# mihaibujanca/dynamicfusion

Hardware: AMD Instinct MI355X
Metric: frames/sec integrate+raycast, 640x480->512^3 TSDF (higher is better)
Workload: dtype f32 (fp16 TSDF / u16 weight storage, f64 exp + normalise as in the reference)

## Files before the change

dynamicfusion_amd/build.py:

```python
import os
import re
import shutil
import subprocess

PKG_DIR = os.path.dirname(os.path.abspath(__file__))
REPO_DIR = os.path.dirname(PKG_DIR)
CSRC = os.path.join(PKG_DIR, "csrc")
LIB_PATH = os.path.join(PKG_DIR, "libdfusion_hip.so")

SOURCES = ["dfusion_volume.hip", "dfusion_warp.hip", "dfusion_warp_nodes.hip", "dfusion_warp_points.hip", "dfusion_warp_index.hip",
           "dfusion_raycast.hip", "dfusion_frontend.hip", "dfusion_solver.hip", "dfusion_selftest.hip", "dfusion_warp_extend.hip", "dfusion_mesh.hip", "dfusion_associate.hip"]
HEADERS = ["dfusion_device.h", "dfusion_internal.h", "dfusion_nanoflann.h", "dfusion_pyramid.h", "dfusion_warp_topk.h", "dfusion_warp_sweep.h",
           "dfusion_warp_blocks.h", "dfusion_warp_pipe.h", os.path.join(REPO_DIR, "include", "dfusion.h")]

HIPCC_FLAGS = ["--offload-arch=gfx950", "-O3", "-std=c++17", "-ffp-contract=off", "-fPIC", "-shared",
               "-fno-fast-math", "-Wno-unused-result"]


def _hipcc():
    for cand in (shutil.which("hipcc"), "/opt/rocm/bin/hipcc"):
        if cand and os.path.exists(cand):
            return cand
    raise RuntimeError("hipcc not found: the dynamicfusion_amd HIP library cannot be built")


def _stale():
    if not os.path.exists(LIB_PATH):
        return True
    t = os.path.getmtime(LIB_PATH)
    deps = [os.path.join(CSRC, s) for s in SOURCES] + [h if os.path.isabs(h) else os.path.join(CSRC, h) for h in HEADERS]
    return any(os.path.getmtime(d) > t for d in deps)


def _csrc_includes(name, seen):
    if name in seen:
        return seen
    seen.append(name)
    for inc in re.findall(r'^#include "([^"]+)"', open(os.path.join(CSRC, name)).read(), re.M):
        if os.path.exists(os.path.join(CSRC, inc)):
            _csrc_includes(inc, seen)
    return seen


def kernel_source_sha(kernel):
    import hashlib
    k = kernel.replace("void ", "")
    f = ("dfusion_warp_nodes.hip" if k.startswith(("df_pack", "df_node"))
         else "dfusion_warp_points.hip" if k.startswith("df_points")
         else "dfusion_warp_index.hip" if k.startswith(("df_brick", "df_scan", "df_grow"))
         else "dfusion_warp.hip" if k.startswith(("df_warp", "df_sweep", "df_block", "df_blocks", "df_dists_max", "df_alive"))
         else "dfusion_raycast.hip" if k.startswith(("df_raycast", "df_extract"))
         else "dfusion_solver.hip" if k.startswith("df_sv")
         else "dfusion_mesh.hip" if k.startswith("df_mesh")
         else "dfusion_associate.hip" if k.startswith("df_assoc")
         else "dfusion_volume.hip")
    h = hashlib.sha256()
    for name in _csrc_includes(f, []):
        h.update(open(os.path.join(CSRC, name), "rb").read())
    return h.hexdigest()


def build_library(force=False, verbose=False):
    if not force and not _stale():
        return LIB_PATH
    cmd = [_hipcc()] + HIPCC_FLAGS + ["-I", os.path.join(REPO_DIR, "include"), "-I", CSRC]
    cmd += [os.path.join(CSRC, s) for s in SOURCES] + ["-o", LIB_PATH + ".tmp"]
    if verbose:
        print(" ".join(cmd))
    subprocess.check_call(cmd)
    os.replace(LIB_PATH + ".tmp", LIB_PATH)
    return LIB_PATH


HOST_DIR = os.path.join(PKG_DIR, "host")
HOST_LIB = os.path.join(HOST_DIR, "libkfusion_hip.so")
HOST_APP = os.path.join(HOST_DIR, "headless_frame")
HOST_KINFU_APP = os.path.join(HOST_DIR, "kinfu_headless")
HOST_WARP_TESTS = os.path.join(HOST_DIR, "warp_tests")
HOST_DEMO_CALLS = os.path.join(HOST_DIR, "demo_calls")
HOST_REG_SOLVE = os.path.join(HOST_DIR, "reg_solve")
HOST_ROBUST_SOLVE = os.path.join(HOST_DIR, "robust_solve")
HOST_ASSOCIATE = os.path.join(HOST_DIR, "associate")
HOST_PLANE_SOLVE = os.path.join(HOST_DIR, "plane_solve")
HOST_ZSLAB_LIB = os.path.join(HOST_DIR, "libkfusion_zslab.so")
HOST_ZSLAB_APP = os.path.join(HOST_DIR, "zslab_frame")


def build_host(force=False, verbose=False):
    build_library(force=False)
    src = os.path.join(HOST_DIR, "src", "kfusion_hip.cpp")
    app = os.path.join(HOST_DIR, "apps", "headless_frame.cpp")
    app2 = os.path.join(HOST_DIR, "apps", "kinfu_headless.cpp")
    app3 = os.path.join(HOST_DIR, "apps", "warp_tests.cpp")
    app4 = os.path.join(HOST_DIR, "apps", "demo_calls.cpp")
    zsrc = os.path.join(HOST_DIR, "src", "zslab_rccl.cpp")
    app5 = os.path.join(HOST_DIR, "apps", "zslab_frame.cpp")
    app6 = os.path.join(HOST_DIR, "apps", "reg_solve.cpp")
    app7 = os.path.join(HOST_DIR, "apps", "robust_solve.cpp")
    app8 = os.path.join(HOST_DIR, "apps", "associate.cpp")
    app9 = os.path.join(HOST_DIR, "apps", "plane_solve.cpp")
    deps = [src, app, app2, app3, app4, zsrc, app5, app6, app7, app8, app9, LIB_PATH] + [os.path.join(r, f) for r, _, fs in os.walk(os.path.join(HOST_DIR, "include")) for f in fs]
    outs = (HOST_LIB, HOST_APP, HOST_KINFU_APP, HOST_WARP_TESTS, HOST_DEMO_CALLS, HOST_ZSLAB_LIB, HOST_ZSLAB_APP, HOST_REG_SOLVE, HOST_ROBUST_SOLVE, HOST_ASSOCIATE, HOST_PLANE_SOLVE)
    if not force and all(os.path.exists(f) for f in outs) and min(os.path.getmtime(f) for f in outs) >= max(os.path.getmtime(d) for d in deps):
        return HOST_LIB, HOST_APP
    rocm = os.environ.get("ROCM_PATH", "/opt/rocm")
    common = ["g++", "-std=c++17", "-O2", "-D__HIP_PLATFORM_AMD__", "-I", os.path.join(HOST_DIR, "include"),
              "-I", os.path.join(REPO_DIR, "include"), "-I", os.path.join(rocm, "include")]
    link = ["-L", PKG_DIR, "-ldfusion_hip", "-L", os.path.join(rocm, "lib"), "-lamdhip64"]
    cmds = [common + ["-fPIC", "-shared", src, "-o", HOST_LIB] + link + ["-Wl,-rpath,$ORIGIN/.."],
            common + [app, "-o", HOST_APP, "-L", HOST_DIR, "-lkfusion_hip"] + link + ["-Wl,-rpath,$ORIGIN", "-Wl,-rpath,$ORIGIN/.."],
            common + [app2, "-o", HOST_KINFU_APP, "-L", HOST_DIR, "-lkfusion_hip"] + link + ["-Wl,-rpath,$ORIGIN", "-Wl,-rpath,$ORIGIN/.."],
            common + [app3, "-o", HOST_WARP_TESTS, "-L", HOST_DIR, "-lkfusion_hip"] + link + ["-Wl,-rpath,$ORIGIN", "-Wl,-rpath,$ORIGIN/.."],
            common + [app4, "-o", HOST_DEMO_CALLS, "-L", HOST_DIR, "-lkfusion_hip"] + link + ["-Wl,-rpath,$ORIGIN", "-Wl,-rpath,$ORIGIN/.."],
            common + [app6, "-o", HOST_REG_SOLVE, "-L", HOST_DIR, "-lkfusion_hip"] + link + ["-Wl,-rpath,$ORIGIN", "-Wl,-rpath,$ORIGIN/.."],
            common + [app7, "-o", HOST_ROBUST_SOLVE, "-L", HOST_DIR, "-lkfusion_hip"] + link + ["-Wl,-rpath,$ORIGIN", "-Wl,-rpath,$ORIGIN/.."],
            common + [app8, "-o", HOST_ASSOCIATE, "-L", HOST_DIR, "-lkfusion_hip"] + link + ["-Wl,-rpath,$ORIGIN", "-Wl,-rpath,$ORIGIN/.."],
            common + [app9, "-o", HOST_PLANE_SOLVE, "-L", HOST_DIR, "-lkfusion_hip"] + link + ["-Wl,-rpath,$ORIGIN", "-Wl,-rpath,$ORIGIN/.."],
            common + ["-fPIC", "-shared", zsrc, "-o", HOST_ZSLAB_LIB, "-L", HOST_DIR, "-lkfusion_hip"] + link + ["-lrccl", "-Wl,-rpath,$ORIGIN", "-Wl,-rpath,$ORIGIN/.."],
            common + [app5, "-o", HOST_ZSLAB_APP, "-L", HOST_DIR, "-lkfusion_zslab", "-lkfusion_hip"] + link + ["-lrccl", "-Wl,-rpath,$ORIGIN", "-Wl,-rpath,$ORIGIN/.."]]
    for c in cmds:
        if verbose:
            print(" ".join(c))
        subprocess.check_call(c)
    return HOST_LIB, HOST_APP


if __name__ == "__main__":
    print(build_library(force=True, verbose=True))
    print(build_host(force=True, verbose=True))
```

dynamicfusion_amd/capi.py:

```python
import ctypes as C
import os

from . import build as _build

_lib = None


class DfVolume(C.Structure):
    _fields_ = [("data", C.c_void_p), ("dims", C.c_int * 3), ("voxel_size", C.c_float * 3),
                ("trunc_dist", C.c_float), ("max_weight", C.c_int)]


class DfIcpLevel(C.Structure):
    _fields_ = [("curr", C.c_void_p), ("curr_pitch", C.c_size_t), ("ncurr", C.c_void_p), ("ncurr_pitch", C.c_size_t),
                ("prev", C.c_void_p), ("prev_pitch", C.c_size_t), ("nprev", C.c_void_p), ("nprev_pitch", C.c_size_t),
                ("cols", C.c_int), ("rows", C.c_int), ("iters", C.c_int)]


class DfSlab(C.Structure):
    _fields_ = [("z_store0", C.c_int), ("z_store_n", C.c_int), ("z_own0", C.c_int), ("z_own_n", C.c_int)]


DF_WARP_NO_CULL = 1
DF_WARP_NO_TABLE = 2
DF_WARP_NO_WEIGHT_TABLE = 4
DF_WARP_NO_LDS = 8
DF_WARP_NO_PIPELINE = 16
DF_WARP_NO_ZERO_SKIP = 32
DF_WARP_NO_DEPTH_PYRAMID = 64
DF_WARP_NO_BLOCK_MODEL = 128
DF_WARP_BLOCK_MODEL_NOW = 256
DF_WARP_NO_PREFETCH = 512
DF_WARP_STEADY_PREFETCH = 1024
DF_WARP_NO_CODES = 2048
DF_RIGID_NO_DEPTH_CULL = 1
DF_RIGID_NO_SHORT_FORMS = 2
DF_RIGID_KEEP_ALL = 4
DF_RIGID_NO_SAT = 8
DF_RIGID_POISON_SCRATCH = 16
DF_INDEX_VOXEL_TABLE = 1
DF_INDEX_WEIGHT_TABLE = 2
DF_INDEX_TABLES_ON_DEMAND = 4

SYMBOLS = [
    "dfusion_abi_version", "dfusion_error_string", "dfusion_clear", "dfusion_compute_dists", "dfusion_project_and_remove", "dfusion_integrate",
    "dfusion_raycast_points", "dfusion_raycast_depth", "dfusion_raycast_march", "dfusion_raycast_shade", "dfusion_extract_cloud",
    "dfusion_extract_normals", "dfusion_warp_create", "dfusion_warp_destroy",
    "dfusion_warp_set_nodes", "dfusion_warp_set_transforms", "dfusion_warp_build_index", "dfusion_knn",
    "dfusion_warp_points", "dfusion_integrate_warped", "dfusion_copy_bandwidth_probe", "dfusion_read_bandwidth_probe",
    "dfusion_bilateral_filter", "dfusion_truncate_depth", "dfusion_depth_pyramid", "dfusion_compute_normals_mask_depth",
    "dfusion_compute_point_normals", "dfusion_resize_depth_normals", "dfusion_resize_points_normals",
    "dfusion_icp_workspace_floats", "dfusion_icp_sums_points", "dfusion_icp_sums_depth", "dfusion_transform_points", "dfusion_warp_solve_data_term", "dfusion_warp_index_info", "dfusion_icp_estimate", "dfusion_release_scratch", "dfusion_raycast_points_of_keys",
    "dfusion_selftest_exact_forms", "dfusion_warp_set_point_tiling", "dfusion_integrate_ex", "dfusion_warp_debug_counters", "dfusion_warp_alive_blocks", "dfusion_warp_coded_blocks", "dfusion_raycast_points_of_keys_rows", "dfusion_raycast_sum_pieces", "dfusion_raycast_min_pieces", "dfusion_integrate_warped_prepare", "dfusion_integrate_warped_sweep",
    "dfusion_render_image_points", "dfusion_render_image_depth", "dfusion_render_tangent_colors", "dfusion_cloud_to_depth",
    "dfusion_warp_extend", "dfusion_warp_solve", "dfusion_warp_node_graph", "dfusion_extract_mesh",
    "dfusion_warp_solve_robust", "dfusion_associate_projective", "dfusion_warp_solve_plane",
]


class DfusionError(RuntimeError):
    pass


def library_path():
    return _build.LIB_PATH


def lib():
    global _lib
    if _lib is not None:
        return _lib
    try:
        import torch
    except Exception:
        pass
    path = _build.LIB_PATH
    try:
        path = _build.build_library()
    except Exception as e:
        if not os.path.exists(path):
            raise DfusionError("libdfusion_hip.so is missing and could not be built: %s" % e)
    _lib = load(path)
    return _lib


def load(path, strict=True):
    L = C.CDLL(path)
    if not strict:
        class _Missing:
            missing = True
        for s in SYMBOLS:
            if not hasattr(L, s):
                setattr(L, s, _Missing())
    fp = C.POINTER(C.c_float)
    vp = C.c_void_p
    L.dfusion_abi_version.restype = C.c_int
    L.dfusion_error_string.restype = C.c_char_p
    L.dfusion_error_string.argtypes = [C.c_int]
    L.dfusion_clear.argtypes = [DfVolume, C.POINTER(DfSlab), vp]
    L.dfusion_compute_dists.argtypes = [vp, C.c_size_t, vp, C.c_size_t, C.c_int, C.c_int, fp, vp]
    L.dfusion_project_and_remove.argtypes = [vp, C.c_size_t, vp, C.c_size_t, C.c_int, C.c_int, vp, C.c_ulonglong, fp, vp, vp, vp]
    L.dfusion_integrate.argtypes = [vp, C.c_size_t, C.c_int, C.c_int, DfVolume, C.POINTER(DfSlab), fp, fp, vp, vp]
    L.dfusion_raycast_points.argtypes = [DfVolume, C.POINTER(DfSlab), fp, fp, fp, vp, C.c_size_t, vp, C.c_size_t,
                                         C.c_int, C.c_int, C.c_float, C.c_float, vp, vp]
    L.dfusion_raycast_depth.argtypes = [DfVolume, C.POINTER(DfSlab), fp, fp, fp, vp, C.c_size_t, vp, C.c_size_t,
                                        C.c_int, C.c_int, C.c_float, C.c_float, vp]
    L.dfusion_raycast_march.argtypes = [DfVolume, C.POINTER(DfSlab), fp, fp, C.c_int, C.c_int, C.c_float, C.c_uint, vp, vp]
    L.dfusion_raycast_shade.argtypes = [DfVolume, C.POINTER(DfSlab), fp, fp, fp, vp, vp, C.c_size_t, vp, C.c_size_t,
                                        C.c_int, C.c_int, C.c_float, vp]
    L.dfusion_raycast_points_of_keys.argtypes = [fp, fp, fp, vp, vp, C.c_size_t, vp, C.c_size_t, C.c_int, C.c_int, vp]
    L.dfusion_raycast_points_of_keys_rows.argtypes = [fp, fp, fp, vp, vp, C.c_size_t, vp, C.c_size_t, C.c_int, C.c_int, C.c_int, C.c_int, vp]
    L.dfusion_extract_cloud.argtypes = [DfVolume, C.POINTER(DfSlab), fp, vp, C.c_ulonglong, vp, vp]
    L.dfusion_extract_normals.argtypes = [DfVolume, C.POINTER(DfSlab), fp, fp, vp, C.c_ulonglong, C.c_float, vp, vp]
    L.dfusion_extract_mesh.argtypes = [DfVolume, C.POINTER(DfSlab), fp, vp, C.c_ulonglong, vp, C.c_ulonglong, vp, vp]
    L.dfusion_warp_create.argtypes = [C.POINTER(vp)]
    L.dfusion_warp_destroy.argtypes = [vp]
    L.dfusion_warp_set_nodes.argtypes = [vp, vp, vp, vp, C.c_int, vp]
    L.dfusion_warp_set_transforms.argtypes = [vp, vp, vp]
    L.dfusion_warp_build_index.argtypes = [vp, DfVolume, C.POINTER(DfSlab), fp, C.c_int, C.c_uint, vp]
    L.dfusion_knn.argtypes = [vp, C.c_int, vp, C.c_int, vp, vp, vp]
    L.dfusion_warp_points.argtypes = [vp, C.c_int, vp, vp, C.c_int, fp, vp]
    L.dfusion_integrate_warped.argtypes = [vp, C.c_size_t, C.c_int, C.c_int, DfVolume, C.POINTER(DfSlab), fp, fp, fp,
                                           vp, C.c_int, C.c_uint, vp, vp]
    sz = C.c_size_t
    L.dfusion_bilateral_filter.argtypes = [vp, sz, vp, sz, C.c_int, C.c_int, C.c_int, C.c_float, C.c_float, vp]
    L.dfusion_truncate_depth.argtypes = [vp, sz, C.c_int, C.c_int, C.c_float, vp]
    L.dfusion_cloud_to_depth.argtypes = [vp, sz, vp, sz, C.c_int, C.c_int, vp]
    L.dfusion_depth_pyramid.argtypes = [vp, sz, C.c_int, C.c_int, vp, sz, C.c_float, vp]
    L.dfusion_compute_normals_mask_depth.argtypes = [vp, sz, vp, sz, C.c_int, C.c_int, fp, vp]
    L.dfusion_compute_point_normals.argtypes = [vp, sz, vp, sz, vp, sz, C.c_int, C.c_int, fp, vp]
    L.dfusion_resize_depth_normals.argtypes = [vp, sz, vp, sz, C.c_int, C.c_int, vp, sz, vp, sz, vp]
    L.dfusion_resize_points_normals.argtypes = [vp, sz, vp, sz, C.c_int, C.c_int, vp, sz, vp, sz, vp]
    L.dfusion_transform_points.argtypes = [vp, sz, C.c_int, vp, sz, C.c_int, C.c_int, C.c_int, fp, vp]
    L.dfusion_warp_solve_data_term.argtypes = [vp, C.c_int, vp, vp, C.c_int, C.c_int, C.c_float, vp, vp, vp]
    L.dfusion_warp_solve.argtypes = [vp, C.c_int, vp, vp, C.c_int, C.c_int, C.c_float, C.c_int, C.c_float, vp, vp, vp]
    L.dfusion_warp_node_graph.argtypes = [vp, C.c_int, vp, vp, vp]
    L.dfusion_warp_solve_robust.argtypes = [vp, C.c_int, vp, vp, C.c_int, C.c_int, C.c_float, C.c_int, C.c_float, C.c_int, C.c_float, C.c_float,
                                            vp, vp, vp, vp, vp]
    L.dfusion_warp_solve_plane.argtypes = [vp, C.c_int, vp, vp, vp, C.c_int, C.c_int, C.c_float, C.c_int, C.c_float, C.c_int, C.c_float, C.c_float,
                                           vp, vp, vp, vp, vp]
    L.dfusion_associate_projective.argtypes = [vp, vp, C.c_int, vp, C.c_size_t, vp, C.c_size_t, C.c_int, C.c_int, fp, C.c_float, C.c_float, C.c_float,
                                               vp, vp, vp, vp]
    L.dfusion_warp_extend.argtypes = [vp, C.c_int, vp, C.c_int, C.c_float, C.c_float, C.c_int, vp, vp, vp, C.POINTER(C.c_int),
                                      C.POINTER(C.c_int), vp]
    L.dfusion_warp_index_info.argtypes = [vp, C.POINTER(C.c_ulonglong), C.POINTER(C.c_uint), C.POINTER(C.c_int)]
    L.dfusion_selftest_exact_forms.argtypes = [C.c_ulonglong, vp, vp]
    L.dfusion_raycast_sum_pieces.argtypes = [vp, C.c_int, C.c_ulonglong, vp, vp]
    L.dfusion_raycast_min_pieces.argtypes = [vp, C.c_int, C.c_ulonglong, vp, vp]
    L.dfusion_integrate_warped_prepare.argtypes = [vp, C.c_size_t, C.c_int, C.c_int, DfVolume, C.POINTER(DfSlab), fp, fp, fp, vp, C.c_int, C.c_uint, vp]
    L.dfusion_integrate_warped_sweep.argtypes = [DfVolume, C.POINTER(DfSlab), vp, vp, vp]
    L.dfusion_warp_set_point_tiling.argtypes = [vp, C.c_int]
    L.dfusion_icp_estimate.argtypes = [C.POINTER(DfIcpLevel), C.c_int, C.c_int, fp, C.c_float, C.c_float, vp, vp, vp]
    L.dfusion_icp_workspace_floats.argtypes = [C.c_int, C.c_int]
    L.dfusion_icp_sums_points.argtypes = [vp, sz, vp, sz, vp, sz, vp, sz, C.c_int, C.c_int, fp, fp, C.c_float, C.c_float, vp, vp, vp, vp]
    L.dfusion_icp_sums_depth.argtypes = [vp, sz, vp, sz, vp, sz, vp, sz, C.c_int, C.c_int, fp, fp, C.c_float, C.c_float, vp, vp, vp, vp]
    L.dfusion_render_image_points.argtypes = [vp, sz, vp, sz, C.c_int, C.c_int, fp, vp, sz, vp]
    L.dfusion_render_image_depth.argtypes = [vp, sz, vp, sz, C.c_int, C.c_int, fp, fp, vp, sz, vp]
    L.dfusion_render_tangent_colors.argtypes = [vp, sz, C.c_int, C.c_int, vp, sz, vp]
    L.dfusion_integrate_ex.argtypes = [vp, C.c_size_t, C.c_int, C.c_int, DfVolume, C.POINTER(DfSlab), fp, fp, C.c_uint, vp, vp, vp]
    L.dfusion_warp_debug_counters.argtypes = [vp, vp]
    L.dfusion_warp_alive_blocks.argtypes = [vp, C.c_int, C.c_int, vp, C.c_int, vp]
    L.dfusion_warp_coded_blocks.argtypes = [vp, C.c_int, C.c_int, vp, C.c_int, vp]
    L.dfusion_copy_bandwidth_probe.argtypes = [vp, vp, C.c_size_t, vp]
    L.dfusion_read_bandwidth_probe.argtypes = [vp, C.c_size_t, vp, vp]
    for s in SYMBOLS:
        if s not in ("dfusion_error_string",):
            getattr(L, s).restype = C.c_int
    return L


def check(rc, what=""):
    if rc != 0:
        msg = lib().dfusion_error_string(rc)
        raise DfusionError("%s failed: %s (code %d)" % (what or "dfusion call", msg.decode() if msg else "?", rc))


def floats(seq):
    seq = [float(x) for x in seq]
    return (C.c_float * len(seq))(*seq)
```

dynamicfusion_amd/csrc/dfusion_internal.h:

```cpp
#pragma once
#include <hip/hip_runtime.h>
#include <stdint.h>
#include <string.h>
#include <memory>
#include <utility>
#include "dfusion.h"
#include "dfusion_device.h"
#include "dfusion_nanoflann.h"

#define DF_BRICK 8
#define DF_WARP_PREFETCH_MARGIN_M 0.05f
#define DF_WARP_PREFETCH_CAP 1024u

#define DF_HIP(expr) do { hipError_t e__ = (expr); if (e__ != hipSuccess) return (int)e__; } while (0)
#define DF_LAUNCH_CHECK() do { hipError_t e__ = hipGetLastError(); if (e__ != hipSuccess) return (int)e__; } while (0)

static inline DfSlab df_slab_or_full(const DfVolume& v, const DfSlab* s)
{
    if (s) return *s;
    DfSlab f; f.z_store0 = 0; f.z_store_n = v.dims[2]; f.z_own0 = 0; f.z_own_n = v.dims[2]; return f;
}
static inline bool df_slab_valid(const DfVolume& v, const DfSlab& s)
{
    return s.z_store_n > 0 && s.z_own_n >= 0 && s.z_store0 >= 0 && s.z_store0 + s.z_store_n <= v.dims[2] &&
           s.z_own0 >= s.z_store0 && s.z_own0 + s.z_own_n <= s.z_store0 + s.z_store_n;
}
static inline bool df_volume_valid(const DfVolume& v)
{
    return v.data && v.dims[0] > 0 && v.dims[1] > 0 && v.dims[2] > 0 && (v.dims[0] % 4) == 0 &&
           v.voxel_size[0] > 0 && v.voxel_size[1] > 0 && v.voxel_size[2] > 0 && v.trunc_dist > 0;
}
static inline DfAff df_aff(const float a[12]) { DfAff r; memcpy(r.R, a, 36); memcpy(r.t, a + 9, 12); return r; }
static inline bool df_pitch_ok(size_t pitch, int cols, size_t bpp) { return cols > 0 && pitch >= (size_t)cols * bpp; }

struct DfWarpView {
    const float4* pos_sigma;
    const float4* rot;
    const float4* dual;
    const float4* node_t;
    const float4* rt;
    int M;
    const uint32_t* brick_off;
    const uint16_t* brick_list;
    const float* brick_thr;
    int bx, by, bz;
    DfNfView nf;
};

template <typename T>
struct DfDevBuf {
    T* p = nullptr; size_t cap = 0;
    DfDevBuf() = default;
    DfDevBuf(DfDevBuf&& o) noexcept : p(o.p), cap(o.cap) { o.p = nullptr; o.cap = 0; }
    DfDevBuf& operator=(DfDevBuf&& o) noexcept { std::swap(p, o.p); std::swap(cap, o.cap); return *this; }
    ~DfDevBuf() { (void)hipFree(p); }
    operator T*() const { return p; }
    void release() { (void)hipFree(p); p = nullptr; cap = 0; }
    int reserve(size_t n)
    {
        if (n <= cap) return DF_OK;
        release();
        DF_HIP(hipMalloc((void**)&p, n * sizeof(T)));
        cap = n;
        return DF_OK;
    }
};

struct DfPrepared;

struct __attribute__((visibility("hidden"))) DfWarpField {
    DfWarpField(); ~DfWarpField();
    int device = 0;
    int M = 0, cap = 0;
    DfDevBuf<float4> pos_sigma, rot, dual, node_t;
    DfDevBuf<uint32_t> brick_off, brick_cnt; DfDevBuf<uint16_t> brick_list; DfDevBuf<float> brick_thr;
    size_t off_cap = 0;
    DfDevBuf<uint32_t> scan_tmp; size_t scan_cap = 0;
    int bx = 0, by = 0, bz = 0, k_built = 0;
    int geom_dims[3] = {}; float geom_vs[3] = {}; float geom_aff[12] = {};
    float geom_inv[12] = {}; bool geom_inv_ok = false;
    bool index_valid = false;
    unsigned index_flags = 0; DfSlab index_slab = {};
    DfDevBuf<uint16_t> knn_tab;
    int tab_z0 = 0, tab_zn = 0, tab_k = 0; bool tab_valid = false;
    DfDevBuf<float> w_tab; bool w_tab_valid = false;
    DfDevBuf<float> tile_wmax;
    DfDevBuf<float> bounds_dev;
    int max_phase = 0;
    std::unique_ptr<DfPrepared> prep; bool prep_valid = false;
    hipEvent_t ev_prep_done = nullptr, ev_sweep_done[2] = {}; bool split_events = false;
    DfDevBuf<float4> rot_alt, dual_alt, node_t_alt;
    DfDevBuf<float4> rt, rt_alt;
    unsigned long long seq = 0, recorded_seq = 0;
    unsigned long long ring_seq[2] = {};
    unsigned long long node_reader[2] = {}; int nphase = 0;
    unsigned long long plan_reader[2] = {};
    DfDevBuf<unsigned long long> plan_mask2[2]; DfDevBuf<unsigned int> plan_list2[2]; int pphase = 0; unsigned hphase = 0;
    DfDevBuf<unsigned long long> plan_code2[2];
    DfDevBuf<uint16_t> pyr_mem;
    DfDevBuf<char> solver_ws;
    DfDevBuf<int> graph_nbr; DfDevBuf<float> graph_alpha; DfDevBuf<unsigned int> graph_in_off, graph_in_edge; DfDevBuf<char> graph_ws;
    int graph_kg = 0;
    DfDevBuf<int> pt_ids;
    int pt_image_cols = 0;
    DfDevBuf<DfNfNode> nf_nodes; DfDevBuf<uint16_t> nf_vpos; bool nf_ok = false; int nf_depth = 0;
    DfDevBuf<unsigned int> plan_hist; size_t plan_cap = 0;
    DfDevBuf<uint8_t> blk_state; DfDevBuf<float> blk_wmax; DfDevBuf<uint8_t> blk_alive; DfDevBuf<uint32_t> blk_work, blk_cnt; size_t blk_cap = 0; int blk_phase = 0;
    DfDevBuf<uint8_t> blk_tie;
    DfDevBuf<uint16_t> bm_idx; DfDevBuf<uint32_t> bm_lam, bm_w; DfDevBuf<uint8_t> bm_cnt; size_t bm_cap = 0;
    DfDevBuf<uint32_t> code_tab; size_t code_cap = 0; DfDevBuf<uint32_t> bm_ids; DfDevBuf<uint8_t> bm_coded;
    bool tab_complete = false;
    int tab_sweeps = 0;
    unsigned long long* dbg_swept = nullptr;
    bool alive_valid = false;
    hipStream_t side = nullptr; hipEvent_t ev_fork = nullptr, ev_join = nullptr; bool side_pending = false;
    volatile uint32_t* host_report = nullptr;
    DfDevBuf<char> ext_ws;
    DfDevBuf<char> grow_ws;
};

#define DF_DISPATCH_K(k, ...)                             \
    switch (k) {                                          \
        case 1: { constexpr int K = 1; __VA_ARGS__; } break; \
        case 2: { constexpr int K = 2; __VA_ARGS__; } break; \
        case 3: { constexpr int K = 3; __VA_ARGS__; } break; \
        case 4: { constexpr int K = 4; __VA_ARGS__; } break; \
        case 5: { constexpr int K = 5; __VA_ARGS__; } break; \
        case 6: { constexpr int K = 6; __VA_ARGS__; } break; \
        case 7: { constexpr int K = 7; __VA_ARGS__; } break; \
        case 8: { constexpr int K = 8; __VA_ARGS__; } break; \
        default: return DF_E_INVALID;                     \
    }

struct DfWarpedArgs;
#define DF_LOCAL __attribute__((visibility("hidden")))
DF_LOCAL DfWarpView df_view(const DfWarpField* wf);
DF_LOCAL int df_side_init(DfWarpField* wf);
DF_LOCAL int df_side_join(DfWarpField* wf, hipStream_t st);
DF_LOCAL void df_side_drain(DfWarpField* wf);
DF_LOCAL int df_wait_split_sweep(DfWarpField* wf, hipStream_t st);
DF_LOCAL int df_wait_reader(DfWarpField* wf, unsigned long long reader, hipStream_t st);
DF_LOCAL int df_wait_all_sweeps_host(DfWarpField* wf);
DF_LOCAL int df_warp_reserve(DfWarpField* wf, int M);
DF_LOCAL int df_warp_pack_current(DfWarpField* wf, const float* pos, const float* dq, const float* sigma, hipStream_t st);
DF_LOCAL int df_warp_build_tie_tree(DfWarpField* wf, hipStream_t st);
DF_LOCAL int df_index_bricks(DfWarpField* wf, const DfVolume& v, const float vol2world[12], int k, hipStream_t st);
DF_LOCAL DfWarpedArgs df_table_args(const DfWarpField* wf);
DF_LOCAL int df_tables_complete(DfWarpField* wf, hipStream_t st);
DF_LOCAL int df_build_voxel_table(DfWarpField* wf, const DfVolume& v, const DfSlab& s, const float vol2world[12], int k, bool weights,
                                  bool on_demand, hipStream_t st);

struct DfScratchEntry;
DF_LOCAL DfScratchEntry* df_scratch_acquire(hipStream_t st, size_t bytes, char** mem_out);
DF_LOCAL void df_scratch_release(DfScratchEntry* entry);
struct DfScratchHold {
    char* mem = nullptr; DfScratchEntry* entry;
    DfScratchHold(hipStream_t st, size_t bytes) : entry(df_scratch_acquire(st, bytes, &mem)) {}
    ~DfScratchHold() { if (entry) df_scratch_release(entry); }
    DfScratchHold(const DfScratchHold&) = delete; DfScratchHold& operator=(const DfScratchHold&) = delete;
};

int df_warp_grow(DfWarpField* wf, const float* pos, const float* dq, const float* sigma, int Mn, hipStream_t st);

template <int K>
__device__ __forceinline__ void dqb_weights(const DfWarpView& W, const float (&bd)[K], const int (&bi)[K], float (&wt)[K])
{
#pragma unroll
    for (int i = 0; i < K; ++i) wt[i] = dqb_weight(bd[i], W.pos_sigma[bi[i]].w);
}
template <int K>
__device__ __forceinline__ void dqb_blend_w(const DfWarpView& W, const float (&wt)[K], const int (&bi)[K], quat* rot_out,
                                            quat* dual_out)
{
    quat tsum, rsum;
    tsum.w = tsum.x = tsum.y = tsum.z = 0.f;
    rsum.w = rsum.x = rsum.y = rsum.z = 0.f;
#pragma unroll
    for (int i = 0; i < K; ++i) {
        const int j = bi[i];
        const float w = wt[i];
        const float4 t4 = W.node_t[j], r4 = W.rot[j];
        quat t, r;
        t.w = t4.x; t.x = t4.y; t.y = t4.z; t.z = t4.w;
        r.w = r4.x; r.x = r4.y; r.y = r4.z; r.z = r4.w;
        tsum = q_add(tsum, q_scale(w, t));
        rsum = q_add(rsum, q_scale(w, r));
    }
    rsum = q_normalize(rsum);
    quat half;
    half.w = 0.5f * tsum.w; half.x = 0.5f * tsum.x; half.y = 0.5f * tsum.y; half.z = 0.5f * tsum.z;
    *rot_out = rsum;
    *dual_out = q_mul(half, rsum);
}
```

dynamicfusion_amd/csrc/dfusion_warp.hip:

```cpp
#include "dfusion_internal.h"
#include "dfusion_pyramid.h"
#include "dfusion_warp_sweep.h"
#include "dfusion_warp_blocks.h"
#include "dfusion_warp_pipe.h"
#include <atomic>
#include <stdlib.h>
#include <stdio.h>
#include <math.h>

__global__ __launch_bounds__(256) void df_dists_max_kernel(const uint16_t* __restrict__ dists, size_t pitch, int cols, int rows,
                                                           float* __restrict__ out)
{
    float m = 0.f;
    for (int i = blockIdx.x * 256 + threadIdx.x; i < cols * rows; i += gridDim.x * 256) {
        const int y = i / cols, x = i - y * cols;
        const float d = h2f_bits(*(const uint16_t*)((const char*)dists + (size_t)y * pitch + 2 * (size_t)x));
        if (!(d <= 3.0e38f)) m = 3.0e38f;
        else m = fmaxf(m, d);
    }
#pragma unroll
    for (int o = 32; o >= 1; o >>= 1) m = fmaxf(m, __shfl_xor(m, o, 64));
    if ((threadIdx.x & 63) == 0) atomicMax((unsigned int*)out, __float_as_uint(m));
}

static double df_tile_radius(const float vol2world[12], double nx, double ny, double nz, const DfVolume& v)
{
    double r = 0.0;
    for (int sx = -1; sx <= 1; sx += 2) for (int sy = -1; sy <= 1; sy += 2) for (int sz = -1; sz <= 1; sz += 2) {
        double ex = sx * 0.5 * (nx - 1) * v.voxel_size[0], ey = sy * 0.5 * (ny - 1) * v.voxel_size[1], ez = sz * 0.5 * (nz - 1) * v.voxel_size[2];
        double wx = vol2world[0] * ex + vol2world[1] * ey + vol2world[2] * ez;
        double wy = vol2world[3] * ex + vol2world[4] * ey + vol2world[5] * ez;
        double wz = vol2world[6] * ex + vol2world[7] * ey + vol2world[8] * ez;
        double d = sqrt(wx * wx + wy * wy + wz * wz);
        if (d > r) r = d;
    }
    return r;
}

extern "C" int dfusion_warp_debug_counters(DfWarpField* wf, unsigned long long* swept_dev)
{
    if (!wf) return DF_E_INVALID;
    wf->dbg_swept = swept_dev;
    return DF_OK;
}

__global__ __launch_bounds__(256) void df_alive_per_layer_kernel(const uint8_t* __restrict__ alive, unsigned mask, unsigned per_layer, int layer0, int l_lo,
                                                                 int l_hi, unsigned long long* __restrict__ out)
{
    __shared__ unsigned s[4];
    const int layer = layer0 + (int)blockIdx.x;
    if (layer < l_lo || layer >= l_hi) return;
    const uint8_t* a = alive + (size_t)blockIdx.x * per_layer;
    unsigned n = 0;
    for (unsigned i = threadIdx.x; i < per_layer; i += 256) n += (a[i] & mask) ? 1u : 0u;
#pragma unroll
    for (int o = 32; o >= 1; o >>= 1) n += __shfl_xor(n, o, 64);
    if ((threadIdx.x & 63) == 0) s[threadIdx.x >> 6] = n;
    __syncthreads();
    if (threadIdx.x == 0) atomicAdd(&out[layer], (unsigned long long)(s[0] + s[1] + s[2] + s[3]));
}
static int df_count_verdicts(DfWarpField* wf, unsigned mask, int z0, int zn, unsigned long long* per_layer_dev, int n_layers, dfStream stream)
{
    if (!wf || !per_layer_dev || n_layers <= 0 || z0 < 0 || zn < 0) return DF_E_INVALID;
    if (!wf->tab_valid || !wf->alive_valid || !wf->blk_alive) return DF_E_NO_INDEX;
    const int ntx = (wf->geom_dims[0] + DF_TAB_TX - 1) / DF_TAB_TX, nty = (wf->geom_dims[1] + DF_TAB_TY - 1) / DF_TAB_TY;
    const unsigned per_layer = (unsigned)(ntx * (DF_TAB_TX / 8)) * (unsigned)(nty * (DF_TAB_TY / 8));
    const int nbz = wf->tab_zn / 8, layer0 = wf->tab_z0 / 8;
    const int l_lo = (z0 + 7) / 8, l_hi = min((z0 + zn) / 8, n_layers);
    if (nbz <= 0 || l_hi <= l_lo) return DF_OK;
    hipLaunchKernelGGL(df_alive_per_layer_kernel, dim3((unsigned)nbz), dim3(256), 0, (hipStream_t)stream, wf->blk_alive, mask, per_layer, layer0, l_lo,
                       l_hi, per_layer_dev);
    DF_LAUNCH_CHECK();
    return DF_OK;
}
extern "C" int dfusion_warp_alive_blocks(DfWarpField* wf, int z0, int zn, unsigned long long* per_layer_dev, int n_layers, dfStream stream)
{
    return df_count_verdicts(wf, 0xffu, z0, zn, per_layer_dev, n_layers, stream);
}
extern "C" int dfusion_warp_coded_blocks(DfWarpField* wf, int z0, int zn, unsigned long long* per_layer_dev, int n_layers, dfStream stream)
{
    return df_count_verdicts(wf, 2u, z0, zn, per_layer_dev, n_layers, stream);
}

DfWarpedArgs df_table_args(const DfWarpField* wf)
{
    DfWarpedArgs a;
    memset(&a, 0, sizeof(a));
    const int ntx = (wf->geom_dims[0] + DF_TAB_TX - 1) / DF_TAB_TX, nty = (wf->geom_dims[1] + DF_TAB_TY - 1) / DF_TAB_TY;
    a.w_tab = wf->w_tab_valid ? wf->w_tab : nullptr;
    a.tile_wmax = wf->w_tab_valid ? wf->tile_wmax : nullptr;
    a.blk_wmax = wf->w_tab_valid ? wf->blk_wmax : nullptr;
    a.X = wf->geom_dims[0]; a.Y = wf->geom_dims[1]; a.Z = wf->geom_dims[2];
    a.z_store0 = wf->tab_z0; a.z_own0 = wf->tab_z0; a.z_own_n = wf->tab_zn;
    a.vsx = wf->geom_vs[0]; a.vsy = wf->geom_vs[1]; a.vsz = wf->geom_vs[2];
    a.vol2world = df_aff(wf->geom_aff);
    a.knn_tab = wf->knn_tab; a.tab_z0 = wf->tab_z0; a.tab_ntx = ntx; a.tab_nty = nty;
    a.tab_nvox = (size_t)ntx * DF_TAB_TX * nty * DF_TAB_TY * wf->tab_zn;
    a.bz0 = wf->tab_z0 / DF_BRICK;
    a.bm_nbx = ntx * (DF_TAB_TX / 8); a.bm_nby = nty * (DF_TAB_TY / 8);
    a.code_tab = wf->code_tab; a.bm_ids = wf->bm_ids; a.bm_coded = wf->bm_coded;
    a.blk_tie = wf->blk_tie;
    return a;
}
static size_t df_lds_limit()
{
    static std::atomic<size_t> cached{0};
    size_t v = cached.load();
    if (v) return v;
    int dev = 0, bytes = 0;
    if (hipGetDevice(&dev) != hipSuccess || hipDeviceGetAttribute(&bytes, hipDeviceAttributeMaxSharedMemoryPerBlock, dev) != hipSuccess || bytes < 64 * 1024) {
        (void)hipGetLastError();
        bytes = 64 * 1024;
    }
    v = (size_t)bytes < (size_t)160 * 1024 ? (size_t)bytes : (size_t)160 * 1024;
    cached.store(v);
    return v;
}

static unsigned df_work_grid(const void* kernel)
{
    int per_cu = 0, dev = 0; hipDeviceProp_t prop;
    if (hipOccupancyMaxActiveBlocksPerMultiprocessor(&per_cu, kernel, 256, 0) != hipSuccess || per_cu < 1) per_cu = 2;
    if (hipGetDevice(&dev) != hipSuccess || hipGetDeviceProperties(&prop, dev) != hipSuccess || prop.multiProcessorCount < 1) return 512u;
    return (unsigned)per_cu * (unsigned)prop.multiProcessorCount;
}

static int df_build_listed(DfWarpField* wf, const uint32_t* cnt, hipStream_t st, int list = 0)
{
    DfWarpedArgs b = df_table_args(wf);
    b.work = wf->blk_work + (size_t)list * wf->blk_cap; b.work_cnt = cnt + (list ? 3 : 0); b.work_cursor = const_cast<uint32_t*>(cnt) + (list ? 4 : 2);
    b.work_cap = list ? DF_WARP_PREFETCH_CAP : 0u;
    const DfWarpView W = df_view(wf);
    static unsigned grid[9] = {0};
    DF_DISPATCH_K(wf->tab_k, {
        if (!grid[K]) grid[K] = df_work_grid((const void*)df_warp_brick_kernel<K, true>);
        df_warp_brick_kernel<K, true><<<dim3(grid[K]), dim3(256), 0, st>>>(b, W);
    });
    DF_LAUNCH_CHECK();
    return DF_OK;
}

int df_tables_complete(DfWarpField* wf, hipStream_t st)
{
    if (wf->tab_complete) return DF_OK;
    const DfWarpedArgs b = df_table_args(wf);
    const int nbz = wf->tab_zn / 8;
    const size_t nblk = (size_t)b.bm_nbx * b.bm_nby * nbz;
    uint32_t* cnt = wf->blk_cnt + 8 * wf->blk_phase;
    uint32_t* cnt_next = wf->blk_cnt + 8 * (wf->blk_phase ^ 1);
    hipLaunchKernelGGL(df_blocks_unbuilt_kernel, dim3((unsigned)((nblk + 255) / 256)), dim3(256), 0, st, b.bm_nbx, b.bm_nby, nbz, wf->bx, wf->by,
                       wf->tab_z0 / 8, wf->blk_state, wf->blk_work, cnt, cnt_next);
    DF_LAUNCH_CHECK();
    wf->blk_phase ^= 1;
    int rc = df_build_listed(wf, cnt, st);
    if (rc) return rc;
    wf->tab_complete = true;
    return DF_OK;
}

static int df_block_verdicts(DfWarpField* wf, DfWarpedArgs& a, int k, unsigned flags, hipStream_t st)
{
    const int nbx = a.tab_ntx * (DF_TAB_TX / 8), nby = a.tab_nty * (DF_TAB_TY / 8), nbz = wf->tab_zn / 8;
    const size_t nblk = (size_t)nbx * nby * nbz;
    if (nblk == 0 || nblk > wf->blk_cap) return DF_E_INVALID;
    const bool use_models = !(flags & DF_WARP_NO_BLOCK_MODEL) && (k == 8 || k == 4);
    const int want_models = !use_models ? 0 : (flags & DF_WARP_BLOCK_MODEL_NOW) ? 2 : wf->tab_sweeps >= 1 ? 1 : 0;
    if (want_models && nblk > wf->bm_cap) {
        wf->bm_cap = 0;
        { int rc = wf->bm_idx.reserve(nblk * DF_BM_NU); if (rc) return rc; }
        { int rc = wf->bm_lam.reserve(nblk * DF_BM_NU); if (rc) return rc; }
        { int rc = wf->bm_w.reserve(nblk * DF_BM_NU); if (rc) return rc; }
        { int rc = wf->bm_cnt.reserve(nblk); if (rc) return rc; }
        wf->bm_cap = nblk;
    }
    if (want_models && k == 8 && (nblk * 512 > wf->code_cap || !wf->bm_ids || !wf->code_tab || !wf->bm_coded)) {
        wf->code_cap = 0;
        { int rc = wf->bm_ids.reserve(nblk * 64); if (rc) return rc; }
        { int rc = wf->code_tab.reserve(nblk * 512); if (rc) return rc; }
        { int rc = wf->bm_coded.reserve(nblk); if (rc) return rc; }
        DF_HIP(hipMemsetAsync(wf->bm_coded, 0, nblk, st));
        wf->code_cap = nblk * 512;
    }
    bool ahead = !(flags & (DF_WARP_NO_PREFETCH | DF_WARP_BLOCK_MODEL_NOW));
    if (ahead) { int rc = df_side_init(wf); if (rc) return rc; }
    if (ahead && !(flags & DF_WARP_STEADY_PREFETCH) && wf->tab_sweeps >= 8 && (wf->tab_sweeps & 7) != 0 && wf->host_report &&
        wf->host_report[0] == 0u && wf->host_report[1] == 0u && wf->host_report[2] == 0u) ahead = false;
    const bool quiet = !ahead && !(flags & (DF_WARP_NO_PREFETCH | DF_WARP_BLOCK_MODEL_NOW));
    const int want_models_policy = want_models;
    const int want_models_now = quiet ? 0 : want_models_policy;
    a.pf_margin = ahead && !wf->tab_complete && wf->tab_sweeps >= 1 ? DF_WARP_PREFETCH_MARGIN_M : 0.f;
    a.pf_cap = DF_WARP_PREFETCH_CAP;
    uint32_t* cnt = wf->blk_cnt + 8 * wf->blk_phase;
    uint32_t* cnt_next = wf->blk_cnt + 8 * (wf->blk_phase ^ 1);
    uint32_t* list_urgent = wf->blk_work, *list_ahead = wf->blk_work + wf->blk_cap, *list_model = wf->blk_work + 2 * wf->blk_cap;
    hipLaunchKernelGGL(df_block_verdict_kernel, dim3((unsigned)((nblk + 255) / 256)), dim3(256), 0, st, a, wf->rot, wf->node_t, nbx, nby, nbz,
                       wf->blk_state, wf->blk_wmax, wf->brick_thr + wf->off_cap, wf->bx, wf->by, a.tile_wmax != nullptr ? 1 : 0,
                       (use_models && wf->bm_cap >= nblk ? 1 : 0) | (k == 8 && wf->bm_cnt && wf->code_tab && wf->bm_ids && wf->bm_coded && wf->code_cap >= nblk * 512 ? 2 : 0),
                       want_models_now,
                       wf->tab_complete ? 0 : 1, wf->bm_idx, wf->bm_lam, wf->bm_w, wf->bm_cnt, wf->bm_coded, wf->blk_alive, list_urgent, list_ahead, list_model,
                       cnt, cnt_next);
    a.blk_cnt = cnt; a.host_report = (uint32_t*)wf->host_report; a.sweep_no = (uint32_t)wf->tab_sweeps;
    DF_LAUNCH_CHECK();
#ifdef DF_TRACE_VERDICT
    if (getenv("DF_TRACE_VERDICT_FILE")) {
        DF_HIP(hipStreamSynchronize(st));
        static unsigned long long h[8192 * 4];
        DF_HIP(hipMemcpyFromSymbol(h, HIP_SYMBOL(g_df_vtrace), sizeof(h)));
        FILE* f = fopen(getenv("DF_TRACE_VERDICT_FILE"), "wb");
        if (f) { fwrite(h, 8, 8192 * 4, f); fclose(f); }
    }
#endif
    wf->blk_phase ^= 1;
    auto launch_models = [&](hipStream_t s2) -> int {
        const DfWarpedArgs b = df_table_args(wf);
        static unsigned g8 = 0, g4 = 0;
        if (!g8) {
            g8 = df_work_grid((const void*)df_block_model_kernel<8>); g4 = df_work_grid((const void*)df_block_model_kernel<4>);
        }
        if (k == 8) hipLaunchKernelGGL(df_block_model_kernel<8>, dim3(g8), dim3(256), 0, s2, b, nbx, nby, nbz, list_model, cnt + 1,
                                       wf->bm_idx, wf->bm_lam, wf->bm_w, wf->bm_cnt, wf->blk_state);
        else hipLaunchKernelGGL(df_block_model_kernel<4>, dim3(g4), dim3(256), 0, s2, b, nbx, nby, nbz, list_model, cnt + 1,
                                wf->bm_idx, wf->bm_lam, wf->bm_w, wf->bm_cnt, wf->blk_state);
        DF_LAUNCH_CHECK();
        return DF_OK;
    };
    const bool side_work = ahead && (!wf->tab_complete || want_models_now);
    if (side_work) {
        DF_HIP(hipEventRecord(wf->ev_fork, st));
        DF_HIP(hipStreamWaitEvent(wf->side, wf->ev_fork, 0));
        int rc_side = DF_OK;
        if (!wf->tab_complete) rc_side = df_build_listed(wf, cnt, wf->side, 1);
        if (rc_side == DF_OK && want_models_now) rc_side = launch_models(wf->side);
        if (hipEventRecord(wf->ev_join, wf->side) == hipSuccess) wf->side_pending = true;
        else { (void)hipGetLastError(); df_side_drain(wf); if (rc_side == DF_OK) rc_side = (int)hipErrorUnknown; }
        if (rc_side != DF_OK) return rc_side;
    }
    if (!wf->tab_complete) { int rc = df_build_listed(wf, cnt, st, 0); if (rc) return rc; }
    if (want_models_now && !ahead) { int rc = launch_models(st); if (rc) return rc; }
    a.blk_alive = wf->blk_alive; a.bm_nbx = nbx; a.bm_nby = nby;
    wf->alive_valid = true;
    return DF_OK;
}

typedef void (*df_lds_kernel_t)(const DfWarpedArgs, const DfWarpView, int);
struct DfPrepared { DfWarpedArgs a; DfWarpView W; df_lds_kernel_t kern; dim3 grid; unsigned threads; size_t lds; int tiles_x; DfVolume v; DfSlab s; unsigned long long seq; };
DfWarpField::DfWarpField() = default;
DfWarpField::~DfWarpField() = default;
enum { DF_MODE_WHOLE = 0, DF_MODE_PREPARE = 1 };

static int df_integrate_warped_impl(const uint16_t* dists, size_t pitch, int cols, int rows, DfVolume v, const DfSlab* slab,
                                    const float vol2world[12], const float world2cam[12], const float proj[4],
                                    DfWarpField* wf, int k, unsigned flags, unsigned long long* n_updated, dfStream stream, int mode);

extern "C" int dfusion_integrate_warped(const uint16_t* dists, size_t pitch, int cols, int rows, DfVolume v, const DfSlab* slab,
                                        const float vol2world[12], const float world2cam[12], const float proj[4],
                                        DfWarpField* wf, int k, unsigned flags, unsigned long long* n_updated, dfStream stream)
{
    return df_integrate_warped_impl(dists, pitch, cols, rows, v, slab, vol2world, world2cam, proj, wf, k, flags, n_updated, stream, DF_MODE_WHOLE);
}

extern "C" int dfusion_integrate_warped_prepare(const uint16_t* dists, size_t pitch, int cols, int rows, DfVolume geometry, const DfSlab* slab,
                                                const float vol2world[12], const float world2cam[12], const float proj[4],
                                                DfWarpField* wf, int k, unsigned flags, dfStream stream)
{
    if (!wf) return DF_E_INVALID;
    if (!wf->split_events) {
        hipEvent_t e[3] = {nullptr, nullptr, nullptr};
        for (int i = 0; i < 3; ++i)
            if (hipEventCreateWithFlags(&e[i], hipEventDisableTiming) != hipSuccess) {
                for (int j = 0; j < i; ++j) (void)hipEventDestroy(e[j]);
                return (int)hipGetLastError();
            }
        wf->ev_prep_done = e[0]; wf->ev_sweep_done[0] = e[1]; wf->ev_sweep_done[1] = e[2]; wf->split_events = true;
    }
    wf->prep_valid = false;
    if (!geometry.data) geometry.data = (void*)(size_t)16;
    const int rc = df_integrate_warped_impl(dists, pitch, cols, rows, geometry, slab, vol2world, world2cam, proj, wf, k, flags, nullptr, stream, DF_MODE_PREPARE);
    if (rc != DF_OK) return rc;
    DF_HIP(hipEventRecord(wf->ev_prep_done, (hipStream_t)stream));
    return DF_OK;
}

extern "C" int dfusion_integrate_warped_sweep(DfVolume v, const DfSlab* slab, DfWarpField* wf, unsigned long long* n_updated, dfStream stream)
{
    if (!wf || !df_volume_valid(v)) return DF_E_INVALID;
    const DfSlab s = df_slab_or_full(v, slab);
    if (!df_slab_valid(v, s)) return DF_E_INVALID;
    if (s.z_own_n == 0) return DF_OK;
    DfPrepared* P = wf->prep.get();
    if (!P || !wf->prep_valid) return DF_E_INVALID;
    if (memcmp(P->v.dims, v.dims, sizeof(v.dims)) || memcmp(P->v.voxel_size, v.voxel_size, sizeof(v.voxel_size)) || P->v.trunc_dist != v.trunc_dist ||
        P->v.max_weight != v.max_weight || memcmp(&P->s, &s, sizeof(s))) return DF_E_INVALID;
    hipStream_t st = (hipStream_t)stream;
    wf->prep_valid = false;
    DF_HIP(hipStreamWaitEvent(st, wf->ev_prep_done, 0));
    P->a.vol = (uint32_t*)v.data; P->a.n_upd = n_updated;
    P->kern<<<P->grid, dim3(P->threads), P->lds, st>>>(P->a, P->W, P->tiles_x);
    DF_LAUNCH_CHECK();
    DF_HIP(hipEventRecord(wf->ev_sweep_done[P->seq & 1], st));
    wf->recorded_seq = P->seq; wf->ring_seq[P->seq & 1] = P->seq;
    return DF_OK;
}

static int df_integrate_warped_impl(const uint16_t* dists, size_t pitch, int cols, int rows, DfVolume v, const DfSlab* slab,
                                    const float vol2world[12], const float world2cam[12], const float proj[4],
                                    DfWarpField* wf, int k, unsigned flags, unsigned long long* n_updated, dfStream stream, int mode)
{
    if (!dists || !vol2world || !world2cam || !proj || !wf || cols <= 0 || rows <= 0 || !df_pitch_ok(pitch, cols, 2) || !df_volume_valid(v)) return DF_E_INVALID;
    if (k < 1 || k > 8 || wf->M < k) return DF_E_INVALID;
    DfSlab s = df_slab_or_full(v, slab);
    if (!df_slab_valid(v, s)) return DF_E_INVALID;
    if (!wf->index_valid || wf->k_built < k || memcmp(wf->geom_dims, v.dims, sizeof(wf->geom_dims)) ||
        memcmp(wf->geom_vs, v.voxel_size, sizeof(wf->geom_vs)) || memcmp(wf->geom_aff, vol2world, sizeof(wf->geom_aff)))
        return DF_E_NO_INDEX;
    if (s.z_own_n == 0) return DF_OK;
    hipStream_t st = (hipStream_t)stream;
    if (mode == DF_MODE_WHOLE) { int rc = df_wait_split_sweep(wf, st); if (rc) return rc; }
    { int rc = df_side_join(wf, st); if (rc) return rc; }
    wf->prep_valid = false;

    DfWarpedArgs a;
    memset(&a, 0, sizeof(a));
    a.vol = (uint32_t*)v.data; a.X = v.dims[0]; a.Y = v.dims[1]; a.Z = v.dims[2];
    a.z_store0 = s.z_store0; a.z_own0 = s.z_own0; a.z_own_n = s.z_own_n;
    a.vsx = v.voxel_size[0]; a.vsy = v.voxel_size[1]; a.vsz = v.voxel_size[2];
    a.vol2world = df_aff(vol2world); a.world2cam = df_aff(world2cam);
    {
        static const float I9[9] = {1.f, 0.f, 0.f, 0.f, 1.f, 0.f, 0.f, 0.f, 1.f};
        a.v2w_identity = memcmp(vol2world, I9, sizeof(I9)) == 0;
    }
    a.P.dists = dists; a.P.pitch = pitch; a.P.cols = cols; a.P.rows = rows;
    a.P.fx = proj[0]; a.P.fy = proj[1]; a.P.cx = proj[2]; a.P.cy = proj[3];
    a.P.trunc = v.trunc_dist; a.P.trunc_inv = 1.f / v.trunc_dist; a.P.max_weight = v.max_weight;
    a.sat_ok = df_sat_trunc_ok(v.trunc_dist) ? 1 : 0;
    a.n_upd = n_updated;
    a.n_swept = wf->dbg_swept;
    a.kf = (float)k; a.cam_scale = 1.f; a.origin_cam = -1.f;
    const bool use_tab = wf->tab_valid && wf->tab_k == k && !(flags & DF_WARP_NO_TABLE) && s.z_own0 >= wf->tab_z0 &&
                         s.z_own0 + s.z_own_n <= wf->tab_z0 + wf->tab_zn;
    const bool use_w = use_tab && wf->w_tab_valid && !(flags & DF_WARP_NO_WEIGHT_TABLE);
    if (use_tab) {
        a.knn_tab = wf->knn_tab; a.tab_z0 = wf->tab_z0;
        a.tab_ntx = (a.X + DF_TAB_TX - 1) / DF_TAB_TX; a.tab_nty = (a.Y + DF_TAB_TY - 1) / DF_TAB_TY;
        a.tab_nvox = (size_t)a.tab_ntx * DF_TAB_TX * a.tab_nty * DF_TAB_TY * wf->tab_zn;
    }
    if (use_w) a.w_tab = wf->w_tab;
    const size_t lds_limit = df_lds_limit();
    const bool no_lds = (flags & DF_WARP_NO_LDS) != 0;
    const bool lds_fits = (size_t)wf->M * 32 <= lds_limit;
    const bool pipe_form_ok = use_w && !(flags & DF_WARP_NO_PIPELINE) && pitch < (1u << 24) && rows < (1 << 24) &&
                              (unsigned long long)rows * pitch < (1ull << 32) && (unsigned long long)v.dims[0] * v.dims[1] < (1ull << 30);
    const bool pipe_sweep = use_tab && !no_lds && pipe_form_ok && (k == 8 || k == 4);

    if (!(flags & DF_WARP_NO_CULL) && proj[0] > 0.f && proj[1] > 0.f) {
        if (!(flags & DF_WARP_NO_DEPTH_PYRAMID)) {
            const size_t elems = df_pyramid_elems(cols, rows);
            { int rc = wf->pyr_mem.reserve(elems); if (rc) return rc; }
            const bool pipe_path = pipe_sweep;
            wf->max_phase ^= 1;
            unsigned int* max_word = (unsigned int*)(wf->bounds_dev + 6 + wf->max_phase);
            int rc = df_build_dists_pyramid(dists, pitch, cols, rows, wf->pyr_mem, wf->pyr_mem.cap, &a.py, st, pipe_path, nullptr,
                                            pipe_path ? max_word : nullptr);
            if (rc) return rc;
        }
        if (a.py.top == 0) {
            DF_HIP(hipMemsetAsync(wf->bounds_dev + 2, 0, sizeof(float), st));
            hipLaunchKernelGGL(df_dists_max_kernel, dim3(64), dim3(256), 0, st, dists, pitch, cols, rows, wf->bounds_dev + 2);
            DF_LAUNCH_CHECK();
        }
        {
            bool rigid = true;
            for (int i = 0; i < 3 && rigid; ++i)
                for (int j = 0; j < 3; ++j) {
                    double d = 0.0;
                    for (int r = 0; r < 3; ++r) d += (double)world2cam[3 * r + i] * world2cam[3 * r + j];
                    if (!(fabs(d - (i == j ? 1.0 : 0.0)) < 1e-5)) { rigid = false; break; }
                }
            a.origin_cam = rigid ? (float)(sqrt((double)world2cam[9] * world2cam[9] + (double)world2cam[10] * world2cam[10] +
                                                (double)world2cam[11] * world2cam[11]) * 1.0001 + 1e-6) : -1.f;
        }
        const double r = use_tab ? df_tile_radius(vol2world, DF_ROW_TX, DF_ROW_TY, DF_ROW_TZ, v)
                                 : df_tile_radius(vol2world, DF_BRICK, DF_BRICK, DF_BRICK, v);
        double fro = 0.0;
        for (int i = 0; i < 9; ++i) fro += (double)world2cam[i] * world2cam[i];
        fro = sqrt(fro);
        a.cam_scale = (float)((fabs(fro - 1.7320508075688772) < 1e-3) ? 1.001 : fro * 1.001);
        a.tile_r = (float)(r * 1.001 + 1e-6);
        a.cull = wf->bounds_dev;
        if (use_w && !(flags & DF_WARP_NO_ZERO_SKIP)) a.tile_wmax = wf->tile_wmax;
    }

    DfWarpView W = df_view(wf);
    if (use_tab && !no_lds && (pipe_sweep || lds_fits)) {
        const int tiles_x = (a.X + DF_ROW_TX - 1) / DF_ROW_TX, tiles_y = (a.Y + DF_LDS_TY - 1) / DF_LDS_TY;
        const int zt_lo = s.z_own0 / DF_ROW_TZ, zt_hi = (s.z_own0 + s.z_own_n - 1) / DF_ROW_TZ;
        a.bz0 = zt_lo;
        const bool pipe_ok = pipe_sweep;
        if (a.cull) a.tile_r = (float)(df_tile_radius(vol2world, pipe_ok ? 8 : DF_ROW_TX, pipe_ok ? 8 : DF_LDS_TY, DF_ROW_TZ, v) * 1.001 + 1e-6);
        const bool k4_table = pipe_ok && k == 4 && lds_fits;
        const size_t lds = !pipe_ok || k4_table ? (size_t)wf->M * 32 : k == 8 ? (size_t)(DF_PIPE_WGT / 64) * 4096 : 0;
        typedef void (*lds_kernel_t)(const DfWarpedArgs, const DfWarpView, int);
        lds_kernel_t kern = nullptr;
        const long long cols_layers = (long long)tiles_x * tiles_y * (zt_hi - zt_lo + 1);
        const bool pipe = pipe_sweep;
        a.zt = !pipe ? DF_LDS_ZT : cols_layers <= 8192 ? 4 : cols_layers <= 65536 ? 8 : 16;
        dim3 grid((unsigned)(tiles_x * tiles_y), (unsigned)((zt_hi - zt_lo + 1 + a.zt - 1) / a.zt));
        const bool wide = k4_table && lds > 80 * 1024;
        const bool vi = a.v2w_identity != 0;
        unsigned wg_threads = 512u;
        if (pipe_ok && k == 8) {
            kern = vi ? df_warp_rows_pipe_kernel<8, 1, DF_PIPE_WGT, true, false> : df_warp_rows_pipe_kernel<8, 1, DF_PIPE_WGT, false, false>;
            wg_threads = (unsigned)DF_PIPE_WGT;
        } else if (pipe_ok && k4_table) {
            kern = wide ? (vi ? df_warp_rows_pipe_kernel<4, 2, 1024, true, true> : df_warp_rows_pipe_kernel<4, 2, 1024, false, true>)
                        : (vi ? df_warp_rows_pipe_kernel<4, 2, 512, true, true> : df_warp_rows_pipe_kernel<4, 2, 512, false, true>);
            wg_threads = wide ? 1024u : 512u;
        } else if (pipe_ok) {
            kern = vi ? df_warp_rows_pipe_kernel<4, 2, 512, true, false> : df_warp_rows_pipe_kernel<4, 2, 512, false, false>;
        }
        else if (use_w) { DF_DISPATCH_K(k, kern = (df_warp_rows_lds_kernel<K, true, 2>)); }
        else { DF_DISPATCH_K(k, kern = (df_warp_rows_lds_kernel<K, false, 1>)); }
        if (lds > lds_limit) return DF_E_INVALID;
        DF_HIP(hipFuncSetAttribute((const void*)kern, hipFuncAttributeMaxDynamicSharedMemorySize, (int)lds_limit));
        if (!pipe) { int rc = df_tables_complete(wf, st); if (rc) return rc; }
        if (pipe) {
            const unsigned n_zb = grid.y, n_items = (unsigned)tiles_x * (unsigned)tiles_y * 2u * n_zb;
            if (n_items > wf->plan_cap) {
                { int rc = df_wait_all_sweeps_host(wf); if (rc) return rc; }
                wf->plan_cap = 0;
                for (int i = 0; i < 2; ++i) {
                    { int rc = wf->plan_mask2[i].reserve(n_items); if (rc) return rc; }
                    { int rc = wf->plan_list2[i].reserve((size_t)n_items * DF_PLAN_BINS); if (rc) return rc; }
                    { int rc = wf->plan_code2[i].reserve(n_items); if (rc) return rc; }
                }
                wf->plan_cap = n_items; wf->plan_reader[0] = wf->plan_reader[1] = 0;
            }
            if (!wf->plan_hist) {
                { int rc = wf->plan_hist.reserve(4 * 128); if (rc) return rc; }
                DF_HIP(hipMemsetAsync(wf->plan_hist, 0, 4 * 128 * sizeof(unsigned int), st));
                wf->hphase = 0;
            }
            wf->pphase ^= 1;
            { int rc = df_wait_reader(wf, wf->plan_reader[wf->pphase], st); if (rc) return rc; }
            if (a.cull) { int rc = df_block_verdicts(wf, a, k, flags, st); if (rc) return rc; }
            else { int rc = df_tables_complete(wf, st); if (rc) return rc; }
            ++wf->tab_sweeps;
            unsigned int* cnt = wf->plan_hist + 128 * (wf->hphase & 3u);
            unsigned int* cnt_next = wf->plan_hist + 128 * ((wf->hphase + 2u) & 3u);
            unsigned long long* pmask = wf->plan_mask2[wf->pphase]; unsigned int* plist = wf->plan_list2[wf->pphase];
            unsigned long long* pcode = nullptr;
            if (k == 8 && a.cull && a.blk_alive && wf->code_tab && wf->bm_ids && wf->bm_coded && wf->bm_cap >= (size_t)a.bm_nbx * a.bm_nby * (wf->tab_zn / 8) &&
                !(flags & (DF_WARP_NO_BLOCK_MODEL | DF_WARP_NO_CODES))) {
                pcode = wf->plan_code2[wf->pphase];
                a.code_tab = wf->code_tab; a.bm_ids = wf->bm_ids; a.bm_coded = wf->bm_coded;
            }
            hipLaunchKernelGGL(df_sweep_plan_kernel, dim3((n_items + DF_PLAN_WG / 64 - 1) / (DF_PLAN_WG / 64)), dim3(DF_PLAN_WG), 0, st, a, tiles_x, tiles_y, n_items, pmask, cnt,
                               plist, cnt_next, pcode);
            DF_LAUNCH_CHECK();
            a.plan_code = pcode;
            ++wf->hphase;
            a.plan_mask = pmask; a.plan_bins = plist; a.plan_cnt = cnt; a.plan_items = n_items; a.plan_tiles_y = tiles_y;
            wf->plan_reader[wf->pphase] = wf->node_reader[wf->nphase] = ++wf->seq;
            const unsigned spw = wg_threads >= 256u ? wg_threads / 256u : 1u;
            const unsigned groups = (n_items + spw - 1) / spw;
            grid = dim3(groups, 1);
#ifdef DF_TRACE_WG
            static unsigned long long* trace_dev = nullptr; static size_t trace_cap = 0;
            const size_t trace_n = (size_t)groups * (wg_threads / 64u) * 4;
            if (trace_n > trace_cap) { (void)hipFree(trace_dev); DF_HIP(hipMalloc((void**)&trace_dev, trace_n * 8)); trace_cap = trace_n; }
            DF_HIP(hipMemsetAsync(trace_dev, 0, trace_n * 8, st));
            a.trace = trace_dev;
            kern<<<grid, dim3(wg_threads), lds, st>>>(a, W, tiles_x);
            if (getenv("DF_TRACE_FILE")) {
                DF_HIP(hipStreamSynchronize(st));
                unsigned long long* h = (unsigned long long*)malloc(trace_n * 8);
                DF_HIP(hipMemcpy(h, trace_dev, trace_n * 8, hipMemcpyDeviceToHost));
                FILE* f = fopen(getenv("DF_TRACE_FILE"), "wb");
                if (f) { unsigned long long hdr[4] = {groups, 1, (unsigned long long)(wg_threads / 64u), 0}; fwrite(hdr, 8, 4, f); fwrite(h, 8, trace_n, f); fclose(f); }
                free(h);
            }
            DF_LAUNCH_CHECK();
            return DF_OK;
#endif
        }
        if (mode == DF_MODE_PREPARE) {
            if (!pipe) return DF_E_INVALID;
            if (!wf->prep) wf->prep.reset(new DfPrepared());
            DfPrepared* P = wf->prep.get();
            P->a = a; P->W = W; P->kern = kern; P->grid = grid; P->threads = wg_threads; P->lds = lds; P->tiles_x = tiles_x; P->v = v; P->s = s;
            P->seq = wf->seq;
            wf->prep_valid = true;
            return DF_OK;
        }
        kern<<<grid, dim3(wg_threads), lds, st>>>(a, W, tiles_x);
        if (pipe && wf->split_events) {
            DF_LAUNCH_CHECK();
            DF_HIP(hipEventRecord(wf->ev_sweep_done[wf->seq & 1], st));
            wf->recorded_seq = wf->seq; wf->ring_seq[wf->seq & 1] = wf->seq;
        }
    } else if (use_tab) {
        if (mode == DF_MODE_PREPARE) return DF_E_INVALID;
        { int rc = df_tables_complete(wf, st); if (rc) return rc; }
        const int tiles_x = (a.X + DF_ROW_TX - 1) / DF_ROW_TX, tiles_y = (a.Y + DF_ROW_TY - 1) / DF_ROW_TY;
        const int zt_lo = s.z_own0 / DF_ROW_TZ, zt_hi = (s.z_own0 + s.z_own_n - 1) / DF_ROW_TZ;
        a.bz0 = zt_lo;
        dim3 grid((unsigned)(tiles_x * tiles_y), (unsigned)(zt_hi - zt_lo + 1));
        if (use_w) { DF_DISPATCH_K(k, df_warp_rows_kernel<K, true, 4><<<grid, dim3(256), 0, st>>>(a, W, tiles_x)); }
        else { DF_DISPATCH_K(k, df_warp_rows_kernel<K, false, 4><<<grid, dim3(256), 0, st>>>(a, W, tiles_x)); }
    } else {
        if (mode == DF_MODE_PREPARE) return DF_E_INVALID;
        const int bz_lo = s.z_own0 / DF_BRICK, bz_hi = (s.z_own0 + s.z_own_n - 1) / DF_BRICK;
        a.bz0 = bz_lo;
        dim3 grid((unsigned)(W.bx * W.by), (unsigned)(bz_hi - bz_lo + 1));
        DF_DISPATCH_K(k, df_warp_brick_kernel<K, false><<<grid, dim3(256), 0, st>>>(a, W));
    }
    DF_LAUNCH_CHECK();
    return DF_OK;
}

int df_build_voxel_table(DfWarpField* wf, const DfVolume& v, const DfSlab& s, const float vol2world[12], int k, bool weights,
                                bool on_demand, hipStream_t st)
{
    (void)vol2world;
    if (s.z_own_n == 0) return DF_OK;
    const int bz_lo = s.z_own0 / DF_BRICK, bz_hi = (s.z_own0 + s.z_own_n - 1) / DF_BRICK;
    const int tz0 = bz_lo * DF_BRICK, tzn = (bz_hi - bz_lo + 1) * DF_BRICK;
    const int ntx = (v.dims[0] + DF_TAB_TX - 1) / DF_TAB_TX, nty = (v.dims[1] + DF_TAB_TY - 1) / DF_TAB_TY;
    if (ntx * (DF_TAB_TX / 8) > 1023 || nty * (DF_TAB_TY / 8) > 1023 || bz_hi > 4095) return DF_E_INVALID;
    const size_t nvox = (size_t)ntx * DF_TAB_TX * nty * DF_TAB_TY * tzn;
    const size_t need = nvox * k;
    { int rc = wf->knn_tab.reserve(need); if (rc) return rc; }
    if (weights) { int rc = wf->w_tab.reserve(need); if (rc) return rc; }
    const size_t ntile = (size_t)ntx * nty * (tzn / DF_TAB_TZ);
    if (weights) {
        { int rc = wf->tile_wmax.reserve(ntile); if (rc) return rc; }
        DF_HIP(hipMemsetAsync(wf->tile_wmax, 0, ntile * sizeof(float), st));
    }
    const size_t nblk = (size_t)ntx * (DF_TAB_TX / 8) * nty * (DF_TAB_TY / 8) * (tzn / 8);
    if (nblk > wf->blk_cap) {
        wf->blk_cap = 0;
        { int rc = wf->blk_state.reserve(nblk); if (rc) return rc; }
        { int rc = wf->blk_tie.reserve(nblk); if (rc) return rc; }
        { int rc = wf->blk_wmax.reserve(nblk); if (rc) return rc; }
        { int rc = wf->blk_alive.reserve(nblk); if (rc) return rc; }
        { int rc = wf->blk_work.reserve(3 * nblk); if (rc) return rc; }
        wf->blk_cap = nblk;
    }
    { int rc = wf->blk_cnt.reserve(16); if (rc) return rc; }
    DF_HIP(hipMemsetAsync(wf->blk_cnt, 0, 16 * sizeof(uint32_t), st));
    DF_HIP(hipMemsetAsync(wf->blk_state, on_demand ? 0 : 1, nblk, st));
    DF_HIP(hipMemsetAsync(wf->blk_tie, 0, nblk, st));
    DF_HIP(hipMemsetAsync(wf->blk_wmax, 0, nblk * sizeof(float), st));
    wf->blk_phase = 0;
    wf->tab_z0 = tz0; wf->tab_zn = tzn; wf->tab_k = k; wf->tab_valid = true; wf->w_tab_valid = weights;
    wf->tab_complete = !on_demand; wf->tab_sweeps = 0; wf->alive_valid = false;
    if (on_demand) return DF_OK;
    const DfWarpedArgs a = df_table_args(wf);
    DfWarpView W = df_view(wf);
    dim3 grid((unsigned)(W.bx * W.by), (unsigned)(bz_hi - bz_lo + 1));
    DF_DISPATCH_K(k, df_warp_brick_kernel<K, true><<<grid, dim3(256), 0, st>>>(a, W));
    hipError_t e = hipGetLastError();
    if (e == hipSuccess) e = hipStreamSynchronize(st);
    if (e != hipSuccess) {
        wf->tab_valid = false; wf->w_tab_valid = false; wf->tab_complete = false;
        return (int)e;
    }
    return DF_OK;
}
```

dynamicfusion_amd/csrc/dfusion_warp_blocks.h:

```cpp
#pragma once
#include "dfusion_warp_sweep.h"

#define DF_BM_NU 16
#define DF_BM_NONE 0xffu

struct DfIv { float lo, hi; };
__device__ __forceinline__ DfIv iv(float lo, float hi) { DfIv r; r.lo = lo; r.hi = hi; return r; }
__device__ __forceinline__ DfIv iv_add(DfIv a, DfIv b) { return iv(a.lo + b.lo, a.hi + b.hi); }
__device__ __forceinline__ DfIv iv_sub(DfIv a, DfIv b) { return iv(a.lo - b.hi, a.hi - b.lo); }
__device__ __forceinline__ DfIv iv_mul(DfIv a, DfIv b)
{
    const float p0 = a.lo * b.lo, p1 = a.lo * b.hi, p2 = a.hi * b.lo, p3 = a.hi * b.hi;
    return iv(fminf(fminf(p0, p1), fminf(p2, p3)), fmaxf(fmaxf(p0, p1), fmaxf(p2, p3)));
}
__device__ __forceinline__ DfIv iv_sq(DfIv a)
{
    const float l2 = a.lo * a.lo, h2 = a.hi * a.hi;
    return iv((a.lo <= 0.f && a.hi >= 0.f) ? 0.f : fminf(l2, h2), fmaxf(l2, h2));
}
struct DfIv3 { DfIv x, y, z; };
__device__ __forceinline__ DfIv3 iv_cross(const DfIv3& a, const DfIv3& b)
{
    DfIv3 r;
    r.x = iv_sub(iv_mul(a.y, b.z), iv_mul(a.z, b.y));
    r.y = iv_sub(iv_mul(a.z, b.x), iv_mul(a.x, b.z));
    r.z = iv_sub(iv_mul(a.x, b.y), iv_mul(a.y, b.x));
    return r;
}

__device__ __forceinline__ uint32_t df_f2h_up(float x)
{
    _Float16 h = (_Float16)x;
    unsigned short b = __builtin_bit_cast(unsigned short, h);
    if ((float)h < x) b = (unsigned short)(b + 1u);
    return b;
}
__device__ __forceinline__ uint32_t df_bm_pack(float lo, float hi)
{
    const _Float16 m = (_Float16)(0.5f * (lo + hi));
    const float mf = (float)m;
    const float hw = fmaxf(hi - mf, mf - lo) * 1.00390625f + 1e-7f;
    return (uint32_t)__builtin_bit_cast(unsigned short, m) | (df_f2h_up(hw) << 16);
}

template <int K>
__global__ __launch_bounds__(256, K == 8 ? 3 : 4) void df_block_model_kernel(const DfWarpedArgs a, int nbx, int nby, int nbz, const uint32_t* __restrict__ list,
                                                             const uint32_t* __restrict__ count, uint16_t* __restrict__ bm_idx,
                                                             uint32_t* __restrict__ bm_lam, uint32_t* __restrict__ bm_w,
                                                             uint8_t* __restrict__ bm_cnt, uint8_t* __restrict__ blk_state)
{
    __shared__ uint32_t s_idx[4][DF_BM_NU], s_lam[4][DF_BM_NU], s_w[4][DF_BM_NU];
    __shared__ float s_hw[4][DF_BM_NU];
    const int wave = threadIdx.x >> 6, ln = threadIdx.x & 63;
    const size_t nblk = (size_t)nbx * nby * nbz;
    const uint32_t n_work = *count;
    for (uint32_t it = blockIdx.x * 4 + wave; it < n_work; it += gridDim.x * 4) {
    const size_t blk = list[it];
    const int bx = (int)(blk % (size_t)nbx), by = (int)((blk / (size_t)nbx) % (size_t)nby), bz = (int)(blk / ((size_t)nbx * nby));
    const int x = bx * 8 + (ln & 7), y = by * 8 + (ln >> 3), z0 = a.tab_z0 + bz * 8;
    const bool col_in = x < a.X && y < a.Y;
    int ids[8][K];
    float wv[8][K], inv[8];
    bool bad = false;
    unsigned valid = 0;
#pragma unroll
    for (int j = 0; j < 8; ++j) {
        const bool in = col_in && z0 + j < a.Z;
        const size_t tv = df_tab_index(a, in ? x : 0, in ? y : 0, in ? z0 + j : z0);
        knn_tab_load<K>(a.knn_tab, tv, ids[j]);
        w_tab_load<K>(a.w_tab, a.tab_nvox, tv, wv[j]);
        float s = 0.f;
#pragma unroll
        for (int i = 0; i < K; ++i) s += wv[j][i];
        inv[j] = 1.f / s;
        if (in) { valid |= 1u << j; if (!(s > 1e-30f && s < 3.0e38f)) bad = true; }
    }
    bad = __builtin_amdgcn_ballot_w64(bad) != 0ull;
    const bool any_valid = __builtin_amdgcn_ballot_w64(valid != 0u) != 0ull;
    int n = 0, last = -1;
    bool overflow = false;
    if (!bad && any_valid) {
        for (;;) {
            int cand = 0x7fffffff;
#pragma unroll
            for (int j = 0; j < 8; ++j)
                if (valid & (1u << j)) {
#pragma unroll
                    for (int i = 0; i < K; ++i) { const int id = ids[j][i]; cand = (id > last && id < cand) ? id : cand; }
                }
#pragma unroll
            for (int o = 32; o >= 1; o >>= 1) cand = min(cand, __shfl_xor(cand, o, 64));
            if (cand == 0x7fffffff) break;
            if (n == DF_BM_NU) { overflow = true; break; }
            float lmin = 3.0e38f, lmax = 0.f, wmin = 3.0e38f, wmax = 0.f;
#pragma unroll
            for (int j = 0; j < 8; ++j)
                if (valid & (1u << j)) {
                    float w = 0.f;
#pragma unroll
                    for (int i = 0; i < K; ++i) w = ids[j][i] == cand ? wv[j][i] : w;
                    const float lam = w * inv[j];
                    lmin = fminf(lmin, lam); lmax = fmaxf(lmax, lam); wmin = fminf(wmin, w); wmax = fmaxf(wmax, w);
                }
#pragma unroll
            for (int o = 32; o >= 1; o >>= 1) {
                lmin = fminf(lmin, __shfl_xor(lmin, o, 64)); lmax = fmaxf(lmax, __shfl_xor(lmax, o, 64));
                wmin = fminf(wmin, __shfl_xor(wmin, o, 64)); wmax = fmaxf(wmax, __shfl_xor(wmax, o, 64));
            }
            if (ln == 0) {
                const uint32_t lp = df_bm_pack(lmin * (1.f - 0x1p-18f), lmax * (1.f + 0x1p-18f));
                s_idx[wave][n] = (uint32_t)cand; s_lam[wave][n] = lp; s_w[wave][n] = df_bm_pack(wmin, wmax);
                s_hw[wave][n] = h2f_bits(lp >> 16);
            }
            last = cand; ++n;
        }
    }
    __builtin_amdgcn_wave_barrier();
    if constexpr (K == 8) {
        if (a.code_tab && a.bm_ids && !any_valid) { if (ln == 0) a.bm_coded[blk] = 0; }
        if (a.code_tab && a.bm_ids && any_valid) {
            unsigned code[8];
#pragma unroll
            for (int j = 0; j < 8; ++j) code[j] = 0u;
            int last_h[2] = {-1, -1};
            bool sub_over = false;
            const bool writer = (ln & 0x1b) == 0;
            const unsigned qd = ((unsigned)(ln >> 2) & 1u) | (((unsigned)(ln >> 5) & 1u) << 1);
            uint32_t* ids_out = a.bm_ids + blk * 64;
            ids_out[ln] = 0u;
            __builtin_amdgcn_wave_barrier();
            for (int e = 0;; ++e) {
                int cand_h[2];
#pragma unroll
                for (int h = 0; h < 2; ++h) {
                    int c = 0x7fffffff;
#pragma unroll
                    for (int j = 4 * h; j < 4 * h + 4; ++j)
                        if (valid & (1u << j)) {
#pragma unroll
                            for (int i = 0; i < K; ++i) { const int id = ids[j][i]; c = (id > last_h[h] && id < c) ? id : c; }
                        }
                    c = min(c, __shfl_xor(c, 1, 64)); c = min(c, __shfl_xor(c, 2, 64)); c = min(c, __shfl_xor(c, 8, 64)); c = min(c, __shfl_xor(c, 16, 64));
                    cand_h[h] = c;
                }
                if (__builtin_amdgcn_ballot_w64(cand_h[0] != 0x7fffffff || cand_h[1] != 0x7fffffff) == 0ull) break;
                if (e == DF_BM_NU) { sub_over = true; break; }
#pragma unroll
                for (int h = 0; h < 2; ++h) {
                    if (cand_h[h] == 0x7fffffff) continue;
#pragma unroll
                    for (int j = 4 * h; j < 4 * h + 4; ++j)
                        if (valid & (1u << j)) {
                            unsigned hit = 0u;
#pragma unroll
                            for (int i = 0; i < K; ++i) hit = ids[j][i] == cand_h[h] ? (unsigned)e << (4 * i) : hit;
                            code[j] |= hit;
                        }
                    if (writer) ((uint16_t*)(ids_out + qd * 16 + (unsigned)e))[h] = (uint16_t)cand_h[h];
                    last_h[h] = cand_h[h];
                }
            }
            if (!sub_over) {
#pragma unroll
                for (int j = 0; j < 8; ++j)
                    if (col_in && z0 + j < a.Z) a.code_tab[df_code_index(a, x, y, z0 + j)] = code[j];
            }
            __builtin_amdgcn_wave_barrier();
            if (ln == 0) a.bm_coded[blk] = sub_over ? (uint8_t)0 : (uint8_t)1;
        }
    }
    if (ln == 0) blk_state[blk] = 2;
    if (bad || overflow || n == 0) { if (ln == 0) bm_cnt[blk] = DF_BM_NONE; continue; }
    float h = ln < n ? s_hw[wave][ln] : -1.f;
    int e0 = ln;
#pragma unroll
    for (int o = 32; o >= 1; o >>= 1) {
        const float ho = __shfl_xor(h, o, 64); const int eo = __shfl_xor(e0, o, 64);
        if (ho > h || (ho == h && eo < e0)) { h = ho; e0 = eo; }
    }
    if (ln < n) {
        const int dst = ln == e0 ? 0 : ln == 0 ? e0 : ln;
        bm_idx[(size_t)dst * nblk + blk] = (uint16_t)s_idx[wave][ln];
        bm_lam[(size_t)dst * nblk + blk] = s_lam[wave][ln];
        bm_w[(size_t)dst * nblk + blk] = s_w[wave][ln];
    }
    if (ln == 0) bm_cnt[blk] = (uint8_t)n;
    __builtin_amdgcn_wave_barrier();
    }
}

__device__ __forceinline__ bool df_block_box_dead(const DfWarpedArgs& a, const float4* __restrict__ rot, const float4* __restrict__ node_t,
                                                  int nbx, int nby, size_t nblk, size_t blk, unsigned n, const uint16_t* __restrict__ bm_idx,
                                                  const uint32_t* __restrict__ bm_lam, const uint32_t* __restrict__ bm_w)
{
    float slm = 0.f, Nx = 0.f, Ny = 0.f, Nz = 0.f, Ex = 0.f, Ey = 0.f, Ez = 0.f, Dmin = 3.0e38f, Dmax = 0.f;
    float Tx = 0.f, Ty = 0.f, Tz = 0.f, Fx = 0.f, Fy = 0.f, Fz = 0.f, sx = 0.f, sy = 0.f, sz = 0.f;
    {   const float4 r0 = rot[bm_idx[blk]]; sx = r0.y; sy = r0.z; sz = r0.w; }
    for (unsigned e0 = 0; e0 < n; e0 += 4) {
        unsigned id[4]; uint32_t lp[4], wp[4];
#pragma unroll
        for (int i = 0; i < 4; ++i) {
            const size_t at = (size_t)min(e0 + (unsigned)i, n - 1u) * nblk + blk;
            id[i] = bm_idx[at]; lp[i] = bm_lam[at]; wp[i] = bm_w[at];
        }
        float4 r4[4], t4[4];
#pragma unroll
        for (int i = 0; i < 4; ++i) { r4[i] = rot[id[i]]; t4[i] = node_t[id[i]]; }
#pragma unroll
        for (int i = 0; i < 4; ++i) {
            const bool on = e0 + (unsigned)i < n;
            const float lm = on ? h2f_bits(lp[i]) : 0.f, lh = on ? h2f_bits(lp[i] >> 16) : 0.f, wm = on ? h2f_bits(wp[i]) : 0.f, wh = on ? h2f_bits(wp[i] >> 16) : 0.f;
            slm += lm;
            Nx += lm * r4[i].y; Ny += lm * r4[i].z; Nz += lm * r4[i].w;
            Ex += lh * fabsf(r4[i].y - sx); Ey += lh * fabsf(r4[i].z - sy); Ez += lh * fabsf(r4[i].w - sz);
            Dmin = fminf(Dmin, r4[i].x); Dmax = fmaxf(Dmax, r4[i].x);
            Tx += wm * t4[i].y; Ty += wm * t4[i].z; Tz += wm * t4[i].w;
            Fx += wh * fabsf(t4[i].y); Fy += wh * fabsf(t4[i].z); Fz += wh * fabsf(t4[i].w);
        }
    }
    const float rest = 1.f - slm;
    Nx += rest * sx; Ny += rest * sy; Nz += rest * sz;
    bool dead = false;
    if (Dmin > 0.f) {
        const float id0 = 1.f / Dmin, id1 = 1.f / Dmax;
        DfIv3 U, Q;
        U.x = iv(fminf((Nx - Ex) * id0, (Nx - Ex) * id1), fmaxf((Nx + Ex) * id0, (Nx + Ex) * id1));
        U.y = iv(fminf((Ny - Ey) * id0, (Ny - Ey) * id1), fmaxf((Ny + Ey) * id0, (Ny + Ey) * id1));
        U.z = iv(fminf((Nz - Ez) * id0, (Nz - Ez) * id1), fmaxf((Nz + Ez) * id0, (Nz + Ez) * id1));
        const float umax = fmaxf(fmaxf(fmaxf(fabsf(U.x.lo), fabsf(U.x.hi)), fmaxf(fabsf(U.y.lo), fabsf(U.y.hi))), fmaxf(fabsf(U.z.lo), fabsf(U.z.hi)));
        const bool u_ok = umax < 1.0e3f;
        const int bx = (int)(blk % (size_t)nbx), by = (int)((blk / (size_t)nbx) % (size_t)nby), bz = (int)(blk / ((size_t)nbx * nby));
        const int x0 = bx * 8, y0 = by * 8, z0 = a.tab_z0 + bz * 8;
        const int x1 = min(x0 + 7, a.X - 1), y1 = min(y0 + 7, a.Y - 1), z1 = min(z0 + 7, a.Z - 1);
        const float cxv = 0.5f * (float)(x0 + x1) * a.vsx, cyv = 0.5f * (float)(y0 + y1) * a.vsy, czv = 0.5f * (float)(z0 + z1) * a.vsz;
        const float hxv = 0.5f * (float)(x1 - x0) * a.vsx, hyv = 0.5f * (float)(y1 - y0) * a.vsy, hzv = 0.5f * (float)(z1 - z0) * a.vsz;
        const f3 c = aff_mul(a.vol2world, mk3(cxv, cyv, czv));
        const float* M = a.vol2world.R;
        const float hx = fabsf(M[0]) * hxv + fabsf(M[1]) * hyv + fabsf(M[2]) * hzv, hy = fabsf(M[3]) * hxv + fabsf(M[4]) * hyv + fabsf(M[5]) * hzv,
                    hz = fabsf(M[6]) * hxv + fabsf(M[7]) * hyv + fabsf(M[8]) * hzv;
        Q.x = iv(c.x - hx, c.x + hx); Q.y = iv(c.y - hy, c.y + hy); Q.z = iv(c.z - hz, c.z + hz);
        const DfIv3 c1 = iv_cross(U, Q), c2 = iv_cross(U, c1);
        const DfIv ux2 = iv_sq(U.x), uy2 = iv_sq(U.y), uz2 = iv_sq(U.z);
        const DfIv S = iv(2.f / (1.f + (ux2.hi + uy2.hi + uz2.hi)), 2.f / (1.f + (ux2.lo + uy2.lo + uz2.lo)));
        DfIv3 P;
        P.x = iv_add(iv_add(Q.x, iv_mul(S, iv_add(c1.x, c2.x))), iv(Tx - Fx, Tx + Fx));
        P.y = iv_add(iv_add(Q.y, iv_mul(S, iv_add(c1.y, c2.y))), iv(Ty - Fy, Ty + Fy));
        P.z = iv_add(iv_add(Q.z, iv_mul(S, iv_add(c1.z, c2.z))), iv(Tz - Fz, Tz + Fz));
        const f3 pc = mk3(0.5f * (P.x.lo + P.x.hi), 0.5f * (P.y.lo + P.y.hi), 0.5f * (P.z.lo + P.z.hi));
        const float prx = 0.5f * (P.x.hi - P.x.lo), pry = 0.5f * (P.y.hi - P.y.lo), prz = 0.5f * (P.z.hi - P.z.lo);
        const f3 cc = aff_mul(a.world2cam, pc);
        const float* R = a.world2cam.R;
        const float mag = fabsf(pc.x) + fabsf(pc.y) + fabsf(pc.z) + fabsf(cc.x) + fabsf(cc.y) + fabsf(cc.z) + prx + pry + prz;
        const float infl = 1e-3f + 1e-5f * mag;
        const float rx = fabsf(R[0]) * prx + fabsf(R[1]) * pry + fabsf(R[2]) * prz + infl, ry = fabsf(R[3]) * prx + fabsf(R[4]) * pry + fabsf(R[5]) * prz + infl,
                    rz = fabsf(R[6]) * prx + fabsf(R[7]) * pry + fabsf(R[8]) * prz + infl;
        const float xl = cc.x - rx, xh = cc.x + rx, yl = cc.y - ry, yh = cc.y + ry, zl = cc.z - rz, zh = cc.z + rz;
        const bool ok = u_ok && mag < 1.0e15f;
        if (zh <= 0.f) dead = true;
        const float nx = (xl <= 0.f && xh >= 0.f) ? 0.f : fminf(fabsf(xl), fabsf(xh)), ny = (yl <= 0.f && yh >= 0.f) ? 0.f : fminf(fabsf(yl), fabsf(yh)),
                    nz = (zl <= 0.f && zh >= 0.f) ? 0.f : fminf(fabsf(zl), fabsf(zh));
        const float rmin = sqrtf(nx * nx + ny * ny + nz * nz) * 0.9999f;
        float max_dist;
        if (a.py.top != 0) { const uint32_t tb = df_pyramid_image_max(a.py); max_dist = tb < 0x7c00u ? h2f_bits((uint16_t)tb) : 3.0e38f; }
        else max_dist = a.cull[2];
        if (rmin > max_dist * 1.002f + a.P.trunc) dead = true;
        if (!dead && ok && zl > 0.05f) {
            const float il = 1.f / zl, ih = 1.f / zh;
            const float ulo = a.P.fx * fminf(xl * il, xl * ih) + a.P.cx - 2.f, uhi = a.P.fx * fmaxf(xh * il, xh * ih) + a.P.cx + 2.f;
            const float vlo = a.P.fy * fminf(yl * il, yl * ih) + a.P.cy - 2.f, vhi = a.P.fy * fmaxf(yh * il, yh * ih) + a.P.cy + 2.f;
            if (ulo == ulo && uhi == uhi && vlo == vlo && vhi == vhi) {
                if (uhi < 0.f || vhi < 0.f || ulo > (float)(a.P.cols - 1) || vlo > (float)(a.P.rows - 1)) dead = true;
                else if (a.py.top != 0) {
                    const int iu0 = (int)fmaxf(ulo, 0.f), iv0 = (int)fmaxf(vlo, 0.f);
                    const int iu1 = (int)fminf(uhi, (float)(a.P.cols - 1)), iv1 = (int)fminf(vhi, (float)(a.P.rows - 1));
                    const uint32_t dbits = df_pyramid_max_fine(a.py, iu0, iv0, iu1, iv1, 2);
                    if (dbits == 0u) dead = true;
                    else if (dbits < 0x7c00u && rmin > h2f_bits((uint16_t)dbits) * 1.002f + a.P.trunc) dead = true;
                }
            }
        }
        dead = dead && ok;
    }
    return dead;
}

#ifdef DF_TRACE_VERDICT
__device__ unsigned long long g_df_vtrace[8192 * 4];
#define DF_VT(i) do { if ((threadIdx.x & 63) == 0 && blockIdx.x * 4 + (threadIdx.x >> 6) < 8192) g_df_vtrace[(blockIdx.x * 4 + (threadIdx.x >> 6)) * 4 + (i)] = wall_clock64(); } while (0)
#else
#define DF_VT(i) do { } while (0)
#endif
__global__ __launch_bounds__(256) void df_block_verdict_kernel(const DfWarpedArgs a, const float4* __restrict__ rot, const float4* __restrict__ node_t,
                                                               int nbx, int nby, int nbz, uint8_t* __restrict__ blk_state,
                                                               const float* __restrict__ blk_wmax, const float* __restrict__ brick_d1, int vbx, int vby, int zero_skip, int use_models, int want_models,
                                                               int build_on_demand, const uint16_t* __restrict__ bm_idx,
                                                               const uint32_t* __restrict__ bm_lam, const uint32_t* __restrict__ bm_w,
                                                               const uint8_t* __restrict__ bm_cnt, const uint8_t* __restrict__ bm_coded, uint8_t* __restrict__ alive,
                                                               uint32_t* __restrict__ build_list, uint32_t* __restrict__ ahead_list, uint32_t* __restrict__ model_list,
                                                               uint32_t* __restrict__ cnt, uint32_t* __restrict__ cnt_next)
{
    const size_t nblk = (size_t)nbx * nby * nbz;
    const size_t blk = (size_t)blockIdx.x * 256 + threadIdx.x;
    DF_VT(0);
    if (blockIdx.x == 0 && threadIdx.x < 8) cnt_next[threadIdx.x] = 0u;
    bool keep = false, near = false, need_build = false, need_ahead = false, need_model = false;
    int bx = 0, by = 0, bz = 0;
    if (blk < nblk) {
        bx = (int)(blk % (size_t)nbx); by = (int)((blk / (size_t)nbx) % (size_t)nby); bz = (int)(blk / ((size_t)nbx * nby));
        const int x0 = bx * 8, y0 = by * 8, z0 = a.tab_z0 + bz * 8;
        const int own1 = min(a.z_own0 + a.z_own_n, a.Z);
        keep = x0 < a.X && y0 < a.Y && max(z0, a.z_own0) < min(z0 + 8, own1);
        const unsigned st = keep ? blk_state[blk] : 0u;
        if (keep) {
            float wk = a.kf;
            if (zero_skip && st >= 1u) {
                const float wmax = blk_wmax[blk];
                keep = !(wmax * a.cull[3] < DF_ZERO_WEIGHT);
                wk = fminf(wk, wmax * 1.0001f);
            } else if (zero_skip && a.cull[4] < 1.0e30f && a.cull[4] > 0.f) {
                const float dmin = fmaxf(brick_d1[((size_t)(a.tab_z0 / 8 + bz) * vby + by) * vbx + bx] - a.tile_r, 0.f) * 0.999f;
                const float sg = a.cull[4];
                const float wmax = a.kf * 1.001f * __expf(-(dmin * dmin) / (2.f * sg * sg) * 0.998f);
                keep = !(wmax * a.cull[3] < DF_ZERO_WEIGHT);
                wk = fminf(wk, wmax);
            }
            if (keep) {
                const f3 c = aff_mul(a.vol2world, mk3(((float)x0 + 3.5f) * a.vsx, ((float)y0 + 3.5f) * a.vsy, ((float)z0 + 3.5f) * a.vsz));
                if (a.pf_margin > 0.f && st < 2u) {
                    near = !df_tile_culled(a, c, wk, a.pf_margin);
                    keep = near && !df_tile_culled(a, c, wk);
                } else keep = !df_tile_culled(a, c, wk);
            }
        }
        DF_VT(1);
        if (keep && st == 2u && (use_models & 1)) {
            const unsigned n = bm_cnt[blk];
            if (n != DF_BM_NONE && a.cull[1] <= 1.0f) keep = !df_block_box_dead(a, rot, node_t, nbx, nby, nblk, blk, n, bm_idx, bm_lam, bm_w);
        }
        DF_VT(2);
        alive[blk] = keep ? (uint8_t)(1u | ((st == 2u && (use_models & 2) && bm_coded[blk] != 0) ? 2u : 0u)) : (uint8_t)0;
        need_build = keep && build_on_demand && st == 0u;
        need_ahead = !keep && near && build_on_demand && st == 0u;
        need_model = (keep || near) && want_models && (st == 1u || (need_build && want_models > 1));
        if (need_build) blk_state[blk] = 1;
    }
    const unsigned long long mb = __builtin_amdgcn_ballot_w64(need_build), ma = __builtin_amdgcn_ballot_w64(need_ahead), mm = __builtin_amdgcn_ballot_w64(need_model);
    const unsigned long long below = ((unsigned long long)1 << (threadIdx.x & 63)) - 1ull;
    const unsigned code = (unsigned)bx | ((unsigned)by << 10) | ((unsigned)(a.tab_z0 / 8 + bz) << 20);
    if (mb) {
        unsigned base = 0;
        if ((threadIdx.x & 63) == 0) base = atomicAdd(&cnt[0], (unsigned)__popcll(mb));
        base = (unsigned)__builtin_amdgcn_readfirstlane((int)base);
        if (need_build) build_list[base + (unsigned)__popcll(mb & below)] = code;
    }
    if (ma) {
        unsigned base = 0;
        if ((threadIdx.x & 63) == 0) base = atomicAdd(&cnt[3], (unsigned)__popcll(ma));
        base = (unsigned)__builtin_amdgcn_readfirstlane((int)base);
        const unsigned slot = base + (unsigned)__popcll(ma & below);
        if (need_ahead && slot < a.pf_cap) { ahead_list[slot] = code; blk_state[blk] = 1; }
    }
    if (mm) {
        unsigned base = 0;
        if ((threadIdx.x & 63) == 0) base = atomicAdd(&cnt[1], (unsigned)__popcll(mm));
        base = (unsigned)__builtin_amdgcn_readfirstlane((int)base);
        if (need_model) model_list[base + (unsigned)__popcll(mm & below)] = (unsigned)blk;
    }
    DF_VT(3);
}

__global__ __launch_bounds__(256) void df_blocks_unbuilt_kernel(int nbx, int nby, int nbz, int vbx, int vby, int tab_bz0, uint8_t* __restrict__ blk_state,
                                                                uint32_t* __restrict__ build_list, uint32_t* __restrict__ cnt,
                                                                uint32_t* __restrict__ cnt_next)
{
    const size_t nblk = (size_t)nbx * nby * nbz;
    const size_t blk = (size_t)blockIdx.x * 256 + threadIdx.x;
    if (blockIdx.x == 0 && threadIdx.x < 8) cnt_next[threadIdx.x] = 0u;
    bool need = false;
    int bx = 0, by = 0, bz = 0;
    if (blk < nblk) {
        bx = (int)(blk % (size_t)nbx); by = (int)((blk / (size_t)nbx) % (size_t)nby); bz = (int)(blk / ((size_t)nbx * nby));
        need = blk_state[blk] == 0 && bx < vbx && by < vby;
        if (blk_state[blk] == 0) blk_state[blk] = 1;
    }
    const unsigned long long m = __builtin_amdgcn_ballot_w64(need);
    if (m) {
        unsigned base = 0;
        if ((threadIdx.x & 63) == 0) base = atomicAdd(&cnt[0], (unsigned)__popcll(m));
        base = (unsigned)__builtin_amdgcn_readfirstlane((int)base);
        if (need) build_list[base + (unsigned)__popcll(m & (((unsigned long long)1 << (threadIdx.x & 63)) - 1ull))] =
                      (unsigned)bx | ((unsigned)by << 10) | ((unsigned)(tab_bz0 + bz) << 20);
    }
}
```

dynamicfusion_amd/csrc/dfusion_warp_pipe.h:

```cpp
#pragma once
#include "dfusion_warp_sweep.h"

template <int K> struct DfTabRaw;
template <> struct DfTabRaw<8> { uint4 idx; float4 w0, w1; unsigned code; };
template <> struct DfTabRaw<4> { uint2 idx; float4 w0; };
__device__ __forceinline__ void tab_raw_load(const DfWarpedArgs& a, size_t tv, DfTabRaw<8>& r)
{
    r.idx = reinterpret_cast<const uint4*>(a.knn_tab)[tv];
    r.w0 = reinterpret_cast<const float4*>(a.w_tab)[tv];
    r.w1 = reinterpret_cast<const float4*>(a.w_tab)[a.tab_nvox + tv];
}
__device__ __forceinline__ void tab_raw_load(const DfWarpedArgs& a, size_t tv, DfTabRaw<4>& r)
{
    r.idx = reinterpret_cast<const uint2*>(a.knn_tab)[tv];
    r.w0 = reinterpret_cast<const float4*>(a.w_tab)[tv];
}
typedef float df_v4f __attribute__((ext_vector_type(4)));
typedef unsigned int df_v4u __attribute__((ext_vector_type(4)));
typedef unsigned int df_v2u __attribute__((ext_vector_type(2)));
template <typename T> using df_global_ptr = __attribute__((address_space(1))) T*;
template <typename T>
__device__ __forceinline__ df_global_ptr<T> df_wave_uniform(T* p)
{
    const unsigned long long v = (unsigned long long)p;
    const unsigned lo = (unsigned)__builtin_amdgcn_readfirstlane((int)(unsigned)v), hi = (unsigned)__builtin_amdgcn_readfirstlane((int)(unsigned)(v >> 32));
    return (df_global_ptr<T>)(((unsigned long long)hi << 32) | lo);
}
#define DF_TAB_LD(p) __builtin_nontemporal_load(p)
__device__ __forceinline__ void tab_raw_load_at(const DfWarpedArgs& a, size_t rec, size_t rec_c, bool coded, unsigned lane, unsigned lane_c, DfTabRaw<8>& r)
{
    r.idx = make_uint4(0u, 0u, 0u, 0u); r.code = 0u;
    if (coded) {
        r.code = DF_TAB_LD(df_wave_uniform(a.code_tab + rec_c) + lane_c);
    } else {
        const df_v4u i4 = DF_TAB_LD(df_wave_uniform(reinterpret_cast<const df_v4u*>(a.knn_tab) + rec) + lane);
        r.idx = make_uint4(i4.x, i4.y, i4.z, i4.w);
    }
    const df_v4f a4 = DF_TAB_LD(df_wave_uniform(reinterpret_cast<const df_v4f*>(a.w_tab) + rec) + lane);
    const df_v4f b4 = DF_TAB_LD(df_wave_uniform(reinterpret_cast<const df_v4f*>(a.w_tab) + a.tab_nvox + rec) + lane);
    r.w0 = make_float4(a4.x, a4.y, a4.z, a4.w); r.w1 = make_float4(b4.x, b4.y, b4.z, b4.w);
}
__device__ __forceinline__ void tab_raw_load_at(const DfWarpedArgs& a, size_t rec, size_t, bool, unsigned lane, unsigned, DfTabRaw<4>& r)
{
    const df_v2u i2 = DF_TAB_LD(df_wave_uniform(reinterpret_cast<const df_v2u*>(a.knn_tab) + rec) + lane);
    const df_v4f a4 = DF_TAB_LD(df_wave_uniform(reinterpret_cast<const df_v4f*>(a.w_tab) + rec) + lane);
    r.idx = make_uint2(i2.x, i2.y); r.w0 = make_float4(a4.x, a4.y, a4.z, a4.w);
}
__device__ __forceinline__ void tab_raw_unpack(const DfTabRaw<8>& r, int (&bi)[8], float (&wt)[8])
{
    bi[0] = r.idx.x & 0xffff; bi[1] = r.idx.x >> 16; bi[2] = r.idx.y & 0xffff; bi[3] = r.idx.y >> 16;
    bi[4] = r.idx.z & 0xffff; bi[5] = r.idx.z >> 16; bi[6] = r.idx.w & 0xffff; bi[7] = r.idx.w >> 16;
    wt[0] = r.w0.x; wt[1] = r.w0.y; wt[2] = r.w0.z; wt[3] = r.w0.w; wt[4] = r.w1.x; wt[5] = r.w1.y; wt[6] = r.w1.z; wt[7] = r.w1.w;
}
__device__ __forceinline__ void tab_raw_unpack(const DfTabRaw<4>& r, int (&bi)[4], float (&wt)[4])
{
    bi[0] = r.idx.x & 0xffff; bi[1] = r.idx.x >> 16; bi[2] = r.idx.y & 0xffff; bi[3] = r.idx.y >> 16;
    wt[0] = r.w0.x; wt[1] = r.w0.y; wt[2] = r.w0.z; wt[3] = r.w0.w;
}
__device__ __forceinline__ unsigned df_node_off_lo(unsigned v)
{
    unsigned r;
    asm("v_lshlrev_b32_sdwa %0, 5, %1 dst_sel:DWORD dst_unused:UNUSED_PAD src0_sel:DWORD src1_sel:WORD_0" : "=v"(r) : "v"(v));
    return r;
}
__device__ __forceinline__ unsigned df_node_off_hi(unsigned v)
{
    unsigned r;
    asm("v_lshlrev_b32_sdwa %0, 5, %1 dst_sel:DWORD dst_unused:UNUSED_PAD src0_sel:DWORD src1_sel:WORD_1" : "=v"(r) : "v"(v));
    return r;
}
typedef const __attribute__((address_space(3))) df_v4f df_lds_cf4;
__device__ __forceinline__ df_v2f df_pk_mul_lo(df_v2f w, df_v2f q)
{
    df_v2f r;
    asm("v_pk_mul_f32 %0, %1, %2 op_sel_hi:[0,1]" : "=v"(r) : "v"(w), "v"(q));
    return r;
}
__device__ __forceinline__ df_v2f df_pk_mul_hi(df_v2f w, df_v2f q)
{
    df_v2f r;
    asm("v_pk_mul_f32 %0, %1, %2 op_sel:[1,0] op_sel_hi:[1,1]" : "=v"(r) : "v"(w), "v"(q));
    return r;
}
__device__ __forceinline__ void df_blend_acc(DfBlendSums& S, df_v2f wp, df_v4f r_lo, df_v4f t_lo, df_v4f r_hi, df_v4f t_hi)
{
    {
        const df_v2f ta = {t_lo.x, t_lo.y}, tb = {t_lo.z, t_lo.w}, ra = {r_lo.x, r_lo.y}, rb = {r_lo.z, r_lo.w};
        S.t01 = S.t01 + df_pk_mul_lo(wp, ta); S.t23 = S.t23 + df_pk_mul_lo(wp, tb);
        S.r01 = S.r01 + df_pk_mul_lo(wp, ra); S.r23 = S.r23 + df_pk_mul_lo(wp, rb);
    }
    {
        const df_v2f ta = {t_hi.x, t_hi.y}, tb = {t_hi.z, t_hi.w}, ra = {r_hi.x, r_hi.y}, rb = {r_hi.z, r_hi.w};
        S.t01 = S.t01 + df_pk_mul_hi(wp, ta); S.t23 = S.t23 + df_pk_mul_hi(wp, tb);
        S.r01 = S.r01 + df_pk_mul_hi(wp, ra); S.r23 = S.r23 + df_pk_mul_hi(wp, rb);
    }
}
__device__ __forceinline__ void df_blend_pair_at(DfBlendSums& S, unsigned off_lo, unsigned off_hi, df_v2f wp)
{
    df_lds_cf4* nl = (df_lds_cf4*)(size_t)off_lo; df_lds_cf4* nh = (df_lds_cf4*)(size_t)off_hi;
    df_blend_acc(S, wp, nl[0], nl[1], nh[0], nh[1]);
}
__device__ __forceinline__ DfBlendSums dqb_sums_lds_rec(const DfTabRaw<4>& r)
{
    DfBlendSums S;
    S.t01 = S.t23 = S.r01 = S.r23 = df_v2f{0.f, 0.f};
    df_blend_pair_at(S, df_node_off_lo(r.idx.x), df_node_off_hi(r.idx.x), df_v2f{r.w0.x, r.w0.y});
    df_blend_pair_at(S, df_node_off_lo(r.idx.y), df_node_off_hi(r.idx.y), df_v2f{r.w0.z, r.w0.w});
    return S;
}
__device__ __forceinline__ void df_blend_pair_global(DfBlendSums& S, df_global_ptr<const char> rt, unsigned idx2, df_v2f wp)
{
    const df_global_ptr<const df_v4f> nl = (df_global_ptr<const df_v4f>)(rt + df_node_off_lo(idx2));
    const df_global_ptr<const df_v4f> nh = (df_global_ptr<const df_v4f>)(rt + df_node_off_hi(idx2));
    df_blend_acc(S, wp, nl[0], nl[1], nh[0], nh[1]);
}
__device__ __forceinline__ DfBlendSums dqb_sums_global_rec(const DfTabRaw<8>& r, df_global_ptr<const char> rt)
{
    DfBlendSums S;
    S.t01 = S.t23 = S.r01 = S.r23 = df_v2f{0.f, 0.f};
    df_blend_pair_global(S, rt, r.idx.x, df_v2f{r.w0.x, r.w0.y}); df_blend_pair_global(S, rt, r.idx.y, df_v2f{r.w0.z, r.w0.w});
    df_blend_pair_global(S, rt, r.idx.z, df_v2f{r.w1.x, r.w1.y}); df_blend_pair_global(S, rt, r.idx.w, df_v2f{r.w1.z, r.w1.w});
    return S;
}
__device__ __forceinline__ DfBlendSums dqb_sums_global_rec(const DfTabRaw<4>& r, df_global_ptr<const char> rt)
{
    DfBlendSums S;
    S.t01 = S.t23 = S.r01 = S.r23 = df_v2f{0.f, 0.f};
    df_blend_pair_global(S, rt, r.idx.x, df_v2f{r.w0.x, r.w0.y}); df_blend_pair_global(S, rt, r.idx.y, df_v2f{r.w0.z, r.w0.w});
    return S;
}
__device__ __forceinline__ DfBlendSums dqb_sums_codes(const DfTabRaw<8>& r, unsigned lbase)
{
    DfBlendSums S;
    S.t01 = S.t23 = S.r01 = S.r23 = df_v2f{0.f, 0.f};
    const unsigned c = r.code;
#define DF_CODE_OFF(i) ((((i) == 0 ? (c << 5) : (i) == 1 ? (c << 1) : (c >> (4 * (i) - 5))) & 0x1e0u) | lbase)
    df_blend_pair_at(S, DF_CODE_OFF(0), DF_CODE_OFF(1), df_v2f{r.w0.x, r.w0.y}); df_blend_pair_at(S, DF_CODE_OFF(2), DF_CODE_OFF(3), df_v2f{r.w0.z, r.w0.w});
    df_blend_pair_at(S, DF_CODE_OFF(4), DF_CODE_OFF(5), df_v2f{r.w1.x, r.w1.y}); df_blend_pair_at(S, DF_CODE_OFF(6), DF_CODE_OFF(7), df_v2f{r.w1.z, r.w1.w});
#undef DF_CODE_OFF
    return S;
}

__device__ __forceinline__ unsigned df_lane_id() { return __builtin_amdgcn_mbcnt_hi(~0u, __builtin_amdgcn_mbcnt_lo(~0u, 0u)); }
__device__ __forceinline__ unsigned df_lane_id_here()
{
    unsigned r;
    asm volatile("v_mbcnt_lo_u32_b32 %0, -1, 0\n\tv_mbcnt_hi_u32_b32 %0, -1, %0" : "=v"(r));
    return r;
}
__device__ __forceinline__ __amdgpu_buffer_rsrc_t df_plane_rsrc(uint32_t* plane_ptr, unsigned bytes)
{
    return __builtin_amdgcn_make_buffer_rsrc((void*)df_wave_uniform(plane_ptr), (short)0, (int)bytes, 0x00020000);
}

#define DF_PLAN_BINS 65
#define DF_PLAN_WG 1024
__global__ __launch_bounds__(DF_PLAN_WG) void df_sweep_plan_kernel(const DfWarpedArgs a, int tiles_x, int tiles_y, unsigned n_items,
                                                                   unsigned long long* __restrict__ mask_out, unsigned int* __restrict__ cnt,
                                                                   unsigned int* __restrict__ bins, unsigned int* __restrict__ cnt_next,
                                                                   unsigned long long* __restrict__ code_out)
{
    __shared__ unsigned int s_cnt[DF_PLAN_BINS], s_base[DF_PLAN_BINS];
    if (threadIdx.x < DF_PLAN_BINS) { s_cnt[threadIdx.x] = 0u; if (blockIdx.x == 0) cnt_next[threadIdx.x] = 0u; }
    if (blockIdx.x == 0 && threadIdx.x < 2 && a.py.capped && a.cull) ((uint32_t*)a.cull)[6 + threadIdx.x] = 0u;
    if (blockIdx.x == 0 && threadIdx.x == 0 && a.host_report && a.blk_cnt) {
        a.host_report[0] = a.blk_cnt[0]; a.host_report[1] = a.blk_cnt[1]; a.host_report[2] = a.blk_cnt[3]; a.host_report[3] = a.sweep_no;
    }
    __syncthreads();
    const unsigned item = blockIdx.x * (DF_PLAN_WG / 64) + (threadIdx.x >> 6);
    const int ln = threadIdx.x & 63, p = ln >> 4, l = ln & 15;
    unsigned long long m = 0;
    if (item < n_items) {
        const unsigned half = item & 1u, tcol = item >> 1;
        const int tx = (int)(tcol % (unsigned)tiles_x), ty = (int)((tcol / (unsigned)tiles_x) % (unsigned)tiles_y);
        const int zb = (int)(tcol / ((unsigned)tiles_x * (unsigned)tiles_y));
        const int lt0 = a.bz0 + zb * a.zt;
        const int own1 = min(a.z_own0 + a.z_own_n, a.Z);
        const int x0 = tx * DF_ROW_TX + p * 8, y0 = ty * DF_LDS_TY + (int)half * 8;
        bool keep = l < a.zt && max((lt0 + l) * DF_ROW_TZ, a.z_own0) < min((lt0 + l + 1) * DF_ROW_TZ, own1) && x0 < a.X && y0 < a.Y;
        unsigned verdict = 1u;
        if (keep && a.blk_alive) {
            verdict = a.blk_alive[((size_t)(lt0 + l - a.tab_z0 / DF_ROW_TZ) * a.bm_nby + (unsigned)(y0 >> 3)) * a.bm_nbx + (unsigned)(x0 >> 3)];
            keep = verdict != 0u;
        }
        m = __builtin_amdgcn_ballot_w64(keep);
        if (code_out) {
            const bool coded = keep && a.blk_alive && (verdict & 2u) != 0u;
            const unsigned long long cm = __builtin_amdgcn_ballot_w64(coded);
            if (ln == 0 && m) code_out[item] = cm;
        }
        if (a.n_swept) {
            unsigned v = keep ? (unsigned)(64 * (min((lt0 + l + 1) * DF_ROW_TZ, own1) - max((lt0 + l) * DF_ROW_TZ, a.z_own0))) : 0u;
#pragma unroll
            for (int o = 32; o >= 1; o >>= 1) v += __shfl_xor(v, o, 64);
            if (ln == 0 && v) atomicAdd(a.n_swept, (unsigned long long)v);
        }
    }
    const unsigned w = (unsigned)__popcll(m);
    unsigned slot = 0;
    if (ln == 0 && m) slot = atomicAdd(&s_cnt[w], 1u);
    __syncthreads();
    if (threadIdx.x < DF_PLAN_BINS && s_cnt[threadIdx.x]) s_base[threadIdx.x] = atomicAdd(&cnt[threadIdx.x], s_cnt[threadIdx.x]);
    __syncthreads();
    if (ln == 0 && m) {
        mask_out[item] = m;
        bins[(size_t)w * n_items + s_base[w] + slot] = item;
    }
}

template <int K, int U, int WGT, bool V2W_IDENTITY, bool LDSN>
__global__ __launch_bounds__(WGT, LDSN ? (WGT == 512 ? 4 : 1) : (K == 8 ? 6 : 5)) void df_warp_rows_pipe_kernel(const DfWarpedArgs a, const DfWarpView W, int tiles_x)
{
    extern __shared__ __attribute__((aligned(16))) float4 s_lds[];
    constexpr bool CODES = !LDSN && K == 8;
    static_assert(!CODES || U == 1, "a coded batch lies in one half layer");
    constexpr unsigned SPW = WGT >= 256 ? WGT / 256 : 1;
    constexpr unsigned NW = WGT / 64;
    const int wave = __builtin_amdgcn_readfirstlane((int)(threadIdx.x >> 6));
    const unsigned group = blockIdx.x, share = (unsigned)wave;
    if ((unsigned)(size_t)(df_lds_cf4*)s_lds != 0u) __builtin_trap();
    if constexpr (LDSN) {
        for (int j = threadIdx.x; j < W.M; j += WGT) { s_lds[2 * j] = W.rot[j]; s_lds[2 * j + 1] = W.node_t[j]; }
        __syncthreads();
    }
    const df_global_ptr<const char> rt_g = (df_global_ptr<const char>)df_wave_uniform(reinterpret_cast<const char*>(W.rt));
    const size_t plane = (size_t)a.X * a.Y;
    const int own1 = min(a.z_own0 + a.z_own_n, a.Z);
    const unsigned pitch24 = (unsigned)a.P.pitch;
    unsigned int wave_upd = 0;
    const unsigned bin_cnt = a.plan_cnt[DF_PLAN_BINS - 1 - df_lane_id_here()];
    unsigned bin_end = bin_cnt;
#pragma unroll
    for (int o = 1; o < 64; o <<= 1) { const unsigned t = __shfl_up(bin_end, o, 64); if ((int)df_lane_id() >= o) bin_end += t; }
    const unsigned n_alive = (unsigned)__builtin_amdgcn_readlane((int)bin_end, 63);
    if (group * SPW >= n_alive) return;
#ifdef DF_TRACE_WG
    const unsigned long long t_start = wall_clock64();
    unsigned n_layers = 0;
#endif
    unsigned items_s[SPW]; unsigned long long masks_s[SPW];
    unsigned long long cmask_s[SPW];
    unsigned total2 = 0;
#pragma unroll
    for (unsigned s_ = 0; s_ < SPW; ++s_) {
        const unsigned sidx = group * SPW + s_;
        items_s[s_] = 0u; masks_s[s_] = 0ull;
        cmask_s[s_] = 0ull;
        if (sidx < n_alive) {
            const int j = __ffsll((unsigned long long)__builtin_amdgcn_ballot_w64(sidx < bin_end)) - 1;
            const unsigned r = sidx - ((unsigned)__builtin_amdgcn_readlane((int)bin_end, j) - (unsigned)__builtin_amdgcn_readlane((int)bin_cnt, j));
            items_s[s_] = (unsigned)__builtin_amdgcn_readfirstlane((int)a.plan_bins[(size_t)(DF_PLAN_BINS - 1 - j) * a.plan_items + r]);
            const unsigned long long m = a.plan_mask[items_s[s_]];
            masks_s[s_] = ((unsigned long long)(unsigned)__builtin_amdgcn_readfirstlane((int)(unsigned)(m >> 32)) << 32) |
                          (unsigned long long)(unsigned)__builtin_amdgcn_readfirstlane((int)(unsigned)m);
            total2 += 2u * (unsigned)__popcll(masks_s[s_]);
            if (CODES && a.plan_code) {
                const unsigned long long cm = a.plan_code[items_s[s_]];
                cmask_s[s_] = ((unsigned long long)(unsigned)__builtin_amdgcn_readfirstlane((int)(unsigned)(cm >> 32)) << 32) |
                              (unsigned long long)(unsigned)__builtin_amdgcn_readfirstlane((int)(unsigned)cm);
            }
        }
    }
    const unsigned c0 = total2 * share / NW, c1 = total2 * (share + 1u) / NW;
    unsigned pre = 0;
#pragma unroll 1
    for (unsigned q = 0; q < SPW * 4u; ++q) {
    unsigned item = items_s[0]; unsigned long long m_item = masks_s[0];
#pragma unroll
    for (unsigned s_ = 1; s_ < SPW; ++s_) if ((q >> 2) == s_) { item = items_s[s_]; m_item = masks_s[s_]; }
    const unsigned a16 = (unsigned)(m_item >> (16u * (q & 3u))) & 0xffffu;
    unsigned long long c_item = cmask_s[0];
#pragma unroll
    for (unsigned s_ = 1; s_ < SPW; ++s_) if ((q >> 2) == s_) c_item = cmask_s[s_];
    const unsigned cbits = CODES ? (unsigned)(c_item >> (16u * (q & 3u))) & 0xffffu : 0u;
    const unsigned n2 = 2u * (unsigned)__popc(a16);
    const unsigned seg_lo = max(c0, pre), seg_hi = min(c1, pre + n2);
    const unsigned pre0 = pre;
    pre += n2;
    if (seg_lo >= seg_hi) continue;
    const unsigned lo = seg_lo - pre0, hi = seg_hi - pre0;
    unsigned alive = a16;
    for (unsigned i = 0; i < (lo >> 1); ++i) alive &= alive - 1u;
    {
        unsigned keep = ((hi - 1u) >> 1) - (lo >> 1) + 1u, rest = alive, seg = 0u;
        for (unsigned i = 0; i < keep; ++i) { const unsigned low = rest & (0u - rest); seg |= low; rest ^= low; }
        alive = seg;
    }
    int first_l = __ffs(alive) - 1, last_l = 31 - __clz(alive);
    int z_first_off = (int)(lo & 1u) * (DF_ROW_TZ / 2), z_last_off = ((int)((hi - 1u) & 1u) + 1) * (DF_ROW_TZ / 2);
    const int wave_patch = (int)(q & 3u);
    const unsigned tcol = item >> 1;
    const int tx = (int)(tcol % (unsigned)tiles_x), ty = (int)((tcol / (unsigned)tiles_x) % (unsigned)a.plan_tiles_y);
    const int wv = (int)(item & 1u) * 4 + wave_patch;
    const int lnq = (int)df_lane_id_here();
    const int x = tx * DF_ROW_TX + (wv & 3) * 8 + (lnq & 7);
    const int y = ty * DF_LDS_TY + (wv >> 2) * 8 + (lnq >> 3);
    const bool in_xy = x < a.X && y < a.Y;
    const int xc = min(x, a.X - 1), yc = min(y, a.Y - 1);
    const float fxv = (float)x * a.vsx, fyv = (float)y * a.vsy;
    const int lt0 = a.bz0 + (int)(tcol / ((unsigned)tiles_x * (unsigned)a.plan_tiles_y)) * a.zt;
    auto layer_zb = [&](int l) { const int z = max((lt0 + l) * DF_ROW_TZ, a.z_own0); return l == first_l ? max(z, (lt0 + l) * DF_ROW_TZ + z_first_off) : z; };
    auto layer_ze = [&](int l) { const int z = min((lt0 + l + 1) * DF_ROW_TZ, own1); return l == last_l ? min(z, (lt0 + l) * DF_ROW_TZ + z_last_off) : z; };
    if (alive && layer_zb(first_l) >= layer_ze(first_l)) { alive &= alive - 1u; first_l = alive ? __ffs(alive) - 1 : 0; z_first_off = 0; }
    if (alive && layer_zb(last_l) >= layer_ze(last_l)) { alive &= ~(1u << last_l); last_l = alive ? 31 - __clz(alive) : 0; z_last_off = DF_ROW_TZ; }
    if (alive) {
        auto advance = [&](int l, int z0, int* nl, int* nz0) {
            *nl = l; *nz0 = z0 + U;
            if (*nz0 >= layer_ze(l)) {
                const unsigned rem = alive >> (l + 1);
                *nl = rem ? l + 1 + (__ffs(rem) - 1) : -1;
                *nz0 = *nl >= 0 ? layer_zb(*nl) : 0;
            }
        };
        const unsigned lane_vox4 = (unsigned)(yc * a.X + xc) * 4u;
        const unsigned plane_bytes = (unsigned)plane * 4u;
        const unsigned lane_tab = df_tab_in_plane(xc, yc);
        const size_t tile_col = (size_t)(yc / DF_TAB_TY) * a.tab_ntx + (size_t)(xc / DF_TAB_TX);
        const size_t tile_col_u = (size_t)__builtin_amdgcn_readfirstlane((int)tile_col);
        static_assert(DF_ROW_TZ == DF_TAB_TZ, "the sweep's layers are the tables' tile layers");
        const size_t rec_layer = (size_t)a.tab_nty * (size_t)a.tab_ntx * (DF_TAB_TX * DF_TAB_TY * DF_TAB_TZ);
        const size_t rec0 = ((size_t)(lt0 - a.tab_z0 / DF_TAB_TZ) * a.tab_nty * a.tab_ntx + tile_col_u) * (DF_TAB_TX * DF_TAB_TY * DF_TAB_TZ);
        const unsigned code_patch = ((unsigned)wv << 6);
        const unsigned lds_wave = (unsigned)wave * 4096u;
        const unsigned lq_base = lds_wave + ((((unsigned)xc >> 2) & 1u) | ((((unsigned)yc >> 2) & 1u) << 1)) * 512u;
        int loc_layer = -1;
        unsigned ids_nxt = 0u;
        const unsigned coded_alive = CODES ? (alive & cbits) : 0u;
        const unsigned blk_x = (unsigned)tx * (DF_ROW_TX / 8) + ((unsigned)wv & 3u), blk_y = (unsigned)ty * (DF_LDS_TY / 8) + ((unsigned)wv >> 2);
        auto lane_id = [&]() -> unsigned { return df_lane_id(); };
        auto ids_load = [&](int l) -> unsigned {
            const size_t blk = ((size_t)(unsigned)(lt0 + l - a.tab_z0 / DF_ROW_TZ) * (unsigned)a.bm_nby + blk_y) * (unsigned)a.bm_nbx + blk_x;
            return *((df_global_ptr<const uint32_t>)(a.bm_ids + blk * 64) + lane_id());
        };
        auto refill = [&](int l) {
            const unsigned ids = ids_nxt;
            const df_global_ptr<const df_v4f> n0 = (df_global_ptr<const df_v4f>)(rt_g + df_node_off_lo(ids));
            const df_global_ptr<const df_v4f> n1 = (df_global_ptr<const df_v4f>)(rt_g + df_node_off_hi(ids));
            const df_v4f r0 = n0[0], t0 = n0[1], r1 = n1[0], t1 = n1[1];
            __builtin_amdgcn_sched_barrier(0);
            const unsigned rem = coded_alive >> (l + 1);
            ids_nxt = ids_load(rem ? l + 1 + (__ffs(rem) - 1) : l);
            __builtin_amdgcn_sched_barrier(0);
            df_v4f* loc = (df_v4f*)((char*)s_lds + lds_wave + lane_id() * 32u);
            loc[0] = r0; loc[1] = t0; loc[128] = r1; loc[129] = t1;
            asm volatile("s_waitcnt lgkmcnt(0)" ::: "memory");
        };
        if (coded_alive) ids_nxt = ids_load(__ffs(coded_alive) - 1);
        auto load_batch = [&](DfTabRaw<K> (&S)[U], int l, int z0) {
#pragma unroll
            for (int u = 0; u < U; ++u) {
                const int zi = min(z0 + u, layer_ze(l) - 1) - (lt0 + l) * DF_ROW_TZ;
                const size_t rec = rec0 + (size_t)(unsigned)l * rec_layer + (size_t)(unsigned)(zi * (DF_TAB_TX * DF_TAB_TY));
                const bool coded_l = CODES && ((cbits >> l) & 1u) != 0u;
                tab_raw_load_at(a, rec, rec + code_patch, coded_l, lane_tab, lane_id(), S[u]);
            }
        };
        int l = __ffs(alive) - 1, z0 = layer_zb(l);
        int l1, z1; advance(l, z0, &l1, &z1);
        DfTabRaw<K> S0[U], S1[U];
        load_batch(S0, l, z0);
        load_batch(S1, l1 >= 0 ? l1 : l, l1 >= 0 ? z1 : z0);

        struct { float d2[U]; uint16_t dpb[U]; uint32_t vox[U]; int z[U]; } pend;
#pragma unroll
        for (int u = 0; u < U; ++u) { pend.d2[u] = 1.f; pend.dpb[u] = 0; pend.vox[u] = 0u; pend.z[u] = a.z_store0; }
        const float sat_t = df_sat_threshold(a.P.trunc);
        auto finish_pending = [&]() {
#pragma unroll
            for (int u = 0; u < U; ++u) {
                const float Dp = h2f_bits(pend.dpb[u]);
                const float d2 = pend.d2[u];
                const float sdf_a = Dp - __builtin_amdgcn_sqrtf(d2);
                const unsigned long long live_m = __builtin_amdgcn_ballot_w64(Dp != 0.f);
                const unsigned long long decided_m = __builtin_amdgcn_ballot_w64(fabsf(sdf_a) >= sat_t) & __builtin_amdgcn_ballot_w64(d2 <= 1024.f);
                bool upd; uint32_t out;
                if (a.sat_ok && (live_m & ~decided_m) == 0ull) {
                    const unsigned long long upd_m = live_m & __builtin_amdgcn_ballot_w64(sdf_a >= sat_t);
                    upd = (Dp != 0.f) & (sdf_a >= sat_t);
                    const unsigned long long one_m = __builtin_amdgcn_ballot_w64(pend.vox[u] == 0u) | __builtin_amdgcn_ballot_w64((pend.vox[u] & 0xffffu) == 0x3c00u);
                    if ((upd_m & ~one_m) == 0ull) out = tsdf_fuse_one(pend.vox[u], a.P.max_weight);
                    else out = tsdf_fuse(pend.vox[u], 1.f, a.P.max_weight);
                    wave_upd += (unsigned)__popcll(upd_m);
                } else {
                    float vn;
                    if (__builtin_expect(df_wave_all(df_sqrt_short_ok(d2)), 1)) vn = df_sqrt_short(d2);
                    else vn = sqrtf(d2);
                    const float sdf = Dp - vn;
                    upd = (Dp != 0.f) & (sdf >= -a.P.trunc);
                    out = tsdf_fuse(pend.vox[u], fminf(1.f, sdf * a.P.trunc_inv), a.P.max_weight);
                    wave_upd += (unsigned)__popcll(live_m & __builtin_amdgcn_ballot_w64(sdf >= -a.P.trunc));
                }
                if (upd) __builtin_amdgcn_raw_buffer_store_b32(out, df_plane_rsrc(a.vol + (size_t)(pend.z[u] - a.z_store0) * plane, plane_bytes), lane_vox4, 0, 0);
            }
        };
        auto step = [&](DfTabRaw<K> (&S)[U], int l, int z0, int l2, int z2) {
            const int ze = layer_ze(l);
            bool inz[U]; int zv[U];
#pragma unroll
            for (int u = 0; u < U; ++u) {
                inz[u] = in_xy && z0 + u < ze;
                zv[u] = min(z0 + u, ze - 1);
            }
            f3 vc[U]; bool ok[U]; uint16_t dpb[U];
            const bool coded = CODES && ((cbits >> l) & 1u) != 0u;
            if (CODES && coded && l != loc_layer) { refill(l); loc_layer = l; }
#pragma unroll
            for (int u = 0; u < U; ++u) {
                const f3 pv3 = mk3(fxv, fyv, (float)(z0 + u) * a.vsz);
                f3 q;
                if constexpr (V2W_IDENTITY) q = add3(pv3, mk3(a.vol2world.t[0], a.vol2world.t[1], a.vol2world.t[2]));
                else q = aff_mul(a.vol2world, pv3);
                DfBlendSums B;
                if constexpr (LDSN) B = dqb_sums_lds_rec(S[u]);
                else if constexpr (CODES) {
                    if (coded) B = dqb_sums_codes(S[u], lq_base | (((unsigned)(z0 + u) & 4u) << 9));
                    else B = dqb_sums_global_rec(S[u], rt_g);
                } else B = dqb_sums_global_rec(S[u], rt_g);
                quat rsum, rn; quat2 half;
                rsum.w = B.r01.x; rsum.x = B.r01.y; rsum.y = B.r23.x; rsum.z = B.r23.y;
                half.wx = B.t01 * 0.5f; half.yz = B.t23 * 0.5f;
                const float s1 = q_sumsq(rsum);
                float n1;
                if (__builtin_expect(df_wave_all(df_sqrt_short_ok(s1)), 1)) n1 = df_sqrt_short(s1);
                else n1 = sqrtf(s1);
                const quat rot = q_scale_f64(df_rcp_short((double)n1), rsum);
                const quat2 dual = q_mul_pk(half, q_pairs(rot));
                const float s2 = q_sumsq(rot);
                if (__builtin_expect(df_wave_all(q_near_unit_ok(s2)), 1)) rn = q_normalize_near_unit(rot, s2);
                else rn = q_normalize(rot);
                vc[u] = aff_mul(a.world2cam, dq_transform_rn_pk(rn, dual, q));
                const float pu = fmaf(a.P.fx, vc[u].x / vc[u].z, a.P.cx);
                const float pv = fmaf(a.P.fy, vc[u].y / vc[u].z, a.P.cy);
                ok[u] = inz[u] & (vc[u].z > 0.f) & (pu >= 0.f) & (pv >= 0.f) & (pu < (float)a.P.cols) & (pv < (float)a.P.rows);
                const int ui = (int)__builtin_amdgcn_fmed3f(pu, 0.f, (float)(a.P.cols - 1));
                const int vi = (int)__builtin_amdgcn_fmed3f(pv, 0.f, (float)(a.P.rows - 1));
                dpb[u] = *(const uint16_t*)((const char*)a.P.dists + (__umul24((unsigned)vi, pitch24) + 2u * (unsigned)ui));
            }
            finish_pending();
            __builtin_amdgcn_sched_barrier(0);
            load_batch(S, l2 >= 0 ? l2 : l, l2 >= 0 ? z2 : z0);
            __builtin_amdgcn_sched_barrier(0);
#pragma unroll
            for (int u = 0; u < U; ++u) {
                uint32_t vw = 0u;
                if (ok[u]) vw = __builtin_amdgcn_raw_buffer_load_b32(df_plane_rsrc(a.vol + (size_t)(zv[u] - a.z_store0) * plane, plane_bytes), lane_vox4, 0, 0);
                pend.d2[u] = dot3(vc[u], vc[u]); pend.dpb[u] = ok[u] ? dpb[u] : (uint16_t)0; pend.vox[u] = vw; pend.z[u] = zv[u];
            }
        };
        for (;;) {
            int l2, z2;
            if (l1 >= 0) advance(l1, z1, &l2, &z2); else { l2 = -1; z2 = 0; }
            step(S0, l, z0, l2, z2);
            if (l1 < 0) break;
            int l3, z3;
            if (l2 >= 0) advance(l2, z2, &l3, &z3); else { l3 = -1; z3 = 0; }
            step(S1, l1, z1, l3, z3);
            if (l2 < 0) break;
// ... 21 lines not shown
```

dynamicfusion_amd/csrc/dfusion_warp_sweep.h:

```cpp
#pragma once
#include "dfusion_internal.h"
#include "dfusion_pyramid.h"
#include "dfusion_warp_topk.h"

struct DfWarpedArgs {
    uint32_t* vol; int X, Y, Z;
    int z_store0, z_own0, z_own_n;
    int bz0;
    float vsx, vsy, vsz;
    DfAff vol2world, world2cam;
    DfIntegrateParams P;
    unsigned long long* n_upd;
    unsigned long long* n_swept;
    const float* cull;
    float kf;
    float tile_r;
    float cam_scale;
    float origin_cam;
    DfDistsPyramid py;
    uint16_t* knn_tab; float* w_tab; int tab_z0; size_t tab_nvox; int tab_ntx, tab_nty;
    int zt;
    int v2w_identity;
    int sat_ok;
    const unsigned long long* plan_mask; const unsigned int* plan_bins; const unsigned int* plan_cnt; unsigned int plan_items; int plan_tiles_y;
    const uint32_t* blk_cnt; uint32_t* host_report; uint32_t sweep_no;
#ifdef DF_TRACE_WG
    unsigned long long* trace;
#endif
    float* tile_wmax;
    const uint8_t* blk_alive; int bm_nbx, bm_nby;
    uint32_t* code_tab; uint32_t* bm_ids; uint8_t* bm_coded;
    const unsigned long long* plan_code;
    float* blk_wmax; const uint32_t* work; const uint32_t* work_cnt; uint32_t* work_cursor;
    float pf_margin;
    unsigned pf_cap;
    unsigned work_cap;
    uint8_t* blk_tie;
};
#define DF_ZERO_WEIGHT 1.3234890e-23f

#define DF_TAB_TX 32
#define DF_TAB_TY 16
#define DF_TAB_TZ 8
__device__ __forceinline__ unsigned df_tab_in_plane(int x, int y)
{
    const unsigned xt = (unsigned)x % DF_TAB_TX, yt = (unsigned)y % DF_TAB_TY;
    return yt * DF_TAB_TX + xt;
}
__device__ __forceinline__ size_t df_tab_index(const DfWarpedArgs& a, int x, int y, int z)
{
    const int zl = z - a.tab_z0;
    const size_t tile = ((size_t)(zl / DF_TAB_TZ) * a.tab_nty + (y / DF_TAB_TY)) * a.tab_ntx + (x / DF_TAB_TX);
    return tile * (DF_TAB_TX * DF_TAB_TY * DF_TAB_TZ) + (size_t)(zl % DF_TAB_TZ) * (DF_TAB_TX * DF_TAB_TY) + df_tab_in_plane(x, y);
}

__device__ __forceinline__ unsigned df_code_in_plane(int x, int y)
{
    const unsigned xt = (unsigned)x % DF_TAB_TX, yt = (unsigned)y % DF_TAB_TY;
    return (((yt >> 3) * (DF_TAB_TX / 8) + (xt >> 3)) << 6) + ((yt & 7u) << 3) + (xt & 7u);
}
__device__ __forceinline__ size_t df_code_index(const DfWarpedArgs& a, int x, int y, int z)
{
    const int zl = z - a.tab_z0;
    const size_t tile = ((size_t)(zl / DF_TAB_TZ) * a.tab_nty + (y / DF_TAB_TY)) * a.tab_ntx + (x / DF_TAB_TX);
    return tile * (DF_TAB_TX * DF_TAB_TY * DF_TAB_TZ) + (size_t)(zl % DF_TAB_TZ) * (DF_TAB_TX * DF_TAB_TY) + df_code_in_plane(x, y);
}

#define DF_CAND_CHUNK 256

template <int K>
__device__ __forceinline__ void knn_tab_store(uint16_t* tab, size_t voxel, const int (&bi)[K])
{
    if constexpr (K == 8) {
        uint4 v;
        v.x = (uint32_t)bi[0] | ((uint32_t)bi[1] << 16); v.y = (uint32_t)bi[2] | ((uint32_t)bi[3] << 16);
        v.z = (uint32_t)bi[4] | ((uint32_t)bi[5] << 16); v.w = (uint32_t)bi[6] | ((uint32_t)bi[7] << 16);
        reinterpret_cast<uint4*>(tab)[voxel] = v;
    } else if constexpr (K == 4) {
        uint2 v;
        v.x = (uint32_t)bi[0] | ((uint32_t)bi[1] << 16); v.y = (uint32_t)bi[2] | ((uint32_t)bi[3] << 16);
        reinterpret_cast<uint2*>(tab)[voxel] = v;
    } else {
#pragma unroll
        for (int i = 0; i < K; ++i) tab[voxel * K + i] = (uint16_t)bi[i];
    }
}
template <int K>
__device__ __forceinline__ void knn_tab_load(const uint16_t* tab, size_t voxel, int (&bi)[K])
{
    if constexpr (K == 8) {
        const uint4 v = reinterpret_cast<const uint4*>(tab)[voxel];
        bi[0] = v.x & 0xffff; bi[1] = v.x >> 16; bi[2] = v.y & 0xffff; bi[3] = v.y >> 16;
        bi[4] = v.z & 0xffff; bi[5] = v.z >> 16; bi[6] = v.w & 0xffff; bi[7] = v.w >> 16;
    } else if constexpr (K == 4) {
        const uint2 v = reinterpret_cast<const uint2*>(tab)[voxel];
        bi[0] = v.x & 0xffff; bi[1] = v.x >> 16; bi[2] = v.y & 0xffff; bi[3] = v.y >> 16;
    } else {
#pragma unroll
        for (int i = 0; i < K; ++i) bi[i] = tab[voxel * K + i];
    }
}
template <int K>
__device__ __forceinline__ void w_tab_store(float* tab, size_t nvox, size_t voxel, const float (&wt)[K])
{
    if constexpr (K % 4 == 0) {
#pragma unroll
        for (int i = 0; i < K / 4; ++i)
            reinterpret_cast<float4*>(tab)[(size_t)i * nvox + voxel] = make_float4(wt[4 * i], wt[4 * i + 1], wt[4 * i + 2], wt[4 * i + 3]);
    } else {
#pragma unroll
        for (int i = 0; i < K; ++i) tab[(size_t)i * nvox + voxel] = wt[i];
    }
}
template <int K>
__device__ __forceinline__ void w_tab_load(const float* tab, size_t nvox, size_t voxel, float (&wt)[K])
{
    if constexpr (K % 4 == 0) {
#pragma unroll
        for (int i = 0; i < K / 4; ++i) {
            const float4 v = reinterpret_cast<const float4*>(tab)[(size_t)i * nvox + voxel];
            wt[4 * i] = v.x; wt[4 * i + 1] = v.y; wt[4 * i + 2] = v.z; wt[4 * i + 3] = v.w;
        }
    } else {
#pragma unroll
        for (int i = 0; i < K; ++i) wt[i] = tab[(size_t)i * nvox + voxel];
    }
}

__device__ __forceinline__ bool df_tile_culled(const DfWarpedArgs& a, f3 c, float wk, float extra = 0.f)
{
    const float max_t = a.cull[0], sin_half = a.cull[1];
    if (!(sin_half <= 1.0f && max_t < 1.0e30f)) return false;
    float max_dist;
    if (a.py.top != 0) { const uint32_t tb = df_pyramid_image_max(a.py); max_dist = tb < 0x7c00u ? h2f_bits((uint16_t)tb) : 3.0e38f; }
    else max_dist = a.cull[2];
    const float cn = sqrtf(dot3(c, c));
    const float delta = 2.f * sin_half * (cn + a.tile_r) + wk * max_t;
    const float rho = a.cam_scale * (a.tile_r + delta + extra) * 1.002f + 1e-3f;
    const float rho_r = a.origin_cam >= 0.f ? fminf(rho, (a.tile_r + 2.f * sin_half * a.origin_cam + wk * max_t + extra) * 1.002f + 1e-3f) : rho;
    const f3 cc = aff_mul(a.world2cam, c);
    const float rmin = sqrtf(dot3(cc, cc)) - rho_r;
    bool out = false;
    if (cc.z + rho <= 0.f) out = true;
    if (rmin > max_dist * 1.002f + a.P.trunc) out = true;
    const float nl = sqrtf(a.P.fx * a.P.fx + a.P.cx * a.P.cx);
    if ((a.P.fx * cc.x + a.P.cx * cc.z) / nl < -rho) out = true;
    const float cr = (float)a.P.cols - a.P.cx;
    const float nr = sqrtf(a.P.fx * a.P.fx + cr * cr);
    if ((-a.P.fx * cc.x + cr * cc.z) / nr < -rho) out = true;
    const float nt = sqrtf(a.P.fy * a.P.fy + a.P.cy * a.P.cy);
    if ((a.P.fy * cc.y + a.P.cy * cc.z) / nt < -rho) out = true;
    const float cb = (float)a.P.rows - a.P.cy;
    const float nbt = sqrtf(a.P.fy * a.P.fy + cb * cb);
    if ((-a.P.fy * cc.y + cb * cc.z) / nbt < -rho) out = true;
    const float zl = cc.z - rho, zh = cc.z + rho;
    if (!out && a.py.top != 0 && zl > 0.05f) {
        const float il = 1.f / zl, ih = 1.f / zh;
        const float xl = cc.x - rho, xh = cc.x + rho, yl = cc.y - rho, yh = cc.y + rho;
        const float ulo = a.P.fx * fminf(xl * il, xl * ih) + a.P.cx - 2.f, uhi = a.P.fx * fmaxf(xh * il, xh * ih) + a.P.cx + 2.f;
        const float vlo = a.P.fy * fminf(yl * il, yl * ih) + a.P.cy - 2.f, vhi = a.P.fy * fmaxf(yh * il, yh * ih) + a.P.cy + 2.f;
        if (ulo == ulo && uhi == uhi && vlo == vlo && vhi == vhi) {
            if (uhi < 0.f || vhi < 0.f || ulo > (float)(a.P.cols - 1) || vlo > (float)(a.P.rows - 1)) out = true;
            else {
                const int iu0 = (int)fmaxf(ulo, 0.f), iv0 = (int)fmaxf(vlo, 0.f);
                const int iu1 = (int)fminf(uhi, (float)(a.P.cols - 1)), iv1 = (int)fminf(vhi, (float)(a.P.rows - 1));
                const uint32_t dbits = df_pyramid_max_fine(a.py, iu0, iv0, iu1, iv1, 2);
                if (dbits == 0u) out = true;
                else if (dbits < 0x7c00u && rmin > h2f_bits((uint16_t)dbits) * 1.002f + a.P.trunc) out = true;
            }
        }
    }
    return out;
}

template <int K>
__device__ __forceinline__ unsigned int df_warp_update(const DfWarpedArgs& a, const DfWarpView& W, f3 q, const float (&wt)[K],
                                                       const int (&bi)[K], uint32_t* vox)
{
    quat rot, dual;
    dqb_blend_w<K>(W, wt, bi, &rot, &dual);
    const f3 vc = aff_mul(a.world2cam, dq_transform(rot, dual, q));
    float ts;
    if (!tsdf_sample(a.P, vc, &ts)) return 0u;
    *vox = tsdf_fuse(*vox, ts, a.P.max_weight);
    return 1u;
// ... 262 lines not shown
```

dynamicfusion_amd/tsdf_volume.py:

```python
import ctypes as C

import numpy as np
import torch

from . import capi
from .synth import aff12, affine_inv, affine_mul

F32 = np.float32


def _stream():
    return C.c_void_p(torch.cuda.current_stream().cuda_stream)


def _ptr(t):
    return C.c_void_p(t.data_ptr())


U16 = (torch.int16, None, 2, 2)
F4 = (torch.float32, 4, 4, 16)
BGRA = (torch.uint8, 4, 1, 4)


def _image(t, kind, check_device=True):
# ... 35 lines not shown


def upload_u16(arr, device="cuda"):
    return torch.from_numpy(np.ascontiguousarray(arr).view(np.int16)).to(device)


def download_u16(t):
    return t.detach().cpu().numpy().view(np.uint16)


def compute_dists(depth, intr, dists=None):
    dp, dpitch, rows, cols = _image(depth, U16)
    if dists is None:
        dists = torch.empty((rows, cols), dtype=torch.int16, device=depth.device)
    op, opitch, orows, ocols = _image(dists, U16)
    if (orows, ocols) != (rows, cols):
        raise ValueError("dists %s does not match depth %s" % ((orows, ocols), (rows, cols)))
    capi.check(capi.lib().dfusion_compute_dists(dp, dpitch, op, opitch, cols, rows,
                                                intr.as_proj(), _stream()), "dfusion_compute_dists")
    return dists


class TsdfVolume:

    def __init__(self, dims, device="cuda", slab=None, allocate=True):
        self.trunc_dist_ = float(F32(0.03))
        self.max_weight_ = 128
        self.size_ = np.full(3, 3.0, F32)
        self.pose_ = np.eye(4, dtype=F32)
        self.gradient_delta_factor_ = 0.75
        self.raycast_step_factor_ = 0.75
        self.device = torch.device(device)
        self.slab_ = slab
        self.data_ = None
        self.allocate_ = allocate
        self.create(dims)

    def create(self, dims):
        self.dims_ = tuple(int(d) for d in dims)
        X, Y, Z = self.dims_
        if X % 4:
            raise ValueError("dims[0] must be a multiple of 4 (reference asserts % 32, kinfu.cpp:97)")
        if self.slab_ is None:
            self.z_store0, self.z_store_n, self.z_own0, self.z_own_n = 0, Z, 0, Z
        else:
            z_own0, z_own_n, halo = self.slab_
            lo, hi = max(0, z_own0 - halo), min(Z, z_own0 + z_own_n + halo)
            self.z_store0, self.z_store_n, self.z_own0, self.z_own_n = lo, hi - lo, z_own0, z_own_n
        self.setTruncDist(self.trunc_dist_)
        if self.allocate_:
            self.data_ = torch.empty((self.z_store_n, Y, X), dtype=torch.int32, device=self.device)
            self.clear()

    def owning_stored_planes(self):
        import copy
        v = copy.copy(self)
        v.slab_ = (self.z_store0, self.z_store_n, 0)
        v.z_own0, v.z_own_n = self.z_store0, self.z_store_n
        return v

    def getDims(self):
        return self.dims_

    def getVoxelSize(self):
        return np.array([F32(self.size_[i]) / F32(self.dims_[i]) for i in range(3)], F32)

    def data(self):
        return self.data_

    def getSize(self):
        return self.size_.copy()

    def setSize(self, size):
        self.size_ = np.asarray(size, F32).reshape(3).copy()
        self.setTruncDist(self.trunc_dist_)

    def getTruncDist(self):
        return self.trunc_dist_

    def setTruncDist(self, distance):
        vsz = self.getVoxelSize()
        max_coeff = max(vsz[0], vsz[1], vsz[2])
        self.trunc_dist_ = float(max(F32(distance), F32(2.1) * F32(max_coeff)))

    def getMaxWeight(self):
        return int(self.max_weight_)

    def setMaxWeight(self, weight):
        self.max_weight_ = weight

    def getPose(self):
        return self.pose_.copy()

    def setPose(self, pose):
        self.pose_ = np.asarray(pose, F32).reshape(4, 4).copy()

    def getRaycastStepFactor(self):
        return self.raycast_step_factor_

    def setRaycastStepFactor(self, factor):
        self.raycast_step_factor_ = float(factor)

    def getGradientDeltaFactor(self):
        return self.gradient_delta_factor_

    def setGradientDeltaFactor(self, factor):
        self.gradient_delta_factor_ = float(factor)

    def swap(self, data):
        self.data_, other = data, self.data_
        return other

    def applyAffine(self, affine):
        self.pose_ = affine_mul(np.asarray(affine, F32), self.pose_)

    def c_volume(self):
        if self.data_ is None:
            raise capi.DfusionError("TsdfVolume has no device blob (allocate=False)")
        v = capi.DfVolume()
        v.data = self.data_.data_ptr()
        v.dims[:] = self.dims_
        v.voxel_size[:] = [float(x) for x in self.getVoxelSize()]
        v.trunc_dist = self.trunc_dist_
        v.max_weight = int(self.max_weight_)
        return v

    def c_slab(self):
        if self.slab_ is None:
            return None
        return C.byref(capi.DfSlab(self.z_store0, self.z_store_n, self.z_own0, self.z_own_n))

    def clear(self):
        capi.check(capi.lib().dfusion_clear(self.c_volume(), self.c_slab(), _stream()), "dfusion_clear")

    def integrate(self, dists, camera_pose, intr, n_updated=None, sync=True, flags=0, n_swept=None):
        vol2cam = affine_mul(affine_inv(np.asarray(camera_pose, F32)), self.pose_)
        dp, pitch, rows, cols = _image(dists, U16)
        if flags == 0 and n_swept is None:
            capi.check(capi.lib().dfusion_integrate(dp, pitch, cols, rows, self.c_volume(), self.c_slab(),
                                                    capi.floats(aff12(vol2cam)), intr.as_proj(),
                                                    _ptr(n_updated) if n_updated is not None else None, _stream()),
                       "dfusion_integrate")
        else:
            capi.check(capi.lib().dfusion_integrate_ex(dp, pitch, cols, rows, self.c_volume(), self.c_slab(),
                                                       capi.floats(aff12(vol2cam)), intr.as_proj(), int(flags),
                                                       _ptr(n_updated) if n_updated is not None else None,
                                                       _ptr(n_swept) if n_swept is not None else None, _stream()),
                       "dfusion_integrate_ex")
        if sync:
            torch.cuda.current_stream().synchronize()

    def integrate_warped(self, dists, camera_pose, intr, warp_field, k=None, n_updated=None, cull=True, sync=True,
                         use_table=True, use_weights=True, use_lds=True, pipelined=True, zero_skip=True, depth_pyramid=True, block_model=True,
                         prefetch=True, codes=True):
        k = warp_field.k if k is None else k
        world2cam = affine_mul(affine_inv(np.asarray(camera_pose, F32)), warp_field.warp_to_live_)
        warp_field.ensure_index(self, k)
        dp, pitch, rows, cols = _image(dists, U16)
        capi.check(capi.lib().dfusion_integrate_warped(
            dp, pitch, cols, rows, self.c_volume(), self.c_slab(), capi.floats(aff12(self.pose_)),
            capi.floats(aff12(world2cam)), intr.as_proj(), warp_field.handle, k,
            (0 if cull else capi.DF_WARP_NO_CULL) | (0 if use_table else capi.DF_WARP_NO_TABLE) |
            (0 if use_weights else capi.DF_WARP_NO_WEIGHT_TABLE) | (0 if use_lds else capi.DF_WARP_NO_LDS) |
            (0 if pipelined else capi.DF_WARP_NO_PIPELINE) | (0 if zero_skip else capi.DF_WARP_NO_ZERO_SKIP) |
            (0 if depth_pyramid else capi.DF_WARP_NO_DEPTH_PYRAMID) | (capi.DF_WARP_STEADY_PREFETCH if prefetch == "steady" else 0 if prefetch else capi.DF_WARP_NO_PREFETCH) |
            (0 if codes else capi.DF_WARP_NO_CODES) |
            (capi.DF_WARP_BLOCK_MODEL_NOW if block_model == "now" else 0 if block_model else capi.DF_WARP_NO_BLOCK_MODEL),
            _ptr(n_updated) if n_updated is not None else None, _stream()), "dfusion_integrate_warped")
        if sync:
            torch.cuda.current_stream().synchronize()

    def integrate_warped_prepare(self, dists, camera_pose, intr, warp_field, k=None, prefetch=True, block_model=True, codes=True):
        k = warp_field.k if k is None else k
        world2cam = affine_mul(affine_inv(np.asarray(camera_pose, F32)), warp_field.warp_to_live_)
        warp_field.ensure_index(self, k)
        dp, pitch, rows, cols = _image(dists, U16)
        capi.check(capi.lib().dfusion_integrate_warped_prepare(
            dp, pitch, cols, rows, self.c_volume(), self.c_slab(), capi.floats(aff12(self.pose_)),
            capi.floats(aff12(world2cam)), intr.as_proj(), warp_field.handle, k,
            (capi.DF_WARP_STEADY_PREFETCH if prefetch == "steady" else 0 if prefetch else capi.DF_WARP_NO_PREFETCH) |
            (0 if codes else capi.DF_WARP_NO_CODES) |
            (capi.DF_WARP_BLOCK_MODEL_NOW if block_model == "now" else 0 if block_model else capi.DF_WARP_NO_BLOCK_MODEL),
            _stream()), "dfusion_integrate_warped_prepare")

    def integrate_warped_sweep(self, warp_field, n_updated=None, sync=False):
        capi.check(capi.lib().dfusion_integrate_warped_sweep(self.c_volume(), self.c_slab(), warp_field.handle,
                                                             _ptr(n_updated) if n_updated is not None else None, _stream()),
                   "dfusion_integrate_warped_sweep")
        if sync:
            torch.cuda.current_stream().synchronize()

    @staticmethod
    def _same_size(img, rows, cols):
        if img[2:] != (rows, cols):
            raise ValueError("image is %dx%d, expected %dx%d" % (img[2], img[3], rows, cols))
        return img[0], img[1]

    def _raycast_args(self, camera_pose):
        cam2vol = affine_mul(affine_inv(self.pose_), np.asarray(camera_pose, F32))
        Rinv = np.linalg.inv(cam2vol[:3, :3].astype(np.float64)).astype(F32)
        return capi.floats(aff12(cam2vol)), capi.floats(Rinv.reshape(-1))

    def raycast(self, camera_pose, intr, points, normals, keys=None):
        aff, Rinv = self._raycast_args(camera_pose)
        np_, npitch, rows, cols = _image(normals, F4)
        L = capi.lib()
        if points.dtype == torch.float32:
            pp, ppitch = self._same_size(_image(points, F4), rows, cols)
            capi.check(L.dfusion_raycast_points(self.c_volume(), self.c_slab(), aff, Rinv, intr.as_reproj(), pp,
                                                ppitch, np_, npitch, cols, rows,
                                                self.raycast_step_factor_, self.gradient_delta_factor_,
                                                _flat(keys) if keys is not None else None, _stream()),
                       "dfusion_raycast_points")
        else:
            dp, dpitch = self._same_size(_image(points, U16), rows, cols)
            capi.check(L.dfusion_raycast_depth(self.c_volume(), self.c_slab(), aff, Rinv, intr.as_reproj(), dp,
                                               dpitch, np_, npitch, cols, rows,
                                               self.raycast_step_factor_, self.gradient_delta_factor_, _stream()),
                       "dfusion_raycast_depth")

    def raycast_march(self, camera_pose, intr, keys64, rank=0):
        aff, _ = self._raycast_args(camera_pose)
        rows, cols = keys64.shape
        capi.check(capi.lib().dfusion_raycast_march(self.c_volume(), self.c_slab(), aff, intr.as_reproj(), cols, rows,
                                                    self.raycast_step_factor_, int(rank), _flat(keys64), _stream()),
                   "dfusion_raycast_march")
        return keys64

    def raycast_shade(self, camera_pose, intr, merged_keys64, points, normals):
        aff, Rinv = self._raycast_args(camera_pose)
        rows, cols = merged_keys64.shape
        np_, npitch = self._same_size(_image(normals, F4), rows, cols)
        pp, ppitch = self._same_size(_image(points, F4), rows, cols) if points is not None else (None, npitch)
        capi.check(capi.lib().dfusion_raycast_shade(self.c_volume(), self.c_slab(), aff, Rinv, intr.as_reproj(),
                                                    _flat(merged_keys64), pp, ppitch,
                                                    np_, npitch, cols, rows, self.gradient_delta_factor_,
                                                    _stream()), "dfusion_raycast_shade")
        return points, normals

    def raycast_points_of_keys(self, camera_pose, intr, merged_keys64, normals, points, row0=0, nrows=None):
        aff, Rinv = self._raycast_args(camera_pose)
        rows, cols = merged_keys64.shape
        nrows = rows - row0 if nrows is None else nrows
        np_, npitch = self._same_size(_image(normals, F4), nrows, cols)
        pp, ppitch = self._same_size(_image(points, F4), nrows, cols)
        capi.check(capi.lib().dfusion_raycast_points_of_keys_rows(aff, Rinv, intr.as_reproj(), _flat(merged_keys64), np_, npitch,
                                                                  pp, ppitch, cols, rows, int(row0), int(nrows), _stream()),
                   "dfusion_raycast_points_of_keys_rows")
        return points

    def fetchCloud(self, cloud_buffer=None):
        if cloud_buffer is None:
            cap = min(256 * 256 * 256, int(np.prod(self.dims_)))
            cloud_buffer = torch.empty((cap, 4), dtype=torch.float32, device=self.device)
        count = torch.zeros(1, dtype=torch.int64, device=self.device)
        capi.check(capi.lib().dfusion_extract_cloud(self.c_volume(), self.c_slab(), capi.floats(aff12(self.pose_)),
                                                    _ptr(cloud_buffer), cloud_buffer.shape[0], _ptr(count), _stream()),
                   "dfusion_extract_cloud")
        n = int(count.item())
        self.last_cloud_count_ = n
        return cloud_buffer[:min(n, cloud_buffer.shape[0])]

    def fetchNormals(self, cloud, normals=None):
        n = int(cloud.shape[0])
        if normals is None:
            normals = torch.empty((n, 4), dtype=torch.float32, device=self.device)
        Rinv = np.linalg.inv(self.pose_[:3, :3].astype(np.float64)).astype(F32)
        capi.check(capi.lib().dfusion_extract_normals(self.c_volume(), self.c_slab(), capi.floats(aff12(self.pose_)),
                                                      capi.floats(Rinv.reshape(-1)), _ptr(cloud), n,
                                                      self.gradient_delta_factor_, _ptr(normals), _stream()),
                   "dfusion_extract_normals")
        return normals

    def fetchMesh(self, with_normals=False):
        aff = capi.floats(aff12(self.pose_))
        counts = torch.empty(2, dtype=torch.int64, device=self.device)
        capi.check(capi.lib().dfusion_extract_mesh(self.c_volume(), self.c_slab(), aff, None, 0, None, 0, _ptr(counts), _stream()),
                   "dfusion_extract_mesh")
        nv, nt = (int(c) for c in counts.tolist())
        self.last_mesh_counts_ = (nv, nt)
        vertices = torch.empty((nv, 4), dtype=torch.float32, device=self.device)
        triangles = torch.empty((nt, 3), dtype=torch.int32, device=self.device)
        if nv or nt:
            capi.check(capi.lib().dfusion_extract_mesh(self.c_volume(), self.c_slab(), aff, _ptr(vertices) if nv else None, nv,
                                                       _ptr(triangles) if nt else None, nt, _ptr(counts), _stream()),
                       "dfusion_extract_mesh")
        if with_normals:
            return vertices, triangles, self.fetchNormals(vertices)
        return vertices, triangles

    def psdf(self, warped, dists, intr, return_points=False):
        n = int(warped.shape[0])
        pts = torch.zeros((n, 4), dtype=torch.float32, device=self.device)
        pts[:, :3] = warped[:, :3]
        ro = torch.empty(n, dtype=torch.float32, device=self.device)
        op, opitch, rows, cols = _image(dists, U16)
        snapshot = dists.clone(memory_format=torch.contiguous_format)
        ip, ipitch, _, _ = _image(snapshot, U16)
        capi.check(capi.lib().dfusion_project_and_remove(ip, ipitch, op, opitch, cols, rows,
                                                         _flat(pts), n, intr.as_proj(), _ptr(ro), None, _stream()),
                   "dfusion_project_and_remove")
        return (ro, pts) if return_points else ro

    def download(self):
        return self.data_.detach().cpu().numpy().view(np.uint32)

    def upload(self, arr_u32):
        self.data_.copy_(torch.from_numpy(np.ascontiguousarray(arr_u32).view(np.int32)).reshape(self.data_.shape))
```

include/dfusion.h:

```cpp
#ifndef DFUSION_H
#define DFUSION_H

#include <stddef.h>
#include <stdint.h>

#ifdef __cplusplus
extern "C" {
#endif

#define DFUSION_ABI_VERSION 7

typedef void *dfStream;

typedef struct DfVolume {
    void *data;
    int dims[3];
    float voxel_size[3];
    float trunc_dist;
    int max_weight;
} DfVolume;

typedef struct DfSlab {
    int z_store0, z_store_n;
    int z_own0, z_own_n;
} DfSlab;

typedef struct DfWarpField DfWarpField;

enum {
    DF_OK = 0,
    DF_E_INVALID = 100001,
    DF_E_NO_INDEX = 100002,
    DF_E_NO_DEVICE = 100003
};

#define DF_WARP_NO_CULL 1u
#define DF_WARP_NO_TABLE 2u
#define DF_WARP_NO_WEIGHT_TABLE 4u
#define DF_WARP_NO_LDS 8u
#define DF_WARP_NO_PIPELINE 16u
#define DF_WARP_NO_ZERO_SKIP 32u
#define DF_WARP_NO_DEPTH_PYRAMID 64u
#define DF_WARP_NO_BLOCK_MODEL 128u
#define DF_WARP_BLOCK_MODEL_NOW 256u
#define DF_WARP_NO_PREFETCH 512u
#define DF_WARP_NO_CODES 2048u
#define DF_WARP_STEADY_PREFETCH 1024u
#define DF_INDEX_VOXEL_TABLE 1u
#define DF_INDEX_WEIGHT_TABLE 2u
#define DF_INDEX_TABLES_ON_DEMAND 4u

int dfusion_abi_version(void);
const char *dfusion_error_string(int err);

int dfusion_clear(DfVolume v, const DfSlab *slab, dfStream stream);

int dfusion_compute_dists(const uint16_t *depth_dev, size_t depth_pitch, uint16_t *dists_dev, size_t dists_pitch,
                          int cols, int rows, const float intr[4], dfStream stream);

int dfusion_project_and_remove(const uint16_t *dists_in_dev, size_t in_pitch, uint16_t *dists_out_dev, size_t out_pitch,
                               int cols, int rows, float *points_dev, unsigned long long n, const float proj[4],
                               float *ro_dev, unsigned long long *n_inside_dev, dfStream stream);

int dfusion_integrate(const uint16_t *dists_dev, size_t dists_pitch, int cols, int rows, DfVolume v,
                      const DfSlab *slab, const float vol2cam[12], const float proj[4],
                      unsigned long long *n_updated_dev, dfStream stream);

#define DF_RIGID_NO_DEPTH_CULL 1u
#define DF_RIGID_NO_SHORT_FORMS 2u
#define DF_RIGID_KEEP_ALL 4u
#define DF_RIGID_NO_SAT 8u
#define DF_RIGID_POISON_SCRATCH 16u
int dfusion_integrate_ex(const uint16_t *dists_dev, size_t dists_pitch, int cols, int rows, DfVolume v,
                         const DfSlab *slab, const float vol2cam[12], const float proj[4], unsigned flags,
                         unsigned long long *n_updated_dev, unsigned long long *n_swept_dev, dfStream stream);

int dfusion_release_scratch(void);

int dfusion_raycast_points(DfVolume v, const DfSlab *slab, const float cam2vol[12], const float Rinv[9],
                           const float reproj[4], float *points_dev, size_t points_pitch, float *normals_dev,
                           size_t normals_pitch, int cols, int rows, float step_factor, float delta_factor,
                           uint32_t *keys_dev, dfStream stream);

int dfusion_raycast_depth(DfVolume v, const DfSlab *slab, const float cam2vol[12], const float Rinv[9],
                          const float reproj[4], uint16_t *depth_dev, size_t depth_pitch, float *normals_dev,
                          size_t normals_pitch, int cols, int rows, float step_factor, float delta_factor,
                          dfStream stream);

#define DF_RC_KEY_NONE 0x7fffffffffffffffull
#define DF_RC_KEY_MAX_RANK 127u
int dfusion_raycast_march(DfVolume v, const DfSlab *slab, const float cam2vol[12], const float reproj[4], int cols,
                          int rows, float step_factor, unsigned int rank_tag, unsigned long long *keys64_dev,
                          dfStream stream);
int dfusion_raycast_shade(DfVolume v, const DfSlab *slab, const float cam2vol[12], const float Rinv[9],
                          const float reproj[4], const unsigned long long *merged_keys64_dev,
                          float *points_dev, size_t points_pitch, float *normals_dev, size_t normals_pitch, int cols,
                          int rows, float delta_factor, dfStream stream);
int dfusion_raycast_points_of_keys(const float cam2vol[12], const float Rinv[9], const float reproj[4],
                                   const unsigned long long *merged_keys64_dev, const float *normals_dev, size_t normals_pitch,
                                   float *points_dev, size_t points_pitch, int cols, int rows, dfStream stream);
int dfusion_raycast_points_of_keys_rows(const float cam2vol[12], const float Rinv[9], const float reproj[4],
                                        const unsigned long long *merged_keys64_dev, const float *normals_dev, size_t normals_pitch,
                                        float *points_dev, size_t points_pitch, int cols, int image_rows, int row0, int rows,
                                        dfStream stream);

int dfusion_raycast_sum_pieces(const uint32_t *pieces_dev, int n_pieces, unsigned long long n_words, uint32_t *out_dev, dfStream stream);

int dfusion_raycast_min_pieces(const unsigned long long *pieces_dev, int n_pieces, unsigned long long n_keys, unsigned long long *out_dev, dfStream stream);

int dfusion_extract_cloud(DfVolume v, const DfSlab *slab, const float aff[12], float *points_dev,
                          unsigned long long capacity, unsigned long long *count_dev, dfStream stream);
int dfusion_extract_normals(DfVolume v, const DfSlab *slab, const float aff[12], const float Rinv[9],
                            const float *points_dev, unsigned long long n, float gradient_delta_factor,
                            float *normals_dev, dfStream stream);

int dfusion_extract_mesh(DfVolume v, const DfSlab *slab, const float aff[12], float *vertices_dev,
                         unsigned long long vertex_capacity, unsigned int *triangles_dev,
                         unsigned long long triangle_capacity, unsigned long long *counts_dev, dfStream stream);

int dfusion_warp_create(DfWarpField **out);
int dfusion_warp_destroy(DfWarpField *wf);

int dfusion_warp_set_nodes(DfWarpField *wf, const float *pos_dev, const float *dq_dev, const float *sigma_dev,
                           int M, dfStream stream);

int dfusion_warp_set_transforms(DfWarpField *wf, const float *dq_dev, dfStream stream);

int dfusion_warp_build_index(DfWarpField *wf, DfVolume geometry, const DfSlab *slab, const float vol2world[12], int k,
                             unsigned flags, dfStream stream);

int dfusion_warp_extend(DfWarpField *wf, int k, const float *points_dev, int N, float radius, float sigma_new, int max_new,
                        float *new_pos_dev, float *new_dq_dev, float *new_sigma_dev, int *n_added, int *n_winners, dfStream stream);

int dfusion_warp_index_info(const DfWarpField *wf, unsigned long long *total_entries, unsigned int *n_bricks, int *k_built);

int dfusion_warp_set_point_tiling(DfWarpField *wf, int image_cols);

int dfusion_selftest_exact_forms(unsigned long long n_random, unsigned long long *counts_dev, dfStream stream);

int dfusion_warp_debug_counters(DfWarpField *wf, unsigned long long *swept_dev);

int dfusion_warp_alive_blocks(DfWarpField *wf, int z0, int zn, unsigned long long *per_layer_dev, int n_layers, dfStream stream);
int dfusion_warp_coded_blocks(DfWarpField *wf, int z0, int zn, unsigned long long *per_layer_dev, int n_layers, dfStream stream);

int dfusion_knn(DfWarpField *wf, int k, const float *queries_dev, int N, int *idx_dev, float *d2_dev, dfStream stream);

int dfusion_warp_points(DfWarpField *wf, int k, float *points_dev, float *normals_dev, int N,
                        const float warp_to_live[12], dfStream stream);

int dfusion_warp_solve_data_term(DfWarpField *wf, int k, const float *canonical_dev, const float *live_dev, int N, int iters,
                                 float lambda, float *dq_out_dev, float *energy_dev, dfStream stream);

int dfusion_warp_solve(DfWarpField *wf, int k, const float *canonical_dev, const float *live_dev, int N, int iters, float lambda,
                       int kg, float lambda_reg, float *dq_out_dev, float *energy_dev, dfStream stream);
int dfusion_warp_solve_robust(DfWarpField *wf, int k, const float *canonical_dev, const float *live_dev, int N, int iters, float lambda,
                              int kg, float lambda_reg, int rounds, float tukey_c, float huber_delta, float *dq_out_dev,
                              float *energy_dev, float *point_weights_dev, float *edge_weights_dev, dfStream stream);
int dfusion_warp_solve_plane(DfWarpField *wf, int k, const float *canonical_dev, const float *live_dev, const float *normals_dev, int N,
                             int iters, float lambda, int kg, float lambda_reg, int rounds, float tukey_c, float huber_delta,
                             float *dq_out_dev, float *energy_dev, float *point_weights_dev, float *edge_weights_dev, dfStream stream);
int dfusion_warp_node_graph(DfWarpField *wf, int kg, int *nbr_dev, float *alpha_dev, dfStream stream);

int dfusion_integrate_warped(const uint16_t *dists_dev, size_t dists_pitch, int cols, int rows, DfVolume v,
                             const DfSlab *slab, const float vol2world[12], const float world2cam[12],
                             const float proj[4], DfWarpField *wf, int k, unsigned flags,
                             unsigned long long *n_updated_dev, dfStream stream);

int dfusion_integrate_warped_prepare(const uint16_t *dists_dev, size_t dists_pitch, int cols, int rows, DfVolume geometry,
                                     const DfSlab *slab, const float vol2world[12], const float world2cam[12], const float proj[4],
                                     DfWarpField *wf, int k, unsigned flags, dfStream stream);
int dfusion_integrate_warped_sweep(DfVolume v, const DfSlab *slab, DfWarpField *wf, unsigned long long *n_updated_dev, dfStream stream);



int dfusion_bilateral_filter(const uint16_t *src_dev, size_t src_pitch, uint16_t *dst_dev, size_t dst_pitch, int cols, int rows,
                             int kernel_size, float sigma_spatial, float sigma_depth, dfStream stream);
int dfusion_truncate_depth(uint16_t *depth_dev, size_t pitch, int cols, int rows, float max_dist, dfStream stream);
int dfusion_cloud_to_depth(const float *points_dev, size_t points_pitch, uint16_t *depth_dev, size_t depth_pitch, int cols, int rows, dfStream stream);
int dfusion_depth_pyramid(const uint16_t *src_dev, size_t src_pitch, int src_cols, int src_rows, uint16_t *dst_dev, size_t dst_pitch,
                          float sigma_depth, dfStream stream);
int dfusion_compute_normals_mask_depth(uint16_t *depth_dev, size_t depth_pitch, float *normals_dev, size_t normals_pitch, int cols,
                                       int rows, const float intr[4], dfStream stream);
int dfusion_compute_point_normals(const uint16_t *depth_dev, size_t depth_pitch, float *points_dev, size_t points_pitch,
                                  float *normals_dev, size_t normals_pitch, int cols, int rows, const float intr[4], dfStream stream);
int dfusion_resize_depth_normals(const uint16_t *depth_dev, size_t depth_pitch, const float *normals_dev, size_t normals_pitch,
                                 int src_cols, int src_rows, uint16_t *depth_out_dev, size_t depth_out_pitch, float *normals_out_dev,
                                 size_t normals_out_pitch, dfStream stream);
int dfusion_resize_points_normals(const float *points_dev, size_t points_pitch, const float *normals_dev, size_t normals_pitch,
                                  int src_cols, int src_rows, float *points_out_dev, size_t points_out_pitch, float *normals_out_dev,
                                  size_t normals_out_pitch, dfStream stream);

int dfusion_render_image_points(const float *points_dev, size_t points_pitch, const float *normals_dev, size_t normals_pitch, int cols,
                                int rows, const float light_pose[3], unsigned char *image_dev, size_t image_pitch, dfStream stream);
int dfusion_render_image_depth(const uint16_t *depth_dev, size_t depth_pitch, const float *normals_dev, size_t normals_pitch, int cols,
                               int rows, const float intr[4], const float light_pose[3], unsigned char *image_dev, size_t image_pitch,
                               dfStream stream);
int dfusion_render_tangent_colors(const float *normals_dev, size_t normals_pitch, int cols, int rows, unsigned char *image_dev,
                                  size_t image_pitch, dfStream stream);

// ... 34 lines not shown
```

Baseline: 1896.

## Add per-half sub-block verdicts to cull dead z-halves in warped sweep

Block model building now also records per-half, per-quadrant lambda and weight bounds for each node. A new sub-verdict kernel uses these to decide which 4-plane halves of each block are alive. The plan mask widens to two bits per layer, so the sweep can skip dead half-layers instead of only whole layers. This adds extra buffers, an extra kernel launch, and more shuffles during model build, in exchange for less voxel work in the sweep.

```diff
diff --git a/dynamicfusion_amd/build.py b/dynamicfusion_amd/build.py
--- a/dynamicfusion_amd/build.py
+++ b/dynamicfusion_amd/build.py
@@ -11,7 +11,7 @@
 SOURCES = ["dfusion_volume.hip", "dfusion_warp.hip", "dfusion_warp_nodes.hip", "dfusion_warp_points.hip", "dfusion_warp_index.hip",
            "dfusion_raycast.hip", "dfusion_frontend.hip", "dfusion_solver.hip", "dfusion_selftest.hip", "dfusion_warp_extend.hip", "dfusion_mesh.hip", "dfusion_associate.hip"]
 HEADERS = ["dfusion_device.h", "dfusion_internal.h", "dfusion_nanoflann.h", "dfusion_pyramid.h", "dfusion_warp_topk.h", "dfusion_warp_sweep.h",
-           "dfusion_warp_blocks.h", "dfusion_warp_pipe.h", os.path.join(REPO_DIR, "include", "dfusion.h")]
+           "dfusion_warp_blocks.h", "dfusion_warp_pipe.h", "dfusion_plan_halves.h", os.path.join(REPO_DIR, "include", "dfusion.h")]
 
 HIPCC_FLAGS = ["--offload-arch=gfx950", "-O3", "-std=c++17", "-ffp-contract=off", "-fPIC", "-shared",
                "-fno-fast-math", "-Wno-unused-result"]
@@ -48,7 +48,7 @@
     f = ("dfusion_warp_nodes.hip" if k.startswith(("df_pack", "df_node"))
          else "dfusion_warp_points.hip" if k.startswith("df_points")
          else "dfusion_warp_index.hip" if k.startswith(("df_brick", "df_scan", "df_grow"))
-         else "dfusion_warp.hip" if k.startswith(("df_warp", "df_sweep", "df_block", "df_blocks", "df_dists_max", "df_alive"))
+         else "dfusion_warp.hip" if k.startswith(("df_warp", "df_sweep", "df_block", "df_blocks", "df_sub", "df_dists_max", "df_alive"))
          else "dfusion_raycast.hip" if k.startswith(("df_raycast", "df_extract"))
          else "dfusion_solver.hip" if k.startswith("df_sv")
          else "dfusion_mesh.hip" if k.startswith("df_mesh")
diff --git a/dynamicfusion_amd/capi.py b/dynamicfusion_amd/capi.py
--- a/dynamicfusion_amd/capi.py
+++ b/dynamicfusion_amd/capi.py
@@ -33,6 +33,7 @@
 DF_WARP_NO_PREFETCH = 512
 DF_WARP_STEADY_PREFETCH = 1024
 DF_WARP_NO_CODES = 2048
+DF_WARP_NO_SUB_VERDICT = 4096
 DF_RIGID_NO_DEPTH_CULL = 1
 DF_RIGID_NO_SHORT_FORMS = 2
 DF_RIGID_KEEP_ALL = 4
diff --git a/dynamicfusion_amd/csrc/dfusion_internal.h b/dynamicfusion_amd/csrc/dfusion_internal.h
--- a/dynamicfusion_amd/csrc/dfusion_internal.h
+++ b/dynamicfusion_amd/csrc/dfusion_internal.h
@@ -109,6 +109,7 @@
     DfDevBuf<uint8_t> blk_tie;
     DfDevBuf<uint16_t> bm_idx; DfDevBuf<uint32_t> bm_lam, bm_w; DfDevBuf<uint8_t> bm_cnt; size_t bm_cap = 0;
     DfDevBuf<uint32_t> code_tab; size_t code_cap = 0; DfDevBuf<uint32_t> bm_ids; DfDevBuf<uint8_t> bm_coded;
+    DfDevBuf<uint32_t> bm_sub_lam, bm_sub_w; DfDevBuf<uint16_t> bm_sub_cnt; DfDevBuf<uint8_t> bm_sub_ok, blk_sub, blk_alive_prev; DfDevBuf<uint32_t> sub_list;
     bool tab_complete = false;
     int tab_sweeps = 0;
     unsigned long long* dbg_swept = nullptr;
diff --git a/dynamicfusion_amd/csrc/dfusion_plan_halves.h b/dynamicfusion_amd/csrc/dfusion_plan_halves.h
--- /dev/null
+++ b/dynamicfusion_amd/csrc/dfusion_plan_halves.h
@@ -0,0 +1,36 @@
+#pragma once
+#include <stdint.h>
+#if defined(__HIPCC__) || defined(__CUDACC__)
+#define DF_HD __host__ __device__ __forceinline__
+#else
+#define DF_HD static inline
+#endif
+
+DF_HD uint32_t df_spread16(uint32_t x)
+{
+    x &= 0xffffu;
+    x = (x | (x << 8)) & 0x00ff00ffu; x = (x | (x << 4)) & 0x0f0f0f0fu; x = (x | (x << 2)) & 0x33333333u; x = (x | (x << 1)) & 0x55555555u;
+    return x;
+}
+DF_HD uint32_t df_unspread16(uint32_t x)
+{
+    x &= 0x55555555u;
+    x = (x | (x >> 1)) & 0x33333333u; x = (x | (x >> 2)) & 0x0f0f0f0fu; x = (x | (x >> 4)) & 0x00ff00ffu; x = (x | (x >> 8)) & 0x0000ffffu;
+    return x;
+}
+DF_HD uint32_t df_halves_word(uint32_t lower16, uint32_t upper16) { return df_spread16(lower16) | (df_spread16(upper16) << 1); }
+DF_HD uint32_t df_halves_layers(uint32_t hw) { return df_unspread16(hw | (hw >> 1)); }
+DF_HD uint32_t df_halves_segment(uint32_t hw, unsigned lo, unsigned hi)
+{
+    for (unsigned i = 0; i < lo; ++i) hw &= hw - 1u;
+    uint32_t seg = 0u;
+    for (unsigned i = lo; i < hi; ++i) { const uint32_t low = hw & (0u - hw); seg |= low; hw ^= low; }
+    return seg;
+}
+DF_HD int df_halves_z0(uint32_t seg, int l) { return ((seg >> (2 * l)) & 1u) ? 0 : 4; }
+DF_HD int df_halves_z1(uint32_t seg, int l) { return ((seg >> (2 * l + 1)) & 1u) ? 8 : 4; }
+DF_HD int df_half_planes(int zl, int h, int own0, int own1)
+{
+    const int a = zl + 4 * h > own0 ? zl + 4 * h : own0, b = zl + 4 * h + 4 < own1 ? zl + 4 * h + 4 : own1;
+    return b > a ? b - a : 0;
+}
diff --git a/dynamicfusion_amd/csrc/dfusion_warp.hip b/dynamicfusion_amd/csrc/dfusion_warp.hip
--- a/dynamicfusion_amd/csrc/dfusion_warp.hip
+++ b/dynamicfusion_amd/csrc/dfusion_warp.hip
@@ -3,6 +3,7 @@
 #include "dfusion_warp_sweep.h"
 #include "dfusion_warp_blocks.h"
 #include "dfusion_warp_pipe.h"
+#include <algorithm>
 #include <atomic>
 #include <stdlib.h>
 #include <stdio.h>
@@ -99,6 +100,9 @@
     a.bz0 = wf->tab_z0 / DF_BRICK;
     a.bm_nbx = ntx * (DF_TAB_TX / 8); a.bm_nby = nty * (DF_TAB_TY / 8);
     a.code_tab = wf->code_tab; a.bm_ids = wf->bm_ids; a.bm_coded = wf->bm_coded;
+    if (wf->bm_sub_lam && wf->bm_sub_w && wf->bm_sub_cnt && wf->bm_sub_ok) {
+        a.bm_sub_lam = wf->bm_sub_lam; a.bm_sub_w = wf->bm_sub_w; a.bm_sub_cnt = wf->bm_sub_cnt; a.bm_sub_ok = wf->bm_sub_ok;
+    }
     a.blk_tie = wf->blk_tie;
     return a;
 }
@@ -173,12 +177,20 @@
         { int rc = wf->bm_cnt.reserve(nblk); if (rc) return rc; }
         wf->bm_cap = nblk;
     }
-    if (want_models && k == 8 && (nblk * 512 > wf->code_cap || !wf->bm_ids || !wf->code_tab || !wf->bm_coded)) {
+    if (want_models && k == 8 && (nblk * 512 > wf->code_cap || !wf->bm_ids || !wf->code_tab || !wf->bm_coded || !wf->bm_sub_lam || !wf->bm_sub_w ||
+                                  !wf->bm_sub_cnt || !wf->bm_sub_ok || !wf->blk_sub || !wf->sub_list)) {
         wf->code_cap = 0;
         { int rc = wf->bm_ids.reserve(nblk * 64); if (rc) return rc; }
         { int rc = wf->code_tab.reserve(nblk * 512); if (rc) return rc; }
         { int rc = wf->bm_coded.reserve(nblk); if (rc) return rc; }
         DF_HIP(hipMemsetAsync(wf->bm_coded, 0, nblk, st));
+        { int rc = wf->bm_sub_lam.reserve(nblk * 8 * DF_BM_NU); if (rc) return rc; }
+        { int rc = wf->bm_sub_w.reserve(nblk * 8 * DF_BM_NU); if (rc) return rc; }
+        { int rc = wf->bm_sub_cnt.reserve(nblk * 8); if (rc) return rc; }
+        { int rc = wf->bm_sub_ok.reserve(nblk); if (rc) return rc; }
+        { int rc = wf->blk_sub.reserve(nblk); if (rc) return rc; }
+        { int rc = wf->sub_list.reserve(nblk); if (rc) return rc; }
+        DF_HIP(hipMemsetAsync(wf->bm_sub_ok, 0, nblk, st));
         wf->code_cap = nblk * 512;
     }
     bool ahead = !(flags & (DF_WARP_NO_PREFETCH | DF_WARP_BLOCK_MODEL_NOW));
@@ -193,12 +205,17 @@
     uint32_t* cnt = wf->blk_cnt + 8 * wf->blk_phase;
     uint32_t* cnt_next = wf->blk_cnt + 8 * (wf->blk_phase ^ 1);
     uint32_t* list_urgent = wf->blk_work, *list_ahead = wf->blk_work + wf->blk_cap, *list_model = wf->blk_work + 2 * wf->blk_cap;
+    std::swap(wf->blk_alive, wf->blk_alive_prev);
+    const bool codes_exist = k == 8 && wf->bm_cnt && wf->code_tab && wf->bm_ids && wf->bm_coded && wf->code_cap >= nblk * 512;
+    const bool sub_verdicts = use_models && wf->bm_cap >= nblk && codes_exist && !(flags & DF_WARP_NO_SUB_VERDICT) && wf->bm_sub_lam && wf->bm_sub_w &&
+                              wf->bm_sub_cnt && wf->bm_sub_ok && wf->blk_sub && wf->sub_list && wf->blk_alive_prev;
+    if (sub_verdicts) { a.bm_ids = wf->bm_ids; a.bm_sub_lam = wf->bm_sub_lam; a.bm_sub_w = wf->bm_sub_w; a.bm_sub_cnt = wf->bm_sub_cnt; a.bm_sub_ok = wf->bm_sub_ok; }
     hipLaunchKernelGGL(df_block_verdict_kernel, dim3((unsigned)((nblk + 255) / 256)), dim3(256), 0, st, a, wf->rot, wf->node_t, nbx, nby, nbz,
                        wf->blk_state, wf->blk_wmax, wf->brick_thr + wf->off_cap, wf->bx, wf->by, a.tile_wmax != nullptr ? 1 : 0,
-                       (use_models && wf->bm_cap >= nblk ? 1 : 0) | (k == 8 && wf->bm_cnt && wf->code_tab && wf->bm_ids && wf->bm_coded && wf->code_cap >= nblk * 512 ? 2 : 0),
+                       (use_models && wf->bm_cap >= nblk ? 1 : 0) | (codes_exist ? 2 : 0) | (sub_verdicts ? 4 : 0),
                        want_models_now,
                        wf->tab_complete ? 0 : 1, wf->bm_idx, wf->bm_lam, wf->bm_w, wf->bm_cnt, wf->bm_coded, wf->blk_alive, list_urgent, list_ahead, list_model,
-                       cnt, cnt_next);
+                       cnt, cnt_next, sub_verdicts ? (uint8_t*)wf->blk_sub : nullptr, wf->sub_list, wf->blk_alive_prev);
     a.blk_cnt = cnt; a.host_report = (uint32_t*)wf->host_report; a.sweep_no = (uint32_t)wf->tab_sweeps;
     DF_LAUNCH_CHECK();
 #ifdef DF_TRACE_VERDICT
@@ -234,6 +251,12 @@
         if (hipEventRecord(wf->ev_join, wf->side) == hipSuccess) wf->side_pending = true;
         else { (void)hipGetLastError(); df_side_drain(wf); if (rc_side == DF_OK) rc_side = (int)hipErrorUnknown; }
         if (rc_side != DF_OK) return rc_side;
+    }
+    if (sub_verdicts) {
+        const unsigned sub_grid = (unsigned)std::min<size_t>((nblk * 8 + 255) / 256, 1024);
+        hipLaunchKernelGGL(df_sub_verdict_kernel, dim3(sub_grid), dim3(256), 0, st, a, wf->rot, wf->node_t, nbx, nby, nbz, wf->sub_list, cnt + 5, wf->blk_sub);
+        DF_LAUNCH_CHECK();
+        a.blk_sub = wf->blk_sub;
     }
     if (!wf->tab_complete) { int rc = df_build_listed(wf, cnt, st, 0); if (rc) return rc; }
     if (want_models_now && !ahead) { int rc = launch_models(st); if (rc) return rc; }
@@ -429,7 +452,7 @@
                 { int rc = df_wait_all_sweeps_host(wf); if (rc) return rc; }
                 wf->plan_cap = 0;
                 for (int i = 0; i < 2; ++i) {
-                    { int rc = wf->plan_mask2[i].reserve(n_items); if (rc) return rc; }
+                    { int rc = wf->plan_mask2[i].reserve((size_t)n_items * 2); if (rc) return rc; }
                     { int rc = wf->plan_list2[i].reserve((size_t)n_items * DF_PLAN_BINS); if (rc) return rc; }
                     { int rc = wf->plan_code2[i].reserve(n_items); if (rc) return rc; }
                 }
@@ -543,6 +566,7 @@
         { int rc = wf->blk_tie.reserve(nblk); if (rc) return rc; }
         { int rc = wf->blk_wmax.reserve(nblk); if (rc) return rc; }
         { int rc = wf->blk_alive.reserve(nblk); if (rc) return rc; }
+        { int rc = wf->blk_alive_prev.reserve(nblk); if (rc) return rc; }
         { int rc = wf->blk_work.reserve(3 * nblk); if (rc) return rc; }
         wf->blk_cap = nblk;
     }
@@ -551,6 +575,8 @@
     DF_HIP(hipMemsetAsync(wf->blk_state, on_demand ? 0 : 1, nblk, st));
     DF_HIP(hipMemsetAsync(wf->blk_tie, 0, nblk, st));
     DF_HIP(hipMemsetAsync(wf->blk_wmax, 0, nblk * sizeof(float), st));
+    DF_HIP(hipMemsetAsync(wf->blk_alive, 1, nblk, st));
+    DF_HIP(hipMemsetAsync(wf->blk_alive_prev, 1, nblk, st));
     wf->blk_phase = 0;
     wf->tab_z0 = tz0; wf->tab_zn = tzn; wf->tab_k = k; wf->tab_valid = true; wf->w_tab_valid = weights;
     wf->tab_complete = !on_demand; wf->tab_sweeps = 0; wf->alive_valid = false;
diff --git a/dynamicfusion_amd/csrc/dfusion_warp_blocks.h b/dynamicfusion_amd/csrc/dfusion_warp_blocks.h
--- a/dynamicfusion_amd/csrc/dfusion_warp_blocks.h
+++ b/dynamicfusion_amd/csrc/dfusion_warp_blocks.h
@@ -117,13 +117,15 @@
     }
     __builtin_amdgcn_wave_barrier();
     if constexpr (K == 8) {
-        if (a.code_tab && a.bm_ids && !any_valid) { if (ln == 0) a.bm_coded[blk] = 0; }
+        if (a.code_tab && a.bm_ids && !any_valid) { if (ln == 0) { a.bm_coded[blk] = 0; if (a.bm_sub_ok) a.bm_sub_ok[blk] = 0; } }
         if (a.code_tab && a.bm_ids && any_valid) {
             unsigned code[8];
 #pragma unroll
             for (int j = 0; j < 8; ++j) code[j] = 0u;
             int last_h[2] = {-1, -1};
             bool sub_over = false;
+            float wide_h[2] = {-1.f, -1.f};
+            unsigned ref_h[2] = {0u, 0u}, cnt_h[2] = {0u, 0u};
             const bool writer = (ln & 0x1b) == 0;
             const unsigned qd = ((unsigned)(ln >> 2) & 1u) | (((unsigned)(ln >> 5) & 1u) << 1);
             uint32_t* ids_out = a.bm_ids + blk * 64;
@@ -147,16 +149,36 @@
                 if (e == DF_BM_NU) { sub_over = true; break; }
 #pragma unroll
                 for (int h = 0; h < 2; ++h) {
-                    if (cand_h[h] == 0x7fffffff) continue;
+                    float lmin = 3.0e38f, lmax = 0.f, wmin = 3.0e38f, wmax = 0.f;
 #pragma unroll
                     for (int j = 4 * h; j < 4 * h + 4; ++j)
                         if (valid & (1u << j)) {
                             unsigned hit = 0u;
-#pragma unroll
-                            for (int i = 0; i < K; ++i) hit = ids[j][i] == cand_h[h] ? (unsigned)e << (4 * i) : hit;
+                            float w = 0.f;
+#pragma unroll
+                            for (int i = 0; i < K; ++i) { const bool is = ids[j][i] == cand_h[h]; hit = is ? (unsigned)e << (4 * i) : hit; w = is ? wv[j][i] : w; }
                             code[j] |= hit;
+                            const float lam = w * inv[j];
+                            lmin = fminf(lmin, lam); lmax = fmaxf(lmax, lam); wmin = fminf(wmin, w); wmax = fmaxf(wmax, w);
                         }
+                    if (a.bm_sub_lam) {
+#pragma unroll
+                        for (int o = 1; o <= 16; o <<= 1) {
+                            if (o == 4) continue;
+                            lmin = fminf(lmin, __shfl_xor(lmin, o, 64)); lmax = fmaxf(lmax, __shfl_xor(lmax, o, 64));
+                            wmin = fminf(wmin, __shfl_xor(wmin, o, 64)); wmax = fmaxf(wmax, __shfl_xor(wmax, o, 64));
+                        }
+                    }
+                    if (cand_h[h] == 0x7fffffff) continue;
                     if (writer) ((uint16_t*)(ids_out + qd * 16 + (unsigned)e))[h] = (uint16_t)cand_h[h];
+                    if (writer && a.bm_sub_lam) {
+                        const uint32_t lp = df_bm_pack(lmin * (1.f - 0x1p-18f), lmax * (1.f + 0x1p-18f));
+                        const size_t at = (blk * DF_BM_NU + (unsigned)e) * 8 + (unsigned)h * 4u + qd;
+                        a.bm_sub_lam[at] = lp; a.bm_sub_w[at] = df_bm_pack(wmin, wmax);
+                        const float hw = h2f_bits(lp >> 16);
+                        if (hw > wide_h[h]) { wide_h[h] = hw; ref_h[h] = (unsigned)e; }
+                        cnt_h[h] = (unsigned)e + 1u;
+                    }
                     last_h[h] = cand_h[h];
                 }
             }
@@ -165,8 +187,13 @@
                 for (int j = 0; j < 8; ++j)
                     if (col_in && z0 + j < a.Z) a.code_tab[df_code_index(a, x, y, z0 + j)] = code[j];
             }
+            if (writer && a.bm_sub_lam) {
+#pragma unroll
+                for (int h = 0; h < 2; ++h) a.bm_sub_cnt[blk * 8 + (unsigned)h * 4u + qd] = (uint16_t)(cnt_h[h] | (ref_h[h] << 8));
+            }
             __builtin_amdgcn_wave_barrier();
             if (ln == 0) a.bm_coded[blk] = sub_over ? (uint8_t)0 : (uint8_t)1;
+            if (ln == 0 && a.bm_sub_ok) a.bm_sub_ok[blk] = (sub_over || bad) ? (uint8_t)0 : (uint8_t)1;
         }
     }
     if (ln == 0) blk_state[blk] = 2;
@@ -189,35 +216,26 @@
     }
 }
 
-__device__ __forceinline__ bool df_block_box_dead(const DfWarpedArgs& a, const float4* __restrict__ rot, const float4* __restrict__ node_t,
-                                                  int nbx, int nby, size_t nblk, size_t blk, unsigned n, const uint16_t* __restrict__ bm_idx,
-                                                  const uint32_t* __restrict__ bm_lam, const uint32_t* __restrict__ bm_w)
-{
+struct DfBoxSums {
     float slm = 0.f, Nx = 0.f, Ny = 0.f, Nz = 0.f, Ex = 0.f, Ey = 0.f, Ez = 0.f, Dmin = 3.0e38f, Dmax = 0.f;
     float Tx = 0.f, Ty = 0.f, Tz = 0.f, Fx = 0.f, Fy = 0.f, Fz = 0.f, sx = 0.f, sy = 0.f, sz = 0.f;
-    {   const float4 r0 = rot[bm_idx[blk]]; sx = r0.y; sy = r0.z; sz = r0.w; }
-    for (unsigned e0 = 0; e0 < n; e0 += 4) {
-        unsigned id[4]; uint32_t lp[4], wp[4];
-#pragma unroll
-        for (int i = 0; i < 4; ++i) {
-            const size_t at = (size_t)min(e0 + (unsigned)i, n - 1u) * nblk + blk;
-            id[i] = bm_idx[at]; lp[i] = bm_lam[at]; wp[i] = bm_w[at];
-        }
-        float4 r4[4], t4[4];
-#pragma unroll
-        for (int i = 0; i < 4; ++i) { r4[i] = rot[id[i]]; t4[i] = node_t[id[i]]; }
-#pragma unroll
-        for (int i = 0; i < 4; ++i) {
-            const bool on = e0 + (unsigned)i < n;
-            const float lm = on ? h2f_bits(lp[i]) : 0.f, lh = on ? h2f_bits(lp[i] >> 16) : 0.f, wm = on ? h2f_bits(wp[i]) : 0.f, wh = on ? h2f_bits(wp[i] >> 16) : 0.f;
-            slm += lm;
-            Nx += lm * r4[i].y; Ny += lm * r4[i].z; Nz += lm * r4[i].w;
-            Ex += lh * fabsf(r4[i].y - sx); Ey += lh * fabsf(r4[i].z - sy); Ez += lh * fabsf(r4[i].w - sz);
-            Dmin = fminf(Dmin, r4[i].x); Dmax = fmaxf(Dmax, r4[i].x);
-            Tx += wm * t4[i].y; Ty += wm * t4[i].z; Tz += wm * t4[i].w;
-            Fx += wh * fabsf(t4[i].y); Fy += wh * fabsf(t4[i].z); Fz += wh * fabsf(t4[i].w);
-        }
-    }
+    __device__ __forceinline__ void ref(const float4 r0) { sx = r0.y; sy = r0.z; sz = r0.w; }
+    __device__ __forceinline__ void add(bool on, uint32_t lp, uint32_t wp, const float4 r, const float4 t)
+    {
+        const float lm = on ? h2f_bits(lp) : 0.f, lh = on ? h2f_bits(lp >> 16) : 0.f, wm = on ? h2f_bits(wp) : 0.f, wh = on ? h2f_bits(wp >> 16) : 0.f;
+        slm += lm;
+        Nx += lm * r.y; Ny += lm * r.z; Nz += lm * r.w;
+        Ex += lh * fabsf(r.y - sx); Ey += lh * fabsf(r.z - sy); Ez += lh * fabsf(r.w - sz);
+        Dmin = fminf(Dmin, r.x); Dmax = fmaxf(Dmax, r.x);
+        Tx += wm * t.y; Ty += wm * t.z; Tz += wm * t.w;
+        Fx += wh * fabsf(t.y); Fy += wh * fabsf(t.z); Fz += wh * fabsf(t.w);
+    }
+};
+__device__ __forceinline__ bool df_box_dead_finish(const DfWarpedArgs& a, const DfBoxSums& B, int x0, int x1, int y0, int y1, int z0, int z1)
+{
+    float Nx = B.Nx, Ny = B.Ny, Nz = B.Nz;
+    const float Ex = B.Ex, Ey = B.Ey, Ez = B.Ez, Dmin = B.Dmin, Dmax = B.Dmax, Tx = B.Tx, Ty = B.Ty, Tz = B.Tz, Fx = B.Fx, Fy = B.Fy, Fz = B.Fz;
+    const float slm = B.slm, sx = B.sx, sy = B.sy, sz = B.sz;
     const float rest = 1.f - slm;
     Nx += rest * sx; Ny += rest * sy; Nz += rest * sz;
     bool dead = false;
@@ -229,9 +247,6 @@
         U.z = iv(fminf((Nz - Ez) * id0, (Nz - Ez) * id1), fmaxf((Nz + Ez) * id0, (Nz + Ez) * id1));
         const float umax = fmaxf(fmaxf(fmaxf(fabsf(U.x.lo), fabsf(U.x.hi)), fmaxf(fabsf(U.y.lo), fabsf(U.y.hi))), fmaxf(fabsf(U.z.lo), fabsf(U.z.hi)));
         const bool u_ok = umax < 1.0e3f;
-        const int bx = (int)(blk % (size_t)nbx), by = (int)((blk / (size_t)nbx) % (size_t)nby), bz = (int)(blk / ((size_t)nbx * nby));
-        const int x0 = bx * 8, y0 = by * 8, z0 = a.tab_z0 + bz * 8;
-        const int x1 = min(x0 + 7, a.X - 1), y1 = min(y0 + 7, a.Y - 1), z1 = min(z0 + 7, a.Z - 1);
         const float cxv = 0.5f * (float)(x0 + x1) * a.vsx, cyv = 0.5f * (float)(y0 + y1) * a.vsy, czv = 0.5f * (float)(z0 + z1) * a.vsz;
         const float hxv = 0.5f * (float)(x1 - x0) * a.vsx, hyv = 0.5f * (float)(y1 - y0) * a.vsy, hzv = 0.5f * (float)(z1 - z0) * a.vsz;
         const f3 c = aff_mul(a.vol2world, mk3(cxv, cyv, czv));
@@ -284,6 +299,82 @@
     return dead;
 }
 
+__device__ __forceinline__ bool df_block_box_dead(const DfWarpedArgs& a, const float4* __restrict__ rot, const float4* __restrict__ node_t,
+                                                  int nbx, int nby, size_t nblk, size_t blk, unsigned n, const uint16_t* __restrict__ bm_idx,
+                                                  const uint32_t* __restrict__ bm_lam, const uint32_t* __restrict__ bm_w)
+{
+    DfBoxSums B;
+    B.ref(rot[bm_idx[blk]]);
+    for (unsigned e0 = 0; e0 < n; e0 += 4) {
+        unsigned id[4]; uint32_t lp[4], wp[4];
+#pragma unroll
+        for (int i = 0; i < 4; ++i) {
+            const size_t at = (size_t)min(e0 + (unsigned)i, n - 1u) * nblk + blk;
+            id[i] = bm_idx[at]; lp[i] = bm_lam[at]; wp[i] = bm_w[at];
+        }
+        float4 r4[4], t4[4];
+#pragma unroll
+        for (int i = 0; i < 4; ++i) { r4[i] = rot[id[i]]; t4[i] = node_t[id[i]]; }
+#pragma unroll
+        for (int i = 0; i < 4; ++i) B.add(e0 + (unsigned)i < n, lp[i], wp[i], r4[i], t4[i]);
+    }
+    const int bx = (int)(blk % (size_t)nbx), by = (int)((blk / (size_t)nbx) % (size_t)nby), bz = (int)(blk / ((size_t)nbx * nby));
+    const int x0 = bx * 8, y0 = by * 8, z0 = a.tab_z0 + bz * 8;
+    return df_box_dead_finish(a, B, x0, min(x0 + 7, a.X - 1), y0, min(y0 + 7, a.Y - 1), z0, min(z0 + 7, a.Z - 1));
+}
+
+__global__ __launch_bounds__(256) void df_sub_verdict_kernel(const DfWarpedArgs a, const float4* __restrict__ rot, const float4* __restrict__ node_t,
+                                                             int nbx, int nby, int nbz, const uint32_t* __restrict__ list, const uint32_t* __restrict__ count,
+                                                             uint8_t* __restrict__ blk_sub)
+{
+    const size_t nblk = (size_t)nbx * nby * nbz;
+    const unsigned n_lanes = min(*count, (uint32_t)nblk) * 8u;
+    for (unsigned base = blockIdx.x * 256u + (threadIdx.x & ~63u); base < n_lanes; base += gridDim.x * 256u) {
+    const unsigned i = base + (threadIdx.x & 63u);
+    const bool in = i < n_lanes;
+    size_t blk = in ? (size_t)list[i >> 3] : 0;
+    if (blk >= nblk) blk = 0;
+    const unsigned sub = i & 7u, h = sub >> 2, q = sub & 3u;
+    const unsigned cr = a.bm_sub_cnt[blk * 8 + sub];
+    const uint4* idp = (const uint4*)(a.bm_ids + blk * 64 + q * 16);
+    const uint4 i0 = idp[0], i1 = idp[1], i2 = idp[2], i3 = idp[3];
+    const unsigned idw[DF_BM_NU] = {i0.x, i0.y, i0.z, i0.w, i1.x, i1.y, i1.z, i1.w, i2.x, i2.y, i2.z, i2.w, i3.x, i3.y, i3.z, i3.w};
+    uint32_t lp[DF_BM_NU], wp[DF_BM_NU];
+    const size_t at0 = blk * (8 * DF_BM_NU) + sub;
+#pragma unroll
+    for (int e = 0; e < DF_BM_NU; ++e) { lp[e] = a.bm_sub_lam[at0 + 8 * e]; wp[e] = a.bm_sub_w[at0 + 8 * e]; }
+    const unsigned n = in ? min(cr & 0xffu, (unsigned)DF_BM_NU) : 0u, e_ref = min(cr >> 8, (unsigned)DF_BM_NU - 1u);
+    unsigned id[DF_BM_NU], id_ref = 0u;
+#pragma unroll
+    for (int e = 0; e < DF_BM_NU; ++e) {
+        id[e] = (unsigned)e < n ? (idw[e] >> (16u * h)) & 0xffffu : 0u;
+        id_ref = (unsigned)e == e_ref ? id[e] : id_ref;
+    }
+    bool live = n != 0u;
+    const bool judge = in && n != 0u && a.cull[1] <= 1.0f;
+    DfBoxSums B;
+    B.ref(rot[id_ref]);
+#pragma unroll
+    for (int g = 0; g < DF_BM_NU; g += 8) {
+        if (g != 0 && __builtin_amdgcn_ballot_w64(judge && n > (unsigned)g) == 0ull) break;
+        float4 r4[8], t4[8];
+#pragma unroll
+        for (int j = 0; j < 8; ++j) { r4[j] = rot[id[g + j]]; t4[j] = node_t[id[g + j]]; }
+#pragma unroll
+        for (int j = 0; j < 8; ++j) if ((unsigned)(g + j) < n) B.add(true, lp[g + j], wp[g + j], r4[j], t4[j]);
+    }
+    if (judge) {
+        const int bx = (int)(blk % (size_t)nbx), by = (int)((blk / (size_t)nbx) % (size_t)nby), bz = (int)(blk / ((size_t)nbx * nby));
+        const int x0 = bx * 8 + (int)(q & 1u) * 4, y0 = by * 8 + (int)(q >> 1) * 4, z0 = a.tab_z0 + bz * 8 + (int)h * 4;
+        if (x0 < a.X && y0 < a.Y && z0 < a.Z)
+            live = !df_box_dead_finish(a, B, x0, min(x0 + 3, a.X - 1), y0, min(y0 + 3, a.Y - 1), z0, min(z0 + 3, a.Z - 1));
+        else live = false;
+    }
+    const unsigned long long m = __builtin_amdgcn_ballot_w64(live);
+    if (in && sub == 0u) blk_sub[blk] = (uint8_t)((unsigned)(m >> ((threadIdx.x & 63u) & ~7u)) & 0xffu);
+    }
+}
+
 #ifdef DF_TRACE_VERDICT
 __device__ unsigned long long g_df_vtrace[8192 * 4];
 #define DF_VT(i) do { if ((threadIdx.x & 63) == 0 && blockIdx.x * 4 + (threadIdx.x >> 6) < 8192) g_df_vtrace[(blockIdx.x * 4 + (threadIdx.x >> 6)) * 4 + (i)] = wall_clock64(); } while (0)
@@ -297,13 +388,16 @@
                                                                const uint32_t* __restrict__ bm_lam, const uint32_t* __restrict__ bm_w,
                                                                const uint8_t* __restrict__ bm_cnt, const uint8_t* __restrict__ bm_coded, uint8_t* __restrict__ alive,
                                                                uint32_t* __restrict__ build_list, uint32_t* __restrict__ ahead_list, uint32_t* __restrict__ model_list,
-                                                               uint32_t* __restrict__ cnt, uint32_t* __restrict__ cnt_next)
-{
+                                                               uint32_t* __restrict__ cnt, uint32_t* __restrict__ cnt_next,
+                                                               uint8_t* __restrict__ blk_sub, uint32_t* __restrict__ sub_list, const uint8_t* __restrict__ alive_prev)
+{
+    __shared__ unsigned s_sub_n, s_sub_base;
+    if (threadIdx.x == 0) s_sub_n = 0u;
     const size_t nblk = (size_t)nbx * nby * nbz;
     const size_t blk = (size_t)blockIdx.x * 256 + threadIdx.x;
     DF_VT(0);
     if (blockIdx.x == 0 && threadIdx.x < 8) cnt_next[threadIdx.x] = 0u;
-    bool keep = false, near = false, need_build = false, need_ahead = false, need_model = false;
+    bool keep = false, near = false, need_build = false, need_ahead = false, need_model = false, need_sub = false;
     int bx = 0, by = 0, bz = 0;
     if (blk < nblk) {
         bx = (int)(blk % (size_t)nbx); by = (int)((blk / (size_t)nbx) % (size_t)nby); bz = (int)(blk / ((size_t)nbx * nby));
@@ -339,6 +433,15 @@
         }
         DF_VT(2);
         alive[blk] = keep ? (uint8_t)(1u | ((st == 2u && (use_models & 2) && bm_coded[blk] != 0) ? 2u : 0u)) : (uint8_t)0;
+        if (blk_sub) {
+            blk_sub[blk] = 0xffu;
+            if (keep && st == 2u && (use_models & 4) && a.bm_sub_ok[blk] != 0) {
+                const size_t sy = (size_t)nbx, sz = (size_t)nbx * nby;
+                const unsigned n0 = bx > 0 ? alive_prev[blk - 1] : 1u, n1 = bx + 1 < nbx ? alive_prev[blk + 1] : 1u, n2 = by > 0 ? alive_prev[blk - sy] : 1u,
+                               n3 = by + 1 < nby ? alive_prev[blk + sy] : 1u, n4 = bz > 0 ? alive_prev[blk - sz] : 1u, n5 = bz + 1 < nbz ? alive_prev[blk + sz] : 1u;
+                need_sub = n0 == 0u || n1 == 0u || n2 == 0u || n3 == 0u || n4 == 0u || n5 == 0u;
+            }
+        }
         need_build = keep && build_on_demand && st == 0u;
         need_ahead = !keep && near && build_on_demand && st == 0u;
         need_model = (keep || near) && want_models && (st == 1u || (need_build && want_models > 1));
@@ -365,6 +468,17 @@
         if ((threadIdx.x & 63) == 0) base = atomicAdd(&cnt[1], (unsigned)__popcll(mm));
         base = (unsigned)__builtin_amdgcn_readfirstlane((int)base);
         if (need_model) model_list[base + (unsigned)__popcll(mm & below)] = (unsigned)blk;
+    }
+    if (blk_sub) {
+        const unsigned long long ms = __builtin_amdgcn_ballot_w64(need_sub);
+        unsigned wbase = 0;
+        __syncthreads();
+        if (ms && (threadIdx.x & 63) == 0) wbase = atomicAdd(&s_sub_n, (unsigned)__popcll(ms));
+        wbase = (unsigned)__builtin_amdgcn_readfirstlane((int)wbase);
+        __syncthreads();
+        if (threadIdx.x == 0 && s_sub_n) s_sub_base = atomicAdd(&cnt[5], s_sub_n);
+        __syncthreads();
+        if (need_sub) sub_list[s_sub_base + wbase + (unsigned)__popcll(ms & below)] = (unsigned)blk;
     }
     DF_VT(3);
 }
diff --git a/dynamicfusion_amd/csrc/dfusion_warp_pipe.h b/dynamicfusion_amd/csrc/dfusion_warp_pipe.h
--- a/dynamicfusion_amd/csrc/dfusion_warp_pipe.h
+++ b/dynamicfusion_amd/csrc/dfusion_warp_pipe.h
@@ -1,5 +1,6 @@
 #pragma once
 #include "dfusion_warp_sweep.h"
+#include "dfusion_plan_halves.h"
 
 template <int K> struct DfTabRaw;
 template <> struct DfTabRaw<8> { uint4 idx; float4 w0, w1; unsigned code; };
@@ -169,7 +170,8 @@
     __syncthreads();
     const unsigned item = blockIdx.x * (DF_PLAN_WG / 64) + (threadIdx.x >> 6);
     const int ln = threadIdx.x & 63, p = ln >> 4, l = ln & 15;
-    unsigned long long m = 0;
+    unsigned long long m = 0, hw01 = 0, hw23 = 0;
+    unsigned n_half = 0;
     if (item < n_items) {
         const unsigned half = item & 1u, tcol = item >> 1;
         const int tx = (int)(tcol % (unsigned)tiles_x), ty = (int)((tcol / (unsigned)tiles_x) % (unsigned)tiles_y);
@@ -178,32 +180,46 @@
         const int own1 = min(a.z_own0 + a.z_own_n, a.Z);
         const int x0 = tx * DF_ROW_TX + p * 8, y0 = ty * DF_LDS_TY + (int)half * 8;
         bool keep = l < a.zt && max((lt0 + l) * DF_ROW_TZ, a.z_own0) < min((lt0 + l + 1) * DF_ROW_TZ, own1) && x0 < a.X && y0 < a.Y;
-        unsigned verdict = 1u;
+        unsigned verdict = 1u, sub = 0xffu;
         if (keep && a.blk_alive) {
-            verdict = a.blk_alive[((size_t)(lt0 + l - a.tab_z0 / DF_ROW_TZ) * a.bm_nby + (unsigned)(y0 >> 3)) * a.bm_nbx + (unsigned)(x0 >> 3)];
+            const size_t blk = ((size_t)(lt0 + l - a.tab_z0 / DF_ROW_TZ) * a.bm_nby + (unsigned)(y0 >> 3)) * a.bm_nbx + (unsigned)(x0 >> 3);
+            verdict = a.blk_alive[blk];
             keep = verdict != 0u;
-        }
+            if (keep && a.blk_sub) {
+                sub = a.blk_sub[blk];
+                if (sub == 0u) const_cast<uint8_t*>(a.blk_alive)[blk] = 0;
+            }
+        }
+        const int np0 = keep && (sub & 0x0fu) ? df_half_planes((lt0 + l) * DF_ROW_TZ, 0, a.z_own0, own1) : 0;
+        const int np1 = keep && (sub & 0xf0u) ? df_half_planes((lt0 + l) * DF_ROW_TZ, 1, a.z_own0, own1) : 0;
+        keep = (np0 | np1) != 0;
         m = __builtin_amdgcn_ballot_w64(keep);
+        const unsigned long long m0 = __builtin_amdgcn_ballot_w64(np0 != 0), m1 = __builtin_amdgcn_ballot_w64(np1 != 0);
+        n_half = (unsigned)__popcll(m0) + (unsigned)__popcll(m1);
+        hw01 = (unsigned long long)df_halves_word((unsigned)m0 & 0xffffu, (unsigned)m1 & 0xffffu) |
+               ((unsigned long long)df_halves_word((unsigned)(m0 >> 16) & 0xffffu, (unsigned)(m1 >> 16) & 0xffffu) << 32);
+        hw23 = (unsigned long long)df_halves_word((unsigned)(m0 >> 32) & 0xffffu, (unsigned)(m1 >> 32) & 0xffffu) |
+               ((unsigned long long)df_halves_word((unsigned)(m0 >> 48) & 0xffffu, (unsigned)(m1 >> 48) & 0xffffu) << 32);
         if (code_out) {
             const bool coded = keep && a.blk_alive && (verdict & 2u) != 0u;
             const unsigned long long cm = __builtin_amdgcn_ballot_w64(coded);
             if (ln == 0 && m) code_out[item] = cm;
         }
         if (a.n_swept) {
-            unsigned v = keep ? (unsigned)(64 * (min((lt0 + l + 1) * DF_ROW_TZ, own1) - max((lt0 + l) * DF_ROW_TZ, a.z_own0))) : 0u;
+            unsigned v = (unsigned)(64 * (np0 + np1));
 #pragma unroll
             for (int o = 32; o >= 1; o >>= 1) v += __shfl_xor(v, o, 64);
             if (ln == 0 && v) atomicAdd(a.n_swept, (unsigned long long)v);
         }
     }
-    const unsigned w = (unsigned)__popcll(m);
+    const unsigned w = (n_half + 1u) >> 1;
     unsigned slot = 0;
     if (ln == 0 && m) slot = atomicAdd(&s_cnt[w], 1u);
     __syncthreads();
     if (threadIdx.x < DF_PLAN_BINS && s_cnt[threadIdx.x]) s_base[threadIdx.x] = atomicAdd(&cnt[threadIdx.x], s_cnt[threadIdx.x]);
     __syncthreads();
     if (ln == 0 && m) {
-        mask_out[item] = m;
+        mask_out[2 * (size_t)item] = hw01; mask_out[2 * (size_t)item + 1] = hw23;
         bins[(size_t)w * n_items + s_base[w] + slot] = item;
     }
 }
@@ -238,22 +254,25 @@
     const unsigned long long t_start = wall_clock64();
     unsigned n_layers = 0;
 #endif
-    unsigned items_s[SPW]; unsigned long long masks_s[SPW];
+    unsigned items_s[SPW]; unsigned long long masks_s[2 * SPW];
     unsigned long long cmask_s[SPW];
     unsigned total2 = 0;
 #pragma unroll
     for (unsigned s_ = 0; s_ < SPW; ++s_) {
         const unsigned sidx = group * SPW + s_;
-        items_s[s_] = 0u; masks_s[s_] = 0ull;
+        items_s[s_] = 0u; masks_s[2 * s_] = masks_s[2 * s_ + 1] = 0ull;
         cmask_s[s_] = 0ull;
         if (sidx < n_alive) {
             const int j = __ffsll((unsigned long long)__builtin_amdgcn_ballot_w64(sidx < bin_end)) - 1;
             const unsigned r = sidx - ((unsigned)__builtin_amdgcn_readlane((int)bin_end, j) - (unsigned)__builtin_amdgcn_readlane((int)bin_cnt, j));
             items_s[s_] = (unsigned)__builtin_amdgcn_readfirstlane((int)a.plan_bins[(size_t)(DF_PLAN_BINS - 1 - j) * a.plan_items + r]);
-            const unsigned long long m = a.plan_mask[items_s[s_]];
-            masks_s[s_] = ((unsigned long long)(unsigned)__builtin_amdgcn_readfirstlane((int)(unsigned)(m >> 32)) << 32) |
-                          (unsigned long long)(unsigned)__builtin_amdgcn_readfirstlane((int)(unsigned)m);
-            total2 += 2u * (unsigned)__popcll(masks_s[s_]);
+#pragma unroll
+            for (unsigned w_ = 0; w_ < 2u; ++w_) {
+                const unsigned long long m = a.plan_mask[2 * (size_t)items_s[s_] + w_];
+                masks_s[2 * s_ + w_] = ((unsigned long long)(unsigned)__builtin_amdgcn_readfirstlane((int)(unsigned)(m >> 32)) << 32) |
+                                       (unsigned long long)(unsigned)__builtin_amdgcn_readfirstlane((int)(unsigned)m);
+                total2 += (unsigned)__popcll(masks_s[2 * s_ + w_]);
+            }
             if (CODES && a.plan_code) {
                 const unsigned long long cm = a.plan_code[items_s[s_]];
                 cmask_s[s_] = ((unsigned long long)(unsigned)__builtin_amdgcn_readfirstlane((int)(unsigned)(cm >> 32)) << 32) |
@@ -267,27 +286,22 @@
     for (unsigned q = 0; q < SPW * 4u; ++q) {
     unsigned item = items_s[0]; unsigned long long m_item = masks_s[0];
 #pragma unroll
-    for (unsigned s_ = 1; s_ < SPW; ++s_) if ((q >> 2) == s_) { item = items_s[s_]; m_item = masks_s[s_]; }
-    const unsigned a16 = (unsigned)(m_item >> (16u * (q & 3u))) & 0xffffu;
+    for (unsigned s_ = 1; s_ < SPW; ++s_) if ((q >> 2) == s_) item = items_s[s_];
+#pragma unroll
+    for (unsigned w_ = 1; w_ < 2 * SPW; ++w_) if ((q >> 1) == w_) m_item = masks_s[w_];
+    const unsigned h32 = (unsigned)(m_item >> (32u * (q & 1u)));
     unsigned long long c_item = cmask_s[0];
 #pragma unroll
     for (unsigned s_ = 1; s_ < SPW; ++s_) if ((q >> 2) == s_) c_item = cmask_s[s_];
     const unsigned cbits = CODES ? (unsigned)(c_item >> (16u * (q & 3u))) & 0xffffu : 0u;
-    const unsigned n2 = 2u * (unsigned)__popc(a16);
+    const unsigned n2 = (unsigned)__popc(h32);
     const unsigned seg_lo = max(c0, pre), seg_hi = min(c1, pre + n2);
     const unsigned pre0 = pre;
     pre += n2;
     if (seg_lo >= seg_hi) continue;
     const unsigned lo = seg_lo - pre0, hi = seg_hi - pre0;
-    unsigned alive = a16;
-    for (unsigned i = 0; i < (lo >> 1); ++i) alive &= alive - 1u;
-    {
-        unsigned keep = ((hi - 1u) >> 1) - (lo >> 1) + 1u, rest = alive, seg = 0u;
-        for (unsigned i = 0; i < keep; ++i) { const unsigned low = rest & (0u - rest); seg |= low; rest ^= low; }
-        alive = seg;
-    }
-    int first_l = __ffs(alive) - 1, last_l = 31 - __clz(alive);
-    int z_first_off = (int)(lo & 1u) * (DF_ROW_TZ / 2), z_last_off = ((int)((hi - 1u) & 1u) + 1) * (DF_ROW_TZ / 2);
+    const unsigned seg = df_halves_segment(h32, lo, hi);
+    const unsigned alive = df_halves_layers(seg);
     const int wave_patch = (int)(q & 3u);
     const unsigned tcol = item >> 1;
     const int tx = (int)(tcol % (unsigned)tiles_x), ty = (int)((tcol / (unsigned)tiles_x) % (unsigned)a.plan_tiles_y);
@@ -299,10 +313,8 @@
     const int xc = min(x, a.X - 1), yc = min(y, a.Y - 1);
     const float fxv = (float)x * a.vsx, fyv = (float)y * a.vsy;
     const int lt0 = a.bz0 + (int)(tcol / ((unsigned)tiles_x * (unsigned)a.plan_tiles_y)) * a.zt;
-    auto layer_zb = [&](int l) { const int z = max((lt0 + l) * DF_ROW_TZ, a.z_own0); return l == first_l ? max(z, (lt0 + l) * DF_ROW_TZ + z_first_off) : z; };
-    auto layer_ze = [&](int l) { const int z = min((lt0 + l + 1) * DF_ROW_TZ, own1); return l == last_l ? min(z, (lt0 + l) * DF_ROW_TZ + z_last_off) : z; };
-    if (alive && layer_zb(first_l) >= layer_ze(first_l)) { alive &= alive - 1u; first_l = alive ? __ffs(alive) - 1 : 0; z_first_off = 0; }
-    if (alive && layer_zb(last_l) >= layer_ze(last_l)) { alive &= ~(1u << last_l); last_l = alive ? 31 - __clz(alive) : 0; z_last_off = DF_ROW_TZ; }
+    auto layer_zb = [&](int l) { return max((lt0 + l) * DF_ROW_TZ + df_halves_z0(seg, l), a.z_own0); };
+    auto layer_ze = [&](int l) { return min((lt0 + l) * DF_ROW_TZ + df_halves_z1(seg, l), own1); };
     if (alive) {
         auto advance = [&](int l, int z0, int* nl, int* nz0) {
             *nl = l; *nz0 = z0 + U;
diff --git a/dynamicfusion_amd/csrc/dfusion_warp_sweep.h b/dynamicfusion_amd/csrc/dfusion_warp_sweep.h
--- a/dynamicfusion_amd/csrc/dfusion_warp_sweep.h
+++ b/dynamicfusion_amd/csrc/dfusion_warp_sweep.h
@@ -31,6 +31,8 @@
     const uint8_t* blk_alive; int bm_nbx, bm_nby;
     uint32_t* code_tab; uint32_t* bm_ids; uint8_t* bm_coded;
     const unsigned long long* plan_code;
+    uint32_t* bm_sub_lam; uint32_t* bm_sub_w; uint16_t* bm_sub_cnt; uint8_t* bm_sub_ok;
+    const uint8_t* blk_sub;
     float* blk_wmax; const uint32_t* work; const uint32_t* work_cnt; uint32_t* work_cursor;
     float pf_margin;
     unsigned pf_cap;
diff --git a/dynamicfusion_amd/tsdf_volume.py b/dynamicfusion_amd/tsdf_volume.py
--- a/dynamicfusion_amd/tsdf_volume.py
+++ b/dynamicfusion_amd/tsdf_volume.py
@@ -211,7 +211,7 @@
 
     def integrate_warped(self, dists, camera_pose, intr, warp_field, k=None, n_updated=None, cull=True, sync=True,
                          use_table=True, use_weights=True, use_lds=True, pipelined=True, zero_skip=True, depth_pyramid=True, block_model=True,
-                         prefetch=True, codes=True):
+                         prefetch=True, codes=True, sub_verdict=True):
         k = warp_field.k if k is None else k
         world2cam = affine_mul(affine_inv(np.asarray(camera_pose, F32)), warp_field.warp_to_live_)
         warp_field.ensure_index(self, k)
@@ -223,13 +223,13 @@
             (0 if use_weights else capi.DF_WARP_NO_WEIGHT_TABLE) | (0 if use_lds else capi.DF_WARP_NO_LDS) |
             (0 if pipelined else capi.DF_WARP_NO_PIPELINE) | (0 if zero_skip else capi.DF_WARP_NO_ZERO_SKIP) |
             (0 if depth_pyramid else capi.DF_WARP_NO_DEPTH_PYRAMID) | (capi.DF_WARP_STEADY_PREFETCH if prefetch == "steady" else 0 if prefetch else capi.DF_WARP_NO_PREFETCH) |
-            (0 if codes else capi.DF_WARP_NO_CODES) |
+            (0 if codes else capi.DF_WARP_NO_CODES) | (0 if sub_verdict else capi.DF_WARP_NO_SUB_VERDICT) |
             (capi.DF_WARP_BLOCK_MODEL_NOW if block_model == "now" else 0 if block_model else capi.DF_WARP_NO_BLOCK_MODEL),
             _ptr(n_updated) if n_updated is not None else None, _stream()), "dfusion_integrate_warped")
         if sync:
             torch.cuda.current_stream().synchronize()
 
-    def integrate_warped_prepare(self, dists, camera_pose, intr, warp_field, k=None, prefetch=True, block_model=True, codes=True):
+    def integrate_warped_prepare(self, dists, camera_pose, intr, warp_field, k=None, prefetch=True, block_model=True, codes=True, sub_verdict=True):
         k = warp_field.k if k is None else k
         world2cam = affine_mul(affine_inv(np.asarray(camera_pose, F32)), warp_field.warp_to_live_)
         warp_field.ensure_index(self, k)
@@ -238,7 +238,7 @@
             dp, pitch, cols, rows, self.c_volume(), self.c_slab(), capi.floats(aff12(self.pose_)),
             capi.floats(aff12(world2cam)), intr.as_proj(), warp_field.handle, k,
             (capi.DF_WARP_STEADY_PREFETCH if prefetch == "steady" else 0 if prefetch else capi.DF_WARP_NO_PREFETCH) |
-            (0 if codes else capi.DF_WARP_NO_CODES) |
+            (0 if codes else capi.DF_WARP_NO_CODES) | (0 if sub_verdict else capi.DF_WARP_NO_SUB_VERDICT) |
             (capi.DF_WARP_BLOCK_MODEL_NOW if block_model == "now" else 0 if block_model else capi.DF_WARP_NO_BLOCK_MODEL),
             _stream()), "dfusion_integrate_warped_prepare")
 
diff --git a/include/dfusion.h b/include/dfusion.h
--- a/include/dfusion.h
+++ b/include/dfusion.h
@@ -45,6 +45,7 @@
 #define DF_WARP_BLOCK_MODEL_NOW 256u
 #define DF_WARP_NO_PREFETCH 512u
 #define DF_WARP_NO_CODES 2048u
+#define DF_WARP_NO_SUB_VERDICT 4096u
 #define DF_WARP_STEADY_PREFETCH 1024u
 #define DF_INDEX_VOXEL_TABLE 1u
 #define DF_INDEX_WEIGHT_TABLE 2u
```

New measurement: 2009 (median of 6 runs). 1.06x the previous value.
